# facebookresearch/robust_cvd

Measured on AMD Instinct MI355X. Metric: GN/LM iterations/sec (and ms/iter) on 300-frame 384x224 video, 1/2/4/8 GPU, higher is better.
Workload: dtype f64

## Files before the change

### include/cvd_hip_debug.h

```cpp
#ifndef CVD_HIP_DEBUG_H
#define CVD_HIP_DEBUG_H

#include "cvd_hip.h"

#ifdef __cplusplus
extern "C" {
#endif

typedef struct cvd_debug_options {
  uint64_t struct_size;
  int32_t force_iterations;
  int32_t force_sharded_path;
  int32_t pcg_lockstep;
  int32_t stall_fused_tail_once;
  int32_t tail_no_row_staging;
  int32_t tail_closes_scalars;
} cvd_debug_options;
void cvd_debug_options_default(cvd_debug_options* o);
int32_t cvd_set_debug_options(cvd_handle* h, const cvd_debug_options* o);

int32_t cvd_set_generic_kernels(cvd_handle* h, int32_t enabled);

int32_t cvd_comm_init_local_group(cvd_handle* h, int32_t rank, int32_t world, uint64_t group_key);
int32_t cvd_comm_init_phantom(cvd_handle* h, int32_t rank, int32_t world);

int32_t cvd_block_inverse_debug(cvd_handle* h, int32_t num_blocks, int32_t block_size, const double* a, int32_t variant,
                                float* inverse, int32_t* failed);

int32_t cvd_epipolar_debug(cvd_handle* h, int32_t num_pairs, const int64_t* offsets, const float* loc, double pixel_scale,
                           double threshold_px, int32_t iterations, uint64_t seed, uint8_t* is_static_out,
                           double* fundamental_out, int32_t* best_out, int32_t* counts_out, double* hypotheses_out);
int32_t cvd_flow_masks_debug(cvd_handle* h, int32_t num_frames, int32_t height, int32_t width, int32_t channels,
                             const float* color, int32_t num_pairs, const int32_t* pair_frames, const float* flow_ab,
                             const float* flow_ba, float flow_thresh, float color_thresh, uint8_t* mask_ab, uint8_t* mask_ba,
                             int32_t* kept, float* errors, double* kernel_ms, int32_t pixels_per_thread);
int32_t cvd_dense_inverse_debug(cvd_handle* h, int32_t n, const double* a, double* inverse, int32_t* failed);
int32_t cvd_coarse_debug(cvd_handle* h, int32_t* num_unknowns, double* a_c, double* a_c_inverse, int32_t* failed);
int32_t cvd_temporal_debug(cvd_handle* h, int32_t* dims6, double* a_t, double* a_t_inverse, double* lam, int32_t* failed);
int32_t cvd_product_launch_debug(cvd_handle* h, int32_t* out6);
int32_t cvd_assembly_launch_debug(cvd_handle* h, int32_t* out6, double* cost_frame);

#ifdef __cplusplus
}
#endif
#endif
```

### robust_cvd_amd/api.py

```python
import ctypes as C
import os
import sys

from . import build as _build
from .binding import Binding
from .ctypes_types import OptParams, SolveSummary, XformDesc

_lib = None
_variant = None


class SolverOptions(C.Structure):
    _fields_ = [
        ("struct_size", C.c_uint64),
        ("pcg_relative_tolerance", C.c_double),
        ("pcg_max_iterations", C.c_int32),
        ("verbose", C.c_int32),
        ("coarse_level", C.c_int32),
        ("robust_loss", C.c_int32),
        ("dense_matrix_free", C.c_int32),
        ("block_inverse_variant", C.c_int32),
        ("coarse_dense_max_unknowns", C.c_int32),
        ("coarse_rebuild_excess", C.c_int32),
        ("coarse_update_budget", C.c_int64),
        ("coarse_dense_shift", C.c_double),
        ("constraint_order", C.c_int32),
        ("coarse_rebuild_excess_dense", C.c_int32),
        ("pcg_fused_tail", C.c_int32),
        ("coarse_dense_row_split", C.c_int32),
        ("dist_owner_update", C.c_int32),
        ("temporal_level", C.c_int32),
        ("temporal_step", C.c_int32),
        ("temporal_grid_x", C.c_int32),
        ("temporal_grid_y", C.c_int32),
        ("coarse_temporal_step", C.c_int32),
        ("coarse_over_budget", C.c_int32),
        ("coarse_temporal_min_frames", C.c_int32),
        ("temporal_weight", C.c_double),
    ]


class DebugOptions(C.Structure):
    _fields_ = [
        ("struct_size", C.c_uint64),
        ("force_iterations", C.c_int32),
        ("force_sharded_path", C.c_int32),
        ("pcg_lockstep", C.c_int32),
        ("stall_fused_tail_once", C.c_int32),
        ("tail_no_row_staging", C.c_int32),
        ("tail_closes_scalars", C.c_int32),
    ]


class ConsistencyDesc(C.Structure):
    _fields_ = [
        ("struct_size", C.c_uint64),
        ("precision", C.c_int32),
        ("num_frames", C.c_int32),
        ("num_pairs", C.c_int32),
        ("height", C.c_int32),
        ("width", C.c_int32),
        ("distance_type", C.c_int32),
        ("have_warp", C.c_int32),
        ("reserved", C.c_int32),
        ("lambda_reprojection", C.c_double),
        ("lambda_disparity", C.c_double),
        ("lambda_depth_ratio", C.c_double),
        ("distance_scale", C.c_double),
        ("distance_alpha", C.c_double),
    ]


class SceneFlowDesc(C.Structure):
    _fields_ = [
        ("struct_size", C.c_uint64),
        ("precision", C.c_int32),
        ("num_frames", C.c_int32),
        ("num_pairs", C.c_int32),
        ("height", C.c_int32),
        ("width", C.c_int32),
        ("distance_type_static", C.c_int32),
        ("distance_type_smooth", C.c_int32),
        ("have_warp", C.c_int32),
        ("lambda_static", C.c_double),
        ("lambda_smooth_reprojection", C.c_double),
        ("lambda_smooth_disparity", C.c_double),
        ("lambda_smooth_depth_ratio", C.c_double),
        ("distance_scale", C.c_double),
        ("distance_alpha", C.c_double),
    ]


class SpatialDesc(C.Structure):
    _fields_ = [
        ("struct_size", C.c_uint64),
        ("precision", C.c_int32),
        ("num_frames", C.c_int32),
        ("frames_per_sample", C.c_int32),
        ("height", C.c_int32),
        ("width", C.c_int32),
        ("reserved", C.c_int32),
        ("lambda_disparity_smooth", C.c_double),
        ("sigma_color_grad", C.c_double),
        ("lambda_contrast_loss", C.c_double),
        ("contrast_thresh", C.c_double),
    ]


class ParamDesc(C.Structure):
    _fields_ = [
        ("struct_size", C.c_uint64),
        ("precision", C.c_int32),
        ("num_tensors", C.c_int32),
    ]


class ParamRecord(C.Structure):
    _fields_ = [
        ("beta1", C.c_double),
        ("beta2", C.c_double),
        ("eps", C.c_double),
        ("grad_decay", C.c_double),
        ("param_decay", C.c_double),
        ("step", C.c_double),
        ("denom_scale", C.c_double),
        ("rule", C.c_int32),
        ("reserved", C.c_int32),
    ]


class DatasetDesc(C.Structure):
    _fields_ = [
        ("struct_size", C.c_uint64),
        ("num_frames", C.c_int32),
        ("height", C.c_int32),
        ("width", C.c_int32),
        ("num_pairs", C.c_int32),
        ("num_samples", C.c_int32),
        ("temporal", C.c_int32),
        ("has_depth_orig", C.c_int32),
        ("neighbor_rule_frames", C.c_int32),
    ]


class DatasetBatchOut(C.Structure):
    _fields_ = [
        ("struct_size", C.c_uint64),
        ("images", C.c_void_p),
        ("extrinsics", C.c_void_p),
        ("intrinsics", C.c_void_p),
        ("gc_indices", C.c_void_p),
        ("gc_flows", C.c_void_p * 2),
        ("gc_masks", C.c_void_p * 2),
        ("ts_indices", C.c_void_p),
        ("ts_flows", C.c_void_p * 4),
        ("ts_masks", C.c_void_p * 4),
        ("ts_valid", C.c_void_p),
        ("scales", C.c_void_p),
        ("warp", C.c_void_p),
        ("depth_orig", C.c_void_p),
    ]


PARAM_RULES = {"adam": 0, "radam": 1, "radam_sgd": 2, "moments": 3}

DISTANCE_TYPES = {"l1": 0, "l2": 1, "smooth_l1": 2, "cauchy": 3, "general": 4}
CONSISTENCY_TERMS = ("reproj", "disp", "depth ratio")
SCENE_FLOW_TERMS = ("static", "smooth_reproj", "smooth_disparity", "smooth_depth_ratio")

ABI_REVISION = 6


def consistency_desc(precision, num_frames, num_pairs, height, width, distance="l1", scale=1.0, alpha=1.0,
                     lambdas=(1.0, 0.0, 100.0), have_warp=False):
    if distance not in DISTANCE_TYPES:
        raise ValueError(f"unknown distance {distance!r} (one of {sorted(DISTANCE_TYPES)})")
    d = ConsistencyDesc()
    d.struct_size = C.sizeof(ConsistencyDesc) | (ABI_REVISION << 32)
    d.precision = int(precision)
    d.num_frames, d.num_pairs, d.height, d.width = int(num_frames), int(num_pairs), int(height), int(width)
    d.distance_type = DISTANCE_TYPES[distance]
    d.have_warp = int(bool(have_warp))
    d.lambda_reprojection, d.lambda_disparity, d.lambda_depth_ratio = (float(v) for v in lambdas)
    d.distance_scale, d.distance_alpha = float(scale), float(alpha)
    return d


def scene_flow_desc(precision, num_frames, num_pairs, height, width, distance_static="l1", distance_smooth="l1", scale=1.0,
                    alpha=1.0, lambdas=(1.0, 1.0, 0.0, 100.0), have_warp=False):
    for distance in (distance_static, distance_smooth):
        if distance not in DISTANCE_TYPES:
            raise ValueError(f"unknown distance {distance!r} (one of {sorted(DISTANCE_TYPES)})")
    d = SceneFlowDesc()
    d.struct_size = C.sizeof(SceneFlowDesc) | (ABI_REVISION << 32)
    d.precision = int(precision)
    d.num_frames, d.num_pairs, d.height, d.width = int(num_frames), int(num_pairs), int(height), int(width)
    d.distance_type_static, d.distance_type_smooth = DISTANCE_TYPES[distance_static], DISTANCE_TYPES[distance_smooth]
    d.have_warp = int(bool(have_warp))
    (d.lambda_static, d.lambda_smooth_reprojection, d.lambda_smooth_disparity,
     d.lambda_smooth_depth_ratio) = (float(v) for v in lambdas)
    d.distance_scale, d.distance_alpha = float(scale), float(alpha)
    return d

# ... 1289 lines not shown
                self._check(self._fn("raft_encoder_timed")(*args, ms))
                kernel_ms[:] = list(ms)
            if _hip_runtime().hipDeviceSynchronize() != 0:
                raise RuntimeError("raft_encoder: the device reported an error")
            dev.download(do, out)
        return out

    @staticmethod
    def _midas_f32(who, arrays):
        import numpy as np
        for a in arrays:
            if a is not None and a.dtype != np.float32:
                raise TypeError(f"{who}: every array must be float32 (got {a.dtype})")

    def midas_conv(self, x, weight, bias=None, relu_in=False, relu=False, a=None, relu_a=False, b=None, split=0):
        import numpy as np
        x, weight = np.asarray(x), np.asarray(weight)
        bias, a, b = (None if v is None else np.asarray(v) for v in (bias, a, b))
        self._midas_f32("midas_conv", [x, weight, bias, a, b])
        B, H, W, Cin, N, k = midas_check_conv(x.shape, weight.shape, None if bias is None else bias.shape,
                                              None if a is None else a.shape, None if b is None else b.shape, split)
        out = np.zeros((B, N, H, W), np.float32)
        with _DeviceArrays() as dev:
            dx, dw = dev.upload(np.ascontiguousarray(x)), dev.upload(np.ascontiguousarray(weight))
            db, da, d2 = (None if v is None else dev.upload(np.ascontiguousarray(v)) for v in (bias, a, b))
            do = dev.alloc(out.nbytes)
            self._check(self._fn("midas_conv_device")(
                self._h, C.c_int32(B), C.c_int32(H), C.c_int32(W), C.c_int32(Cin), C.c_int32(N), C.c_int32(k), dx, dw, db,
                C.c_int32(1 if relu_in else 0), C.c_int32(1 if relu else 0), da, C.c_int32(1 if relu_a else 0), d2, C.c_int32(split),
                do, None))
            if _hip_runtime().hipDeviceSynchronize() != 0:
                raise RuntimeError("midas_conv: the device reported an error")
            dev.download(do, out)
        return out

    def midas_upsample2x(self, x, align_corners=True):
        import numpy as np
        x = np.asarray(x)
        self._midas_f32("midas_upsample2x", [x])
        B, Cn, H, W = midas_check_upsample2x(x.shape)
        out = np.zeros((B, Cn, 2 * H, 2 * W), np.float32)
        with _DeviceArrays() as dev:
            dx = dev.upload(np.ascontiguousarray(x))
            do = dev.alloc(out.nbytes)
            self._check(self._fn("midas_upsample2x_device")(
                self._h, C.c_int32(B), C.c_int32(Cn), C.c_int32(H), C.c_int32(W), C.c_int32(1 if align_corners else 0), dx, do, None))
            if _hip_runtime().hipDeviceSynchronize() != 0:
                raise RuntimeError("midas_upsample2x: the device reported an error")
            dev.download(do, out)
        return out

    def midas_head(self, x, weight2, bias2, weight4, bias4, non_negative=True):
        import numpy as np
        arrays = [np.asarray(v) for v in (x, weight2, bias2, weight4, bias4)]
        self._midas_f32("midas_head", arrays)
        B, H, W, Cin = midas_check_head(*[v.shape for v in arrays])
        out = np.zeros((B, H, W), np.float32)
        with _DeviceArrays() as dev:
            dx, dw2, db2, dw4, db4 = (dev.upload(np.ascontiguousarray(v)) for v in arrays)
            do = dev.alloc(out.nbytes)
            self._check(self._fn("midas_head_device")(
                self._h, C.c_int32(B), C.c_int32(H), C.c_int32(W), C.c_int32(Cin), C.c_int32(MIDAS_HEAD_MID), dx, dw2, db2, dw4, db4,
                C.c_int32(1 if non_negative else 0), do, None))
            if _hip_runtime().hipDeviceSynchronize() != 0:
                raise RuntimeError("midas_head: the device reported an error")
            dev.download(do, out)
        return out

    def midas_decoder(self, maps, weights, biases, non_negative=True, kernel_ms=None):
        import numpy as np
        maps = [np.asarray(v) for v in maps]
        weights, biases = [np.asarray(v) for v in weights], [np.asarray(v) for v in biases]
        self._midas_f32("midas_decoder", maps + weights + biases)
        B, features, channels, heights, widths = midas_check_decoder([v.shape for v in maps], [v.shape for v in weights],
                                                                     [v.shape for v in biases])
        out = np.zeros((B, 4 * heights[0], 4 * widths[0]), np.float32)
        with _DeviceArrays() as dev:
            dm = (C.c_void_p * 4)(*[dev.upload(np.ascontiguousarray(v)).value for v in maps])
            dw = (C.c_void_p * 21)(*[dev.upload(np.ascontiguousarray(v)).value for v in weights])
            db = (C.c_void_p * 17)(*[dev.upload(np.ascontiguousarray(v)).value for v in biases])
            do = dev.alloc(out.nbytes)
            args = (self._h, C.c_int32(B), C.c_int32(features), (C.c_int32 * 4)(*channels), (C.c_int32 * 4)(*heights),
                    (C.c_int32 * 4)(*widths), dm, dw, db, C.c_int32(1 if non_negative else 0), do, None)
            if kernel_ms is None:
                self._check(self._fn("midas_decoder_device")(*args))
            else:
                ms = (C.c_double * MIDAS_TIMED_SLOTS)()
                self._check(self._fn("midas_decoder_timed")(*args, ms))
                kernel_ms[:] = list(ms)
            if _hip_runtime().hipDeviceSynchronize() != 0:
                raise RuntimeError("midas_decoder: the device reported an error")
            dev.download(do, out)
        return out

    def num_active_constraints(self):
        return int(self._lib.cvd_num_active_constraints(self._h))

    def block_inverse_debug(self, blocks, variant=0):
        import numpy as np
        a = np.ascontiguousarray(blocks, dtype=np.float64)
        n, B, B2 = a.shape
        assert B == B2
        out = np.zeros((n, B, B), dtype=np.float32)
        fl = C.c_int32(0)
        self._check(self._fn("block_inverse_debug")(self._h, C.c_int32(n), C.c_int32(B), a.ctypes.data_as(C.POINTER(C.c_double)),
                                                    C.c_int32(variant), out.ctypes.data_as(C.POINTER(C.c_float)), C.byref(fl)))
        return out, fl.value

    def dense_inverse_debug(self, a):
        import numpy as np
        a = np.ascontiguousarray(a, dtype=np.float64)
        n = a.shape[0]
        assert a.shape == (n, n)
        out = np.zeros((n, n), dtype=np.float64)
        fl = C.c_int32(0)
        self._check(self._fn("dense_inverse_debug")(self._h, C.c_int32(n), a.ctypes.data_as(C.POINTER(C.c_double)),
                                                    out.ctypes.data_as(C.POINTER(C.c_double)), C.byref(fl)))
        return out, fl.value

    def temporal_debug(self):
        import numpy as np
        dims = (C.c_int32 * 6)()
        self._check(self._fn("temporal_debug")(self._h, dims, None, None, None, None))
        if dims[0] == 0:
            return None
        n = dims[0]
        a = np.zeros((n, n))
        ai = np.zeros((n, n))
        lam = np.zeros(self.num_frames * self.block_size())
        fl = C.c_int32(0)
        dp = lambda x: x.ctypes.data_as(C.POINTER(C.c_double))
        self._check(self._fn("temporal_debug")(self._h, dims, dp(a), dp(ai), dp(lam), C.byref(fl)))
        return {"NT": n, "S": dims[1], "nn": dims[2], "step": dims[3], "Sx": dims[4], "Sy": dims[5], "a_t": a, "a_t_inverse": ai,
                "lam": lam, "failed": fl.value}

    def path_info(self):
        out = (C.c_int32 * 8)()
        self._check(self._fn("path_info")(self._h, out))
        form = {-1: "none", 0: "exact sparse factor", 1: "exact dense inverse", 2: "temporal pose level"}[out[1]]
        return {"pose_graph_level": form, "depth_grid_level": bool(out[2]), "fused_tail": bool(out[3] & 1), "tail_rows_staged": bool(out[3] & 2),
                "product_sums_shares": bool(out[3] & 4), "rz_shares": out[3] >> 8,
                "tail_disabled": bool(out[4]),
                "taps": out[5], "work_items": out[6], "cross_blocks": bool(out[7])}

    def product_launch_debug(self):
        out = (C.c_int32 * 6)()
        self._check(self._fn("product_launch_debug")(self._h, out))
        kind = {-1: "none", 0: "generic list", 1: "fast list", 2: "fast dense", 3: "cross blocks"}[out[3]]
        return {"threads": out[0], "spec": out[1], "kd": out[2], "kind": out[3], "kind_name": kind, "work_items": out[4],
                "num_cu": out[5]}

    def assembly_launch_debug(self):
        import numpy as np
        out = (C.c_int32 * 6)()
        cost = np.zeros(self.num_frames, dtype=np.float64)
        self._check(self._fn("assembly_launch_debug")(self._h, out, cost.ctypes.data_as(C.POINTER(C.c_double))))
        kind = {-1: "none", 0: "generic", 1: "fast list", 2: "fast dense", 3: "dense fold"}[out[3]]
        return {"threads": out[0], "spec": out[1], "kd": out[2], "kind": out[3], "kind_name": kind, "workgroups": out[4],
                "split_parts": out[5], "cost_frame": cost}

    def coarse_debug(self):
        import numpy as np
        n = C.c_int32(0)
        self._check(self._fn("coarse_debug")(self._h, C.byref(n), None, None, None))
        if n.value == 0:
            return None
        a = np.zeros((n.value, n.value))
        ai = np.zeros((n.value, n.value))
        fl = C.c_int32(0)
        self._check(self._fn("coarse_debug")(self._h, C.byref(n), a.ctypes.data_as(C.POINTER(C.c_double)),
                                             ai.ctypes.data_as(C.POINTER(C.c_double)), C.byref(fl)))
        return {"a_c": a, "a_c_inverse": ai, "failed": fl.value}
```

### robust_cvd_amd/csrc/cvd_api.hip

```cpp
#include "cvd_host.h"
#include "cvd_coarse.h"

namespace cvd {

static void poseOptimizationStep(cvd_handle* h, const cvd_opt_params& p, double depthDeformReg) {
  solve(h, p, depthDeformReg, PK_POSE_STEP);
  paramsToPoses(h, p);
}

static void poseOptimization(cvd_handle* h, const cvd_opt_params& p) {
  posesToParams(h);
  h->records.clear();
  int ctfRows = p.ctf_long, ctfCols = p.ctf_short;
  int dsoRows = p.dso_long, dsoCols = p.dso_short;
  if (h->aspect >= 1.f) {
    std::swap(ctfCols, ctfRows);
    std::swap(dsoCols, dsoRows);
  }
  int initGrid[3] = {1, 1, 1};
  if (h->ddesc.depth_type == CVD_DEPTH_GRID)
    for (int i = 0; i < 3; ++i) initGrid[i] = h->ddesc.grid_size[i];
  const int Nval = (h->ddesc.depth_type == CVD_DEPTH_IDENTITY) ? 0 : valueNumParams(h->ddesc.value_xform);
  size_t nDmax = static_cast<size_t>(h->nD());
  if (p.coarse_to_fine && h->ddesc.depth_type != CVD_DEPTH_IDENTITY && p.num_steps > 1)
// ... 103 lines not shown
extern "C" {

static std::string g_createError;

cvd_handle* cvd_create(int32_t device) {
  try {
    int count = 0;
    hipError_t e = hipGetDeviceCount(&count);
    if (e != hipSuccess || count <= 0)
      throw std::runtime_error("no HIP device available: the optimizer has no CPU path");
    if (device < 0 || device >= count) throw std::runtime_error("invalid device ordinal");
    HIP_CHECK(hipSetDevice(device));
    auto* h = new cvd_handle_t();
    h->device = device;
    h->frontend = makeFrontend();
    HIP_CHECK(hipDeviceGetAttribute(&h->numCU, hipDeviceAttributeMultiprocessorCount, device));
    HIP_CHECK(hipStreamCreateWithFlags(&h->stream, hipStreamNonBlocking));
    {
      int prioLow = 0, prioHigh = 0;
      HIP_CHECK(hipDeviceGetStreamPriorityRange(&prioLow, &prioHigh));
      HIP_CHECK(hipStreamCreateWithPriority(&h->stream2, hipStreamNonBlocking, prioHigh));
    }
    HIP_CHECK(hipEventCreateWithFlags(&h->evCoarseIn, hipEventDisableTiming));
    HIP_CHECK(hipEventCreateWithFlags(&h->evCoarseDone, hipEventDisableTiming));
    HIP_CHECK(hipStreamCreateWithFlags(&h->stream3, hipStreamNonBlocking));
    HIP_CHECK(hipEventCreateWithFlags(&h->evInvIn, hipEventDisableTiming));
    HIP_CHECK(hipEventCreateWithFlags(&h->evInvDone, hipEventDisableTiming));
    cvd_solver_options_default(&h->opt);
    cvd_debug_options_default(&h->dbg);
    touchModule_setup(); touchModule_eval(); touchModule_matvec(); touchModule_precond(); touchModule_temporal(); touchModule_solve(); touchModule_frontend();
    if (device < PersistentGate::kMaxDevices) {
      PersistentGate::Slot& sl = PersistentGate::slot(device);
      std::lock_guard<std::mutex> lock(sl.m);
      if (++g_liveHandles[device] > 1) HIP_CHECK(hipDeviceSynchronize());
    }
    return h;
  } catch (const std::exception& e) {
    g_createError = e.what();
    return nullptr;
  }
}
void cvd_destroy(cvd_handle* h) {
  if (h && h->device >= 0 && h->device < PersistentGate::kMaxDevices) --g_liveHandles[h->device];
  delete h;
}
const char* cvd_last_error(cvd_handle* h) { return h ? h->err.c_str() : g_createError.c_str(); }

int32_t cvd_abi_revision(void) { return CVD_ABI_REVISION; }
void cvd_abi_sizes(int32_t* out6) {
  out6[0] = sizeof(cvd_xform_desc);
  out6[1] = sizeof(cvd_opt_params);
  out6[2] = sizeof(cvd_frame_pose);
  out6[3] = sizeof(cvd_iteration_record);
  out6[4] = sizeof(cvd_solve_summary);
  out6[5] = sizeof(cvd_solver_options);
}

void cvd_opt_params_default(cvd_opt_params* p) {
  std::memset(p, 0, sizeof(*p));
  p->max_iterations = 1000;
  p->num_threads = 12;
  p->num_steps = 4;
  p->robustness = 0.5;
  p->static_loss_type = CVD_STATIC_REPRO_DISPARITY;
  p->static_spatial_weight = 1.0;
  p->static_depth_weight = 1.0;
  p->smooth_loss_type = CVD_SMOOTH_REPRO_DISPARITY_LAPLACIAN;
  p->scale_reg = 1.0;
  p->scale_reg_grid_size = 10;
  p->depth_deform_reg_initial = 1.0;
  p->depth_deform_reg_final = 0.1;
  p->spatial_deform_reg = 1.0;
  p->focal_reg = 1.0;
  p->coarse_to_fine = 1;
  p->ctf_long = 17;
  p->ctf_short = 10;
  p->dso_long = 4;
  p->dso_short = 3;
  p->focal_long = 0.3461538376301239;
  p->intr_opt = CVD_INTR_PER_FRAME;
  p->normalize_depth_from_first_frame = 1;
}

void cvd_solver_options_default(cvd_solver_options* o) {
  o->struct_size = CVD_STRUCT_STAMP(cvd_solver_options);
  o->pcg_relative_tolerance = 1e-3;
  o->pcg_max_iterations = 300;
  o->verbose = 0;
  o->coarse_level = 1;
  o->robust_loss = 0;
  o->dense_matrix_free = 0;
  o->block_inverse_variant = 0;
  o->coarse_dense_max_unknowns = 4096;
  o->coarse_rebuild_excess = 16;
  o->coarse_update_budget = 40000;
  o->coarse_dense_shift = 1e-5;
  o->constraint_order = 1;
  o->coarse_rebuild_excess_dense = 0;
  o->pcg_fused_tail = 1;
  o->coarse_dense_row_split = 5;
  o->dist_owner_update = 1;
  o->temporal_level = 1;
  o->temporal_step = 32;
  o->temporal_grid_x = 0;
  o->temporal_grid_y = 0;
  o->coarse_temporal_step = 8;
  o->coarse_over_budget = 0;
  o->coarse_temporal_min_frames = 128;
  o->temporal_weight = 0.7;
}
int32_t cvd_set_solver_options(cvd_handle* h, const cvd_solver_options* o) {
  CVD_TRY(h, {
    if (o->struct_size != CVD_STRUCT_STAMP(cvd_solver_options))
      throw std::runtime_error(fmt("cvd_solver_options: struct_size %#llx != %#llx = sizeof | revision << 32 (caller built against "
                                   "another cvd_hip.h; start from cvd_solver_options_default)",
                                   static_cast<unsigned long long>(o->struct_size),
                                   static_cast<unsigned long long>(CVD_STRUCT_STAMP(cvd_solver_options))));
    if (o->pcg_fused_tail < 0 || o->pcg_fused_tail > 1) throw std::runtime_error("pcg_fused_tail in {0, 1}");
    if (!(o->pcg_relative_tolerance > 0.0 && o->pcg_relative_tolerance < 1.0)) throw std::runtime_error("pcg_relative_tolerance must lie in (0, 1)");
    if (o->pcg_max_iterations < 1) throw std::runtime_error("pcg_max_iterations must be >= 1");
    if (!(o->coarse_dense_shift >= 0.0 && o->coarse_dense_shift < 1.0)) throw std::runtime_error("coarse_dense_shift must lie in [0, 1)");
    if (o->coarse_rebuild_excess < 0 || o->coarse_rebuild_excess_dense < -1 || o->coarse_update_budget < 0)
      throw std::runtime_error("coarse_rebuild_excess / coarse_update_budget must be >= 0, coarse_rebuild_excess_dense >= -1");
    if (o->coarse_dense_max_unknowns < 0 || o->coarse_dense_max_unknowns > kDenseCoarseMaxUnknowns)
      throw std::runtime_error(fmt("coarse_dense_max_unknowns must lie in [0, %d] (what k_dense_spd_inverse holds in registers)",
                                   kDenseCoarseMaxUnknowns));
    if (o->coarse_level < 0 || o->coarse_level > 3 || o->coarse_temporal_step < 2 || o->robust_loss < 0 || o->robust_loss > 1 || o->block_inverse_variant < 0 ||
        o->block_inverse_variant > 2)
      throw std::runtime_error("coarse_level in {0, 1, 2, 3}, coarse_temporal_step >= 2, robust_loss in {0, 1}, block_inverse_variant in {0, 1, 2}");
    if (o->coarse_over_budget < 0 || o->coarse_over_budget > 1) throw std::runtime_error("coarse_over_budget in {0, 1}");
    if (o->coarse_temporal_min_frames < 0) throw std::runtime_error("coarse_temporal_min_frames must be >= 0");
    if (!(o->temporal_weight > 0.0 && o->temporal_weight <= 2.0)) throw std::runtime_error("temporal_weight must lie in (0, 2]");
    if (o->coarse_dense_row_split < 0 || o->coarse_dense_row_split > 8) throw std::runtime_error("coarse_dense_row_split must lie in [0, 8]");
    if (o->temporal_level < 0 || o->temporal_level > 2 || o->temporal_step < 2 || o->temporal_grid_x < 0 || o->temporal_grid_y < 0 ||
        o->temporal_grid_x == 1 || o->temporal_grid_y == 1)
      throw std::runtime_error("temporal_level in {0, 1, 2}, temporal_step >= 2, temporal_grid_x / _y 0 (automatic) or >= 2");
    if (o->coarse_update_budget != h->opt.coarse_update_budget || o->coarse_dense_max_unknowns != h->opt.coarse_dense_max_unknowns ||
        (o->coarse_level == 3) != (h->opt.coarse_level == 3) || o->coarse_temporal_step != h->opt.coarse_temporal_step ||
        o->coarse_over_budget != h->opt.coarse_over_budget || o->coarse_temporal_min_frames != h->opt.coarse_temporal_min_frames ||
        o->pcg_fused_tail != h->opt.pcg_fused_tail)
      h->tableValid = false;
    if (o->constraint_order != h->opt.constraint_order) h->orderGx = h->orderGy = -1;
    h->opt = *o;
  });
}
void cvd_debug_options_default(cvd_debug_options* o) {
  o->struct_size = CVD_STRUCT_STAMP(cvd_debug_options);
  o->force_iterations = 0;
  o->force_sharded_path = 0;
  o->pcg_lockstep = 0;
  o->stall_fused_tail_once = 0;
  o->tail_no_row_staging = 0;
  o->tail_closes_scalars = 0;
}
int32_t cvd_set_debug_options(cvd_handle* h, const cvd_debug_options* o) {
  CVD_TRY(h, {
    if (o->struct_size != CVD_STRUCT_STAMP(cvd_debug_options))
      throw std::runtime_error("cvd_debug_options: struct_size does not match this library's cvd_hip_debug.h (start from cvd_debug_options_default)");
    h->dbg = *o;
    h->distForced = h->world == 1 && (h->comm != nullptr || h->localGroup || h->phantom) && o->force_sharded_path != 0;
  });
}
void cvd_comm_unique_id(uint8_t* out128) {
  ncclUniqueId id;
  std::memset(&id, 0, sizeof(id));
  (void)ncclGetUniqueId(&id);
  std::memcpy(out128, &id, sizeof(id));
}
int32_t cvd_comm_init(cvd_handle* h, int32_t rank, int32_t world, const uint8_t* id128) {
  CVD_TRY(h, {
    if (world < 1 || rank < 0 || rank >= world) throw std::runtime_error("invalid rank / world size");
    if (h->comm) { NCCL_CHECK(ncclCommDestroy(h->comm)); h->comm = nullptr; }
    ncclUniqueId id;
    std::memcpy(&id, id128, sizeof(id));
    NCCL_CHECK(ncclCommInitRank(&h->comm, world, id, rank));
    h->rank = rank;
    h->world = world;
    h->localGroup.reset();
    h->distForced = world == 1 && h->dbg.force_sharded_path != 0;
    h->tableValid = false;
  });
}
int32_t cvd_comm_init_local_group(cvd_handle* h, int32_t rank, int32_t world, uint64_t group_key) {
  CVD_TRY(h, {
    if (world < 1 || rank < 0 || rank >= world) throw std::runtime_error("invalid rank / world size");
    if (h->comm) { NCCL_CHECK(ncclCommDestroy(h->comm)); h->comm = nullptr; }
    h->localGroup = joinLocalGroup(group_key, world);
    h->rank = rank;
    h->world = world;
    h->distForced = world == 1 && h->dbg.force_sharded_path != 0;
    h->tableValid = false;
  });
}
int32_t cvd_comm_init_phantom(cvd_handle* h, int32_t rank, int32_t world) {
  CVD_TRY(h, {
    if (world < 1 || rank < 0 || rank >= world) throw std::runtime_error("invalid rank / world size");
    if (h->comm) { NCCL_CHECK(ncclCommDestroy(h->comm)); h->comm = nullptr; }
    if (h->localGroup) { leaveLocalGroup(*h->localGroup); h->localGroup.reset(); }
    h->phantom = true;
    h->rank = rank;
    h->world = world;
    h->distForced = world == 1;
    h->tableValid = false;
  });
}
int32_t cvd_set_generic_kernels(cvd_handle* h, int32_t enabled) { CVD_TRY(h, h->forceGeneric = enabled != 0); }

int32_t cvd_set_video(cvd_handle* h, int32_t numFrames, int32_t width, int32_t height, float aspect, float invAspect) {
  CVD_TRY(h, {
    if (numFrames <= 0 || width <= 0 || height <= 0) throw std::runtime_error("invalid video dimensions");
    h->F = numFrames; h->W = width; h->H = height; h->aspect = aspect; h->invAspect = invAspect;
    h->haveDynMasks = false;
    h->adaptGx = h->adaptGy = 0;
    h->dDepth.ensure(static_cast<size_t>(numFrames) * width * height);
    HIP_CHECK(hipMemsetAsync(h->dDepth.p, 0, static_cast<size_t>(numFrames) * width * height * sizeof(float), h->stream));
    h->median.assign(numFrames, 0.f);
    h->medianDirty = true;
    h->poses.assign(numFrames, cvd_frame_pose{{0, 0, 0}, {0, 0, 0, 1}, 0.f, 0.f});
    h->poseParamsValid = false;
    cvd_xform_desc dd{};
    dd.type = CVD_XFORM_DEPTH;
    dd.depth_type = CVD_DEPTH_IDENTITY;
    cvd_xform_desc sd{};
    sd.type = CVD_XFORM_SPATIAL;
    sd.spatial_type = CVD_SPATIAL_IDENTITY;
    resetXforms(h, dd, false);
    resetXforms(h, sd, true);
    h->tableValid = false;
    h->P = 0;
    h->C = 0;
    h->dense = false;
    h->denseListValid = false;
    h->haveTriplets = false;
    h->tripCenter.clear();
    h->tripOff.clear();
    h->tripC = 0;
    h->tripActive.clear();
    h->haveGlobalEdges = false;
    h->globalEdges.clear();
    h->coarse.valid = false;
    h->pairA.clear();
    h->pairB.clear();
    h->pairOff.assign(1, 0);
  });
}

int32_t cvd_set_depth(cvd_handle* h, int32_t frame, const float* depth) {
  CVD_TRY(h, {
    if (frame < 0 || frame >= h->F) throw std::runtime_error("frame out of range");
    const size_t n = static_cast<size_t>(h->W) * h->H;
    HIP_CHECK(hipMemcpyAsync(h->dDepth.p + frame * n, depth, n * sizeof(float), hipMemcpyHostToDevice, h->stream));
    h->medianDirty = true;
    h->tableValid = false;
    HIP_CHECK(hipStreamSynchronize(h->stream));
  });
}

int32_t cvd_set_depth_all(cvd_handle* h, const float* depth) {
  CVD_TRY(h, {
    if (h->F <= 0) throw std::runtime_error("no video set");
    const size_t n = static_cast<size_t>(h->F) * h->W * h->H;
    HIP_CHECK(hipMemcpyAsync(h->dDepth.p, depth, n * sizeof(float), hipMemcpyHostToDevice, h->stream));
    h->medianDirty = true;
    h->tableValid = false;
    HIP_CHECK(hipStreamSynchronize(h->stream));
  });
}

int32_t cvd_set_pair_constraints(cvd_handle* h, int32_t numPairs, const int32_t* pairFrames, const int64_t* offsets,
                                 const float* loc4, const uint8_t* isStatic) {
  CVD_TRY(h, {
    if (numPairs < 0 || !offsets || (numPairs > 0 && !pairFrames)) throw std::runtime_error("invalid pair constraints");
    std::vector<int> order(numPairs);
    for (int i = 0; i < numPairs; ++i) order[i] = i;
    std::stable_sort(order.begin(), order.end(), [&](int a, int b) {
      if (pairFrames[2 * a] != pairFrames[2 * b]) return pairFrames[2 * a] < pairFrames[2 * b];
      return pairFrames[2 * a + 1] < pairFrames[2 * b + 1];
    });
    if (offsets[0] != 0) throw std::runtime_error("pair constraint offsets must start at 0");
    for (int i = 0; i < numPairs; ++i)
      if (offsets[i + 1] < offsets[i]) throw std::runtime_error("pair constraint offsets must be non-decreasing");
    for (int k = 1; k < numPairs; ++k)
      if (pairFrames[2 * order[k]] == pairFrames[2 * order[k - 1]] && pairFrames[2 * order[k] + 1] == pairFrames[2 * order[k - 1] + 1])
        throw std::runtime_error("duplicate directed frame pair in the constraint list (merge the two lists: the reference keeps "
                                 "one entry per pair key, lib/FlowConstraints.h:149)");
    const long long C = offsets[numPairs];
    if (C > 0 && !loc4) throw std::runtime_error("invalid pair constraints");
    for (int k = 0; k < numPairs; ++k)
      if (pairFrames[2 * k] < 0 || pairFrames[2 * k] >= h->F || pairFrames[2 * k + 1] < 0 || pairFrames[2 * k + 1] >= h->F)
        throw std::runtime_error("pair frame out of range");
    h->dense = false;
    h->denseListValid = false;
    h->dFlow.release();
    h->dFMask.release();
    h->P = numPairs;
    h->C = C;
    h->pairA.resize(numPairs);
    h->pairB.resize(numPairs);
    h->pairOff.assign(numPairs + 1, 0);
    std::vector<float> loc(static_cast<size_t>(C) * 4);
    std::vector<unsigned char> st(C, 1);
    std::vector<int> cpair(C);
    long long o = 0;
    for (int k = 0; k < numPairs; ++k) {
      const int src = order[k];
      const int a = pairFrames[2 * src], b = pairFrames[2 * src + 1];
      if (a < 0 || a >= h->F || b < 0 || b >= h->F) throw std::runtime_error("pair frame out of range");
      h->pairA[k] = a;
      h->pairB[k] = b;
      h->pairOff[k] = o;
      const long long n = offsets[src + 1] - offsets[src];
// ... 463 lines not shown
int32_t cvd_get_summary(cvd_handle* h, cvd_solve_summary* s) { CVD_TRY(h, *s = h->summary); }
int32_t cvd_num_records(cvd_handle* h) { return h ? static_cast<int32_t>(h->records.size()) : 0; }
int32_t cvd_get_records(cvd_handle* h, cvd_iteration_record* out) {
  CVD_TRY(h, std::memcpy(out, h->records.data(), sizeof(cvd_iteration_record) * h->records.size()));
}
int32_t cvd_get_kernel_times(cvd_handle* h, double* avgMs6, int64_t* launches6) {
  CVD_TRY(h, {
    for (int k = 0; k < KC_COUNT; ++k) {
      avgMs6[k] = h->kcN[k] ? h->kcMs[k] / h->kcN[k] : 0.0;
      launches6[k] = h->kcN[k];
    }
  });
}
int32_t cvd_get_dense_times(cvd_handle* h, double* avgMs2, int64_t* launches2) {
  CVD_TRY(h, {
    for (int k = 0; k < 2; ++k) {
      avgMs2[k] = h->kcN[KC_DENSE_WALK + k] ? h->kcMs[KC_DENSE_WALK + k] / h->kcN[KC_DENSE_WALK + k] : 0.0;
      launches2[k] = h->kcN[KC_DENSE_WALK + k];
    }
  });
}
int32_t cvd_get_comm_times(cvd_handle* h, double* avgMs3, int64_t* counts3) {
  CVD_TRY(h, {
    for (int k = 0; k < 3; ++k) {
      avgMs3[k] = h->kcN[KC_COUNT + k] ? h->kcMs[KC_COUNT + k] / h->kcN[KC_COUNT + k] : 0.0;
      counts3[k] = h->kcN[KC_COUNT + k];
    }
  });
}
int32_t cvd_set_kernel_timing(cvd_handle* h, int32_t enabled) {
  CVD_TRY(h, {
    h->timingStride = ((enabled >> 8) & 0xff) + 1;
    h->timingCounter = 0;
    for (auto& k : h->timingCounterKc) k = 0;
    enabled &= 0xff;
    h->timing = enabled == 1 ? 0x3f : enabled;
    for (int k = 0; k < KC_TOTAL; ++k) { h->kcMs[k] = 0.0; h->kcN[k] = 0; }
  });
}
int64_t cvd_num_active_constraints(cvd_handle* h) { return h ? h->numValid : 0; }

int32_t cvd_set_pair_graph(cvd_handle* h, int32_t numPairs, const int32_t* pairFrames) {
  CVD_TRY(h, {
    std::set<std::pair<int, int>> uniq;
    for (int i = 0; i < numPairs; ++i) {
      const int a = pairFrames[2 * i], b = pairFrames[2 * i + 1];
      if (a < 0 || a >= h->F || b < 0 || b >= h->F) throw std::runtime_error("pair graph frame out of range");
      if (a != b) uniq.insert({std::min(a, b), std::max(a, b)});
    }
    h->globalEdges.assign(uniq.begin(), uniq.end());
    h->haveGlobalEdges = numPairs > 0;
    h->tableValid = false;
  });
}

int32_t cvd_block_inverse_debug(cvd_handle* h, int32_t num_blocks, int32_t block_size, const double* a, int32_t variant,
                                float* inverse, int32_t* failed) {
  CVD_TRY(h, {
    if (num_blocks <= 0 || block_size <= 0 || block_size > kMaxFrameBlock) throw std::runtime_error("block_inverse_debug: bad sizes");
    if (variant < 0 || variant > 2) throw std::runtime_error("block_inverse_debug: variant must be 0, 1 or 2");
    const size_t n = static_cast<size_t>(num_blocks) * block_size * block_size;
    DevBuf<double> dA;
    DevBuf<double> dL;
    DevBuf<float> dM;
    DevBuf<int> dF;
    dA.ensure(n);
    dL.ensure(static_cast<size_t>(num_blocks) * block_size);
    dM.ensure(n);
    dF.ensure(1);
    hipStream_t s = h->stream;
    dA.upload(a, n, s);
    HIP_CHECK(hipMemsetAsync(dL.p, 0, static_cast<size_t>(num_blocks) * block_size * sizeof(double), s));
    HIP_CHECK(hipMemsetAsync(dM.p, 0, n * sizeof(float), s));
    HIP_CHECK(hipMemsetAsync(dF.p, 0, sizeof(int), s));
    Layout L{};
    L.F = num_blocks;
    L.B = block_size;
    launchBlockInverseRaw(h, L, dA.p, dL.p, dM.p, dF.p, variant);
    int fl = 0;
    dM.download(inverse, n, s);
    dF.download(&fl, 1, s);
    HIP_CHECK(hipStreamSynchronize(s));
    if (failed) *failed = fl;
  });
}

int32_t cvd_epipolar_debug(cvd_handle* h, int32_t num_pairs, const int64_t* offsets, const float* loc, double pixel_scale,
                           double threshold_px, int32_t iterations, uint64_t seed, uint8_t* is_static_out,
                           double* fundamental_out, int32_t* best_out, int32_t* counts_out, double* hypotheses_out) {
  CVD_TRY(h, epipolarStaticFlags(h, num_pairs, offsets, loc, pixel_scale, threshold_px, iterations, seed, is_static_out,
                                 fundamental_out, best_out, nullptr, counts_out, hypotheses_out));
}

int32_t cvd_dense_inverse_debug(cvd_handle* h, int32_t n, const double* a, double* inverse, int32_t* failed) {
  CVD_TRY(h, {
    if (n <= 0 || n > 8192) throw std::runtime_error("dense_inverse_debug: bad size");
    const size_t nn = static_cast<size_t>(n) * n;
    DevBuf<double> dA;
    DevBuf<double> dM;
    DevBuf<int> dF;
    dA.ensure(nn);
    dM.ensure(nn);
    dF.ensure(2);
    hipStream_t s = h->stream;
    dA.upload(a, nn, s);
    HIP_CHECK(hipMemsetAsync(dM.p, 0, nn * sizeof(double), s));
    HIP_CHECK(hipMemsetAsync(dF.p, 0, 2 * sizeof(int), s));
    launchDenseSpdInverse(h, n, dA.p, dM.p, dF.p, s, dF.p + 1);
    int fl[2] = {0, 0};
    dM.download(inverse, nn, s);
    dF.download(fl, 2, s);
    HIP_CHECK(hipStreamSynchronize(s));
    if (failed) *failed = fl[0];
  });
}

int32_t cvd_temporal_debug(cvd_handle* h, int32_t* dims6, double* a_t, double* a_t_inverse, double* lam, int32_t* failed) {
  CVD_TRY(h, {
    auto& T = h->temporal;
    hipStream_t s = h->stream;
    const bool on = T.on && T.built;
    const int dims[6] = {on ? T.NT : 0, T.S, T.nn, T.step, T.Sx, T.Sy};
    for (int i = 0; i < 6; ++i) dims6[i] = dims[i];
    if (on) {
      const size_t n2 = static_cast<size_t>(T.NT) * T.NT;
      if (a_t) T.A.download(a_t, n2, s);
      if (a_t_inverse) T.Ainv.download(a_t_inverse, n2, s);
      if (lam) h->dLam.download(lam, static_cast<size_t>(h->F) * h->Bsz(), s);
      int fl = 0;
      T.fail.download(&fl, 1, s);
      HIP_CHECK(hipStreamSynchronize(s));
      if (failed) *failed = fl;
    }
  });
}
int32_t cvd_path_info(cvd_handle* h, int32_t* out8) {
  CVD_TRY(h, {
    out8[0] = h->coarseOn ? 1 : 0;
    out8[1] = !h->coarseOn ? -1 : (h->coarse.temporalPose ? 2 : (h->coarse.denseMode ? 1 : 0));
    out8[2] = h->temporal.on ? 1 : 0;
    out8[3] = h->lastFusedTail ? (h->tailStageRows ? 3 : 1) : 0;
    if (h->lastFusedTail && h->lastShares) out8[3] |= 4 | (h->lastShareCount << 8);
    out8[4] = h->tailDisabled ? 1 : 0;
    out8[5] = h->lastKD;
    out8[6] = static_cast<int32_t>(h->itemFa.size());
    out8[7] = h->lastCross ? 1 : 0;
  });
}
int32_t cvd_product_launch_debug(cvd_handle* h, int32_t* out6) {
  CVD_TRY(h, {
    for (int i = 0; i < 6; ++i) out6[i] = h->lastProduct[i];
  });
}
int32_t cvd_assembly_launch_debug(cvd_handle* h, int32_t* out6, double* cost_frame) {
  CVD_TRY(h, {
    for (int i = 0; i < 6; ++i) out6[i] = h->lastAssembly[i];
    const size_t F = static_cast<size_t>(h->F);
    if (cost_frame && h->lastAssembly[3] >= 0 && h->dCostFrame.n >= F) {
      h->dCostFrame.download(cost_frame, F, h->stream);
      HIP_CHECK(hipStreamSynchronize(h->stream));
    }
  });
}
int32_t cvd_coarse_debug(cvd_handle* h, int32_t* num_unknowns, double* a_c, double* a_c_inverse, int32_t* failed) {
  CVD_TRY(h, {
    auto& C = h->coarse;
    if (!C.valid || !h->coarseOn) {
      *num_unknowns = 0;
    } else if (C.temporalPose) {
      const size_t n = static_cast<size_t>(C.ptN);
      *num_unknowns = static_cast<int32_t>(n);
      hipStream_t s = h->stream;
      int fl = 0;
      C.fail.download(&fl, 1, s);
      if (a_c) C.ptMat.download(a_c, n * n, s);
      if (a_c_inverse) C.ptInv.download(a_c_inverse, n * n, s);
      HIP_CHECK(hipStreamSynchronize(s));
      if (failed) *failed = fl;
    } else {
      const int F = h->F;
      const size_t n = static_cast<size_t>(F) * kCB;
      *num_unknowns = static_cast<int32_t>(n);
      hipStream_t s = h->stream;
      int fl = 0;
      C.fail.download(&fl, 1, s);
      if (a_c_inverse) {
        std::vector<double> save(n), unit(n, 0.0);
        C.rc.download(save.data(), n, s);
        HIP_CHECK(hipStreamSynchronize(s));
        DevBuf<double> scalTmp;
        scalTmp.ensure(S_COUNT);
        HIP_CHECK(hipMemsetAsync(scalTmp.p, 0, S_COUNT * sizeof(double), s));
        for (size_t k = 0; k < n; ++k) {
          unit[k] = 1.0;
          C.rc.upload(unit.data(), n, s);
          if (C.denseMode) {
            hipLaunchKernelGGL(k_coarse_dense_apply, dim3(F), dim3(256), 0, s, F, C.denseInv.p, C.rc.p, C.c.p, C.modeActive.p,
                               C.dotPart.p, scalTmp.p, h->dCounters.p + 3, C.fail.p, 1, 0.0, static_cast<double*>(nullptr));
          } else {
            hipLaunchKernelGGL(k_coarse_apply_w, dim3(F), dim3(1024), 0, s, C.plan, C.Wb.p, C.rc.p, C.y.p, C.dotPart.p,
                               scalTmp.p, h->dCounters.p + 3, C.fail.p, 1, 0.0, static_cast<double*>(nullptr));
            hipLaunchKernelGGL(k_coarse_apply_wt, dim3(F), dim3(256), 0, s, coarseView(h, true, true), F, C.c.p,
                               scalTmp.p, 1);
          }
          C.c.download(a_c_inverse + k * n, n, s);
          HIP_CHECK(hipStreamSynchronize(s));
          unit[k] = 0.0;
        }
        C.rc.upload(save.data(), n, s);
        HIP_CHECK(hipStreamSynchronize(s));
      }
      std::vector<double> diag(static_cast<size_t>(F) * kCBB), edges(static_cast<size_t>(std::max(C.nEdges, 1)) * kCBB);
      std::vector<unsigned char> act(n);
      std::vector<int> efa(C.nEdges), efb(C.nEdges);
      C.diag.download(diag.data(), diag.size(), s);
      C.edges.download(edges.data(), static_cast<size_t>(C.nEdges) * kCBB, s);
      C.modeActive.download(act.data(), n, s);
      C.edgeFa.download(efa.data(), efa.size(), s);
      C.edgeFb.download(efb.data(), efb.size(), s);
      HIP_CHECK(hipStreamSynchronize(s));
      if (failed) *failed = fl;
      if (a_c) {
        std::fill(a_c, a_c + n * n, 0.0);
        for (int f = 0; f < F; ++f)
          for (int i = 0; i < kCB; ++i)
            for (int j = 0; j < kCB; ++j) a_c[(static_cast<size_t>(f) * kCB + i) * n + f * kCB + j] = diag[static_cast<size_t>(f) * kCBB + i * kCB + j];
        for (int e = 0; e < C.nEdges; ++e)
          for (int i = 0; i < kCB; ++i)
            for (int j = 0; j < kCB; ++j) {
              double v = edges[static_cast<size_t>(e) * kCBB + i * kCB + j];
              if (!act[efa[e] * kCB + i] || !act[efb[e] * kCB + j]) v = 0.0;
              a_c[(static_cast<size_t>(efa[e]) * kCB + i) * n + efb[e] * kCB + j] = v;
              a_c[(static_cast<size_t>(efb[e]) * kCB + j) * n + efa[e] * kCB + i] = v;
            }
      }
    }
  });
}

}
```

### robust_cvd_amd/csrc/cvd_assembly.h

```cpp
#pragma once

#include "cvd_kernels.h"

namespace cvd {

template <int KD, int KS>
inline __global__ __launch_bounds__(256) void k_assemble(Layout L, Table T, const double* __restrict__ x,
                                                  const FrameConst* __restrict__ fc, const double* __restrict__ mask,
                                                  const float* __restrict__ median,
                                                  const unsigned char* __restrict__ inRange,
                                                  const unsigned char* __restrict__ rangeFlags,
                                                  const int* __restrict__ fpOff, const int* __restrict__ fpList,
                                                  double* __restrict__ gOut, double* __restrict__ hOut,
                                                  double* __restrict__ costFrame, double* __restrict__ focalG,
                                                  double* __restrict__ focalH, AsmPanels panels, int panelCap) {
  extern __shared__ __attribute__((aligned(16))) double sm[];
  const int B = L.B;
  double* Hs = sm;
  double* gs = Hs + panelCap;
  double* xf = gs + B;
  double* xo = xf + B;
  FrameConst* fcs = reinterpret_cast<FrameConst*>(xo + B);
  double* red = reinterpret_cast<double*>(fcs + 2);
  const int f = blockIdx.x;
  const int tid = threadIdx.x;
  for (int i = tid; i < B; i += 256) {
    gs[i] = 0.0;
    xf[i] = x[static_cast<size_t>(f) * B + i];
  }
  constexpr int FCW = sizeof(FrameConst) / 8;
  if (tid < FCW) reinterpret_cast<double*>(fcs)[tid] = reinterpret_cast<const double*>(fc + f)[tid];
  const double* mf = mask + static_cast<size_t>(f) * B;
  double* hf = hOut + static_cast<size_t>(f) * B * B;
  double staticCost = 0.0, regCostTotal = 0.0;

  for (int pass = 0; pass < panels.n; ++pass) {
  const int r0 = panels.row[pass], r1 = panels.row[pass + 1];
  const int base = r0 * (r0 + 1) / 2, npk = r1 * (r1 + 1) / 2 - base;
  const bool first = pass == 0;
#define CVD_PANEL_ADD(hi_, lo_, val_)                                                       \
  do {                                                                                      \
    const int hi__ = (hi_);                                                                 \
    if (hi__ >= r0 && hi__ < r1) atomicAdd(&Hs[packedIdx(hi__, (lo_)) - base], (val_));     \
  } while (0)
  __syncthreads();
  for (int i = tid; i < npk; i += 256) Hs[i] = 0.0;
  __syncthreads();

  double PP[28];
  double gp[7];
  double cost = 0.0;
  double shG = 0.0, shH = 0.0;
#pragma unroll
  for (int i = 0; i < 28; ++i) PP[i] = 0.0;
#pragma unroll
  for (int i = 0; i < 7; ++i) gp[i] = 0.0;

  if (L.includeStatic) {
    for (int e = fpOff[f]; e < fpOff[f + 1]; ++e) {
      const int code = fpList[e];
      const int p = code >> 1;
      const int side = code & 1;
      const int o = side ? T.pairA[p] : T.pairB[p];
      __syncthreads();
      for (int i = tid; i < B; i += 256) xo[i] = x[static_cast<size_t>(o) * B + i];
      if (tid < FCW) reinterpret_cast<double*>(fcs + 1)[tid] = reinterpret_cast<const double*>(fc + o)[tid];
      __syncthreads();
      const FrameConst& fa = side ? fcs[1] : fcs[0];
      const FrameConst& fb = side ? fcs[0] : fcs[1];
      const double* xa = side ? xo : xf;
      const double* xb = side ? xf : xo;
      for (long long c = T.pairOff[p] + tid; c < T.pairOff[p + 1]; c += 256) {
        const float2 d = T.dsrc[c];
        if (!(d.x > 0.f)) continue;
        Sample<KD, KS> s;
        evalSample<KD, KS, true>(L, fa, fb, xa, xb, T.ndc[c], d, s);
        const double w = s.rho1;
        if (L.intrOpt == kIntrShared) {
#pragma unroll
          for (int rr = 0; rr < 3; ++rr) {
            const double tot = s.a.Jp[rr][6] + s.b.Jp[rr][6];
            s.a.Jp[rr][6] = tot;
            s.b.Jp[rr][6] = tot;
          }
          if (!side && first) {
            shG += w * (s.a.Jp[0][6] * s.r[0] + s.a.Jp[1][6] * s.r[1] + s.a.Jp[2][6] * s.r[2]);
            shH += w * (s.a.Jp[0][6] * s.a.Jp[0][6] + s.a.Jp[1][6] * s.a.Jp[1][6] + s.a.Jp[2][6] * s.a.Jp[2][6]);
          }
        }
        const Side<KD, KS>& me = side ? s.b : s.a;
        if (!side && first) cost += s.rho0;
        if (first) {
          int q = 0;
#pragma unroll
          for (int i = 0; i < 7; ++i) {
            gp[i] += w * (me.Jp[0][i] * s.r[0] + me.Jp[1][i] * s.r[1] + me.Jp[2][i] * s.r[2]);
#pragma unroll
            for (int j = 0; j <= i; ++j) {
              PP[q] += w * (me.Jp[0][i] * me.Jp[0][j] + me.Jp[1][i] * me.Jp[1][j] + me.Jp[2][i] * me.Jp[2][j]);
              ++q;
            }
          }
        }
        const int nt = sideNumTapCols(L, me);
        for (int t = 0; t < nt; ++t) {
          int ct;
          double Jt[3];
          sideTapCol(L, me, t, ct, Jt);
          const double wj0 = w * Jt[0], wj1 = w * Jt[1], wj2 = w * Jt[2];
          if (first) atomicAdd(&gs[ct], wj0 * s.r[0] + wj1 * s.r[1] + wj2 * s.r[2]);
          if (ct >= r0 && ct < r1) {
            const int rowBase = ct * (ct + 1) / 2 - base;
#pragma unroll
            for (int i = 0; i < 7; ++i)
              atomicAdd(&Hs[rowBase + i], wj0 * me.Jp[0][i] + wj1 * me.Jp[1][i] + wj2 * me.Jp[2][i]);
          }
          for (int t2 = 0; t2 <= t; ++t2) {
            int c2;
            double J2[3];
            sideTapCol(L, me, t2, c2, J2);
            const double val = wj0 * J2[0] + wj1 * J2[1] + wj2 * J2[2];
            const int hi = ct > c2 ? ct : c2, lo = ct > c2 ? c2 : ct;
            CVD_PANEL_ADD(hi, lo, val);
          }
        }
      }
    }
  }
  __syncthreads();
  if (first) {
    {
#pragma unroll
      for (int i = 0; i < 28; ++i) PP[i] = waveSum(PP[i]);
#pragma unroll
      for (int i = 0; i < 7; ++i) gp[i] = waveSum(gp[i]);
      cost = waveSum(cost);
      const int wv = tid >> 6;
      if ((tid & 63) == 0) {
#pragma unroll
        for (int i = 0; i < 28; ++i) red[wv * 36 + i] = PP[i];
#pragma unroll
        for (int i = 0; i < 7; ++i) red[wv * 36 + 28 + i] = gp[i];
        red[wv * 36 + 35] = cost;
      }
    }
    __syncthreads();
    if (tid < 28) {
      int i = 0;
      while ((i + 1) * (i + 2) / 2 <= tid) ++i;
      const int j = tid - i * (i + 1) / 2;
      Hs[packedIdx(i, j)] += red[tid] + red[36 + tid] + red[72 + tid] + red[108 + tid];
    } else if (tid < 35) {
      gs[tid - 28] += red[tid] + red[36 + tid] + red[72 + tid] + red[108 + tid];
    }
    __syncthreads();
    staticCost = 0.5 * (red[35] + red[36 + 35] + red[72 + 35] + red[108 + 35]);
    __syncthreads();
  }
  if (L.intrOpt == kIntrShared) {
    if (first) {
      shG = waveSum(shG);
      shH = waveSum(shH);
      if ((tid & 63) == 0) { red[tid >> 6] = shG; red[4 + (tid >> 6)] = shH; }
      __syncthreads();
      if (tid == 0) {
        focalG[f] = red[0] + red[1] + red[2] + red[3];
        focalH[f] = red[4] + red[5] + red[6] + red[7];
        gs[6] = 0.0;
        Hs[packedIdx(6, 6)] = 0.0;
      }
    }
    if (f != 0) {
      for (int j = tid; j < B; j += 256) {
        if (j == 6) continue;
        const int hi = j > 6 ? j : 6, lo = j > 6 ? 6 : j;
        if (hi >= r0 && hi < r1) Hs[packedIdx(hi, lo) - base] = 0.0;
      }
    }
    __syncthreads();
  }

  double regCost = 0.0;
  if (inRange[f]) {
    const int nr = numRegResiduals<KD>(L);
    for (int i = tid; i < nr; i += 256) {
      double r;
      int n;
      int cols[2 * KD + 2];
      double jac[2 * KD + 2];
      regResidual<KD>(L, f, i, xf, median[f], r, n, cols, jac);
      if (first) regCost += r * r;
      for (int a = 0; a < n; ++a) {
        if (first) atomicAdd(&gs[cols[a]], jac[a] * r);
        for (int b = 0; b <= a; ++b) {
          const int hi = cols[a] > cols[b] ? cols[a] : cols[b];
          const int lo = cols[a] > cols[b] ? cols[b] : cols[a];
          CVD_PANEL_ADD(hi, lo, jac[a] * jac[b]);
        }
      }
    }
  }
  if (tid == 0 && L.positionRegSqrt > 0.0 && first) {
    double o3[3] = {0, 0, 0}, dg = 0.0, cst = 0.0;
    posRegFrame(L, rangeFlags, f, x, nullptr, o3, dg, cst);
    for (int i = 0; i < 3; ++i) {
      atomicAdd(&gs[i], o3[i]);
      atomicAdd(&Hs[packedIdx(i, i)], dg);
    }
    regCost += cst;
  }
  if (first) {
    regCost = waveSum(regCost);
    __syncthreads();
    if ((tid & 63) == 0) red[tid >> 6] = regCost;
    __syncthreads();
    regCostTotal = 0.5 * (red[0] + red[1] + red[2] + red[3]);
  }
  __syncthreads();
  for (int idx = tid; idx < npk; idx += 256) {
    int i = static_cast<int>((sqrt(8.0 * static_cast<double>(idx + base) + 1.0) - 1.0) * 0.5);
    while (i * (i + 1) / 2 > idx + base) --i;
    while ((i + 1) * (i + 2) / 2 <= idx + base) ++i;
    const int j = idx + base - i * (i + 1) / 2;
    const double v = Hs[idx] * mf[i] * mf[j];
    hf[static_cast<size_t>(i) * B + j] = v;
    hf[static_cast<size_t>(j) * B + i] = v;
  }
#undef CVD_PANEL_ADD
  }
  if (tid == 0) costFrame[f] = staticCost + regCostTotal;
  __syncthreads();
  for (int i = tid; i < B; i += 256) gOut[static_cast<size_t>(f) * B + i] = gs[i] * mf[i];
}

inline __global__ __launch_bounds__(256) void k_shared_focal_fixup(Layout L, const double* __restrict__ focalG,
                                                            const double* __restrict__ focalH,
                                                            const double* __restrict__ mask, double* __restrict__ g,
                                                            double* __restrict__ hBlocks) {
  __shared__ double red[8];
  double a = 0.0, b = 0.0;
  for (int f = threadIdx.x; f < L.F; f += 256) { a += focalG[f]; b += focalH[f]; }
  a = waveSum(a);
  b = waveSum(b);
  if ((threadIdx.x & 63) == 0) { red[threadIdx.x >> 6] = a; red[4 + (threadIdx.x >> 6)] = b; }
  __syncthreads();
  if (threadIdx.x == 0) {
    const double m = mask[6];
    g[6] += (red[0] + red[1] + red[2] + red[3]) * m;
    hBlocks[static_cast<size_t>(6) * L.B + 6] += (red[4] + red[5] + red[6] + red[7]) * m * m;
  }
}

inline __global__ void k_extract_diag(Layout L, const double* __restrict__ hBlocks, double* __restrict__ out) {
  const size_t n = static_cast<size_t>(L.F) * L.B;
  const size_t i = static_cast<size_t>(blockIdx.x) * blockDim.x + threadIdx.x;
  if (i >= n) return;
  const size_t f = i / L.B, c = i - f * L.B;
  out[i] = hBlocks[(f * L.B + c) * L.B + c];
}


#ifdef CVD_ASM_PROFILE
__device__ unsigned long long g_asmProf[2048 * 16];
#define ASM_STAMP(slot) do { if (lane == 0) g_asmProf[(blockIdx.x & 2047) * 16 + (slot)] = wall_clock64(); } while (0)
#else
#define ASM_STAMP(slot) do {} while (0)
#endif

template <int KD, int SPEC>
__device__ __forceinline__ void asmWalkSpec(const Layout& L, const Table& T, RecordStream<false>& rs, long long cBegin, int n,
                                            int lane, const bool side, const FrameConst& Fa, const FrameConst& Fb,
                                            const double* __restrict__ xa, const double* __restrict__ xb, double* Hs,
                                            double* gs, double (&PP)[28], double (&gp)[7], double (&GD)[19], double& cost) {
  const double A = L.aspect;
  double RaU[9], RbU[9], dTU[3];
#pragma unroll
  for (int i = 0; i < 9; ++i) { RaU[i] = uniformValue(Fa.R[i]); RbU[i] = uniformValue(Fb.R[i]); }
#pragma unroll
  for (int i = 0; i < 3; ++i) dTU[i] = uniformValue(Fa.t[i] - Fb.t[i]);
  const double fya = uniformValue(Fa.fy), fxa = fya * A;
  const double fyb = uniformValue(Fb.fy);
  const double ifyb = uniformValue(1.0 / fyb), ifxb = uniformValue(1.0 / (fyb * A));
  for (int ci = lane; ci < n; ci += 64) {
    float4 nd;
    float2 d;
    if (!rs.take(T, cBegin, ci, 64, n, 0, 0, 0, nd, d)) continue;
    const double da = static_cast<double>(d.x), db = static_cast<double>(d.y);
    FastTaps<KD> ta, tb;
    fastGather<KD>(L, nd.x, nd.y, ta);
    fastGather<KD>(L, nd.z, nd.w, tb);
    double Da = 0.0, Db = 0.0;
#pragma unroll
    for (int k = 0; k < KD; ++k) {
      if (ta.ok(k)) Da += xa[7 + ta.I(k)] * ta.Wt(k);
      if (tb.ok(k)) Db += xb[7 + tb.I(k)] * tb.Wt(k);
    }
    Da *= da;
    Db *= db;
    const double pax = static_cast<double>(nd.x), pay = static_cast<double>(nd.y);
    const double pbx = static_cast<double>(nd.z), pby = static_cast<double>(nd.w);
    double ca[3], Rca[3];
    fastRay(RaU, pax, pay, fxa, fya, ca, Rca);
    const double v[3] = {dTU[0] + Rca[0] * Da, dTU[1] + Rca[1] * Da, dTU[2] + Rca[2] * Da};
    double zz, iz, u, vv, r[3], dr2dA, dr2dDb;
    fastProject<true>(L, RbU, v, ifxb, ifyb, pbx, pby, zz, iz, u, vv, r[0], r[1]);
    fastDepthResidual<true>(L, kLossDisparity, zz, iz, Db, r[2], dr2dA, dr2dDb);
    const double sq = r[0] * r[0] + r[1] * r[1] + r[2] * r[2];
    const double w = fastRobustRho1<SPEC>(L, sq);
    if (!side) cost += fastRobustRho0<SPEC>(L, sq);

    double m00, m11, m02, m12;
    fastRows(L, iz, u, vv, ifxb, ifyb, m00, m11, m02, m12);
    const double m22 = -dr2dA;
    double G[3][3];
#pragma unroll
    for (int i = 0; i < 3; ++i) {
      G[0][i] = m00 * RbU[i * 3 + 0] + m02 * RbU[i * 3 + 2];
      G[1][i] = m11 * RbU[i * 3 + 1] + m12 * RbU[i * 3 + 2];
      G[2][i] = m22 * RbU[i * 3 + 2];
    }
    double Jp[3][7];
    double JD[3];
    if (!side) {
      const double X[3] = {Da * Rca[0], Da * Rca[1], Da * Rca[2]};
      const double cf0 = pax * A, cf1 = pay;
      const double dXdf[3] = {Da * (RaU[0] * cf0 + RaU[1] * cf1), Da * (RaU[3] * cf0 + RaU[4] * cf1),
                              Da * (RaU[6] * cf0 + RaU[7] * cf1)};
#pragma unroll
      for (int rr = 0; rr < 3; ++rr) {
        Jp[rr][0] = G[rr][0]; Jp[rr][1] = G[rr][1]; Jp[rr][2] = G[rr][2];
        Jp[rr][3] = X[1] * G[rr][2] - X[2] * G[rr][1];
        Jp[rr][4] = X[2] * G[rr][0] - X[0] * G[rr][2];
        Jp[rr][5] = X[0] * G[rr][1] - X[1] * G[rr][0];
        Jp[rr][6] = dot3(G[rr], dXdf);
        JD[rr] = dot3(G[rr], Rca);
      }
    } else {
#pragma unroll
      for (int rr = 0; rr < 3; ++rr) {
        Jp[rr][0] = -G[rr][0]; Jp[rr][1] = -G[rr][1]; Jp[rr][2] = -G[rr][2];
        Jp[rr][3] = G[rr][1] * v[2] - G[rr][2] * v[1];
        Jp[rr][4] = G[rr][2] * v[0] - G[rr][0] * v[2];
        Jp[rr][5] = G[rr][0] * v[1] - G[rr][1] * v[0];
      }
      Jp[0][6] = -L.ws * u * ifyb;
      Jp[1][6] = -L.ws * vv * ifyb;
      Jp[2][6] = 0.0;
      JD[0] = 0.0; JD[1] = 0.0; JD[2] = dr2dDb;
    }
    int qi = 0;
#pragma unroll
    for (int i = 0; i < 7; ++i) {
      gp[i] += w * (Jp[0][i] * r[0] + Jp[1][i] * r[1] + Jp[2][i] * r[2]);
#pragma unroll
      for (int j = 0; j <= i; ++j) {
        PP[qi] += w * (Jp[0][i] * Jp[0][j] + Jp[1][i] * Jp[1][j] + Jp[2][i] * Jp[2][j]);
        ++qi;
      }
    }
    double v7[7];
#pragma unroll
    for (int i = 0; i < 7; ++i) v7[i] = w * (Jp[0][i] * JD[0] + Jp[1][i] * JD[1] + Jp[2][i] * JD[2]);
    const double sDD = w * (JD[0] * JD[0] + JD[1] * JD[1] + JD[2] * JD[2]);
    const double sDr = w * (JD[0] * r[0] + JD[1] * r[1] + JD[2] * r[2]);
    const FastTaps<KD>& tm = side ? tb : ta;
    const double dm = side ? db : da;
    if constexpr (KD == 1) {
      const double fac = tm.Wt(0) * dm;
#pragma unroll
      for (int i = 0; i < 7; ++i) GD[i] += v7[i] * fac;
      GD[17] += sDr * fac;
      GD[14] += sDD * fac * fac;
    } else {
#pragma unroll
      for (int ka = 0; ka < KD; ++ka) {
        if (!tm.ok(ka)) continue;
        const double fa = tm.Wt(ka) * dm;
        const int ct = 7 + tm.I(ka);
        const int rowBase = ct * (ct + 1) / 2;
        atomicAdd(&gs[ct], sDr * fa);
#pragma unroll
        for (int i = 0; i < 7; ++i) atomicAdd(&Hs[rowBase + i], v7[i] * fa);
        const double sfa = sDD * fa;
#pragma unroll
        for (int kb = 0; kb <= ka; ++kb) {
          if (!tm.ok(kb)) continue;
          const int c2 = 7 + tm.I(kb);
          const int hi = (KD == 16 || ct > c2) ? ct : c2, lo = (KD == 16 || ct > c2) ? c2 : ct;
          atomicAdd(&Hs[packedIdx(hi, lo)], sfa * (tm.Wt(kb) * dm));
        }
      }
    }
  }
}

template <int NT>
__device__ __forceinline__ void asmLocalToAxisAngle(const double* __restrict__ Jl, int B, int tid, double* Hs, double* gs) {
  double J[9];
#pragma unroll
  for (int i = 0; i < 9; ++i) J[i] = Jl[i];
  for (int j = tid; j < B; j += NT) {
    if (j >= 3 && j <= 5) continue;
    const int i0 = j < 3 ? packedIdx(3, j) : packedIdx(j, 3);
    const int i1 = j < 3 ? packedIdx(4, j) : packedIdx(j, 4);
    const int i2 = j < 3 ? packedIdx(5, j) : packedIdx(j, 5);
    const double h0 = Hs[i0], h1 = Hs[i1], h2 = Hs[i2];
    Hs[i0] = J[0] * h0 + J[1] * h1 + J[2] * h2;
    Hs[i1] = J[3] * h0 + J[4] * h1 + J[5] * h2;
    Hs[i2] = J[6] * h0 + J[7] * h1 + J[8] * h2;
  }
  if (tid == NT - 1) {
    double S[3][3], JS[3][3];
#pragma unroll
    for (int a = 0; a < 3; ++a)
#pragma unroll
      for (int b = 0; b < 3; ++b) S[a][b] = Hs[a >= b ? packedIdx(3 + a, 3 + b) : packedIdx(3 + b, 3 + a)];
#pragma unroll
    for (int a = 0; a < 3; ++a)
#pragma unroll
      for (int b = 0; b < 3; ++b) JS[a][b] = J[a * 3] * S[0][b] + J[a * 3 + 1] * S[1][b] + J[a * 3 + 2] * S[2][b];
#pragma unroll
    for (int a = 0; a < 3; ++a)
#pragma unroll
      for (int b = 0; b <= a; ++b)
        Hs[packedIdx(3 + a, 3 + b)] = JS[a][0] * J[b * 3] + JS[a][1] * J[b * 3 + 1] + JS[a][2] * J[b * 3 + 2];
    const double g0 = gs[3], g1 = gs[4], g2 = gs[5];
    gs[3] = J[0] * g0 + J[1] * g1 + J[2] * g2;
    gs[4] = J[3] * g0 + J[4] * g1 + J[5] * g2;
    gs[5] = J[6] * g0 + J[7] * g1 + J[8] * g2;
  }
}

template <int KD, int NT>
__device__ __forceinline__ double asmRegularisersSpec(const Layout& L, int f, int tid, const double* __restrict__ xf, float median,
                                                      double* Hs, double* gs) {
  constexpr double eps = 1e-6;
  double regCost = 0.0;
  if (L.scaleRegSqrt > 0.0) {
    const int ns = L.sregX * L.sregY;
    const bool taps = KD > 1 || L.depthType == kDepthGlobal;
    for (int i = tid; i < ns; i += NT) {
      const int y = i / L.sregX, x = i - y * L.sregX;
      const float lx = __fadd_rn(-1.f, __fdiv_rn(__fmul_rn(2.f, static_cast<float>(x)), static_cast<float>(L.sregX - 1)));
      const float ly = __fadd_rn(-1.f, __fdiv_rn(__fmul_rn(2.f, static_cast<float>(y)), static_cast<float>(L.sregY - 1)));
      FastTaps<KD> t;
      fastGather<KD>(L, lx, ly, t);
      const double d = static_cast<double>(median);
      double D = (L.depthType == kDepthIdentity) ? d : 0.0;
#pragma unroll
      for (int k = 0; k < KD; ++k)
        if (taps && t.ok(k)) D += d * xf[7 + t.I(k)] * t.Wt(k);
      const bool o = !(D < eps);
      const double dd = o ? D : eps;
      const double r = L.scaleRegSqrt * (1.0 / dd - 1.0);
      const double drdD = o ? (-L.scaleRegSqrt / (dd * dd)) : 0.0;
      regCost += r * r;
#pragma unroll
      for (int ka = 0; ka < KD; ++ka) {
        if (!(taps && t.ok(ka))) continue;
        const int ca = 7 + t.I(ka);
        const double ja = drdD * t.Wt(ka) * d;
        atomicAdd(&gs[ca], ja * r);
#pragma unroll
        for (int kb = 0; kb <= ka; ++kb) {
          if (!t.ok(kb)) continue;
          const int cb = 7 + t.I(kb);
          const int hi = ca > cb ? ca : cb, lo = ca > cb ? cb : ca;
          atomicAdd(&Hs[packedIdx(hi, lo)], ja * (drdD * t.Wt(kb) * d));
        }
      }
    }
  }
  Layout Lr = L;
  Lr.scaleRegSqrt = 0.0;
  const int nr = numRegResiduals<KD>(Lr);
  for (int i = tid; i < nr; i += NT) {
    double r;
    int n;
    int cols[2 * KD + 2];
    double jac[2 * KD + 2];
    regResidual<KD>(Lr, f, i, xf, median, r, n, cols, jac);
    regCost += r * r;
    if (n >= 1) {
      atomicAdd(&gs[cols[0]], jac[0] * r);
      atomicAdd(&Hs[packedIdx(cols[0], cols[0])], jac[0] * jac[0]);
    }
    if (n >= 2) {
      atomicAdd(&gs[cols[1]], jac[1] * r);
      const int hi = cols[1] > cols[0] ? cols[1] : cols[0], lo = cols[1] > cols[0] ? cols[0] : cols[1];
      atomicAdd(&Hs[packedIdx(hi, lo)], jac[1] * jac[0]);
      atomicAdd(&Hs[packedIdx(cols[1], cols[1])], jac[1] * jac[1]);
    }
  }
  return regCost;
}

template <int KD, bool DENSE = false, bool STAGE = false, bool FOLD = false, int SPEC = 0>
inline __global__ __launch_bounds__(kAsmThreads) void k_assemble_fast(Layout L, Table T, const double* __restrict__ x,
                                                       const FrameConst* __restrict__ fc,
                                                       const double* __restrict__ mask, const float* __restrict__ median,
                                                       const unsigned char* __restrict__ regOwner,
                                                       const unsigned char* __restrict__ rangeFlags,
                                                       AsmWork work,
                                                       double* __restrict__ gOut, double* __restrict__ hOut,
                                                       double* __restrict__ costFrame, double* __restrict__ focalG,
                                                       double* __restrict__ focalH, DenseRecords dr = DenseRecords{}) {
  extern __shared__ __attribute__((aligned(16))) double sm[];
  constexpr double eps = 1e-6;
  const int B = L.B;
  const int npk = B * (B + 1) / 2;
  double* Hs = sm;
  double* gs = Hs + npk;
  double* xf = gs + B;
  double* red = xf + B;
  double* xstage = red + 4 * 36;
  const AsmPart me = FOLD ? AsmPart{static_cast<int>(blockIdx.x), 0, 0, 0, 1, 0} : work.parts[blockIdx.x];
  const int f = me.frame;
  const int tid = threadIdx.x;
  static_assert(SPEC == 0 || (!DENSE && !FOLD), "the specialised walk is list mode only");
  constexpr int NT = kAsmThreads;
  const int wv = __builtin_amdgcn_readfirstlane(tid >> 6);
  const int lane = tid & 63;
  if (tid == 0) ASM_STAMP(0);
  for (int i = tid; i < npk; i += NT) Hs[i] = 0.0;
  if (tid < 48) red[tid] = 0.0;
  for (int i = tid; i < B; i += NT) {
    gs[i] = 0.0;
    xf[i] = x[static_cast<size_t>(f) * B + i];
  }
  __syncthreads();
  if (tid == 0) ASM_STAMP(1);

  double PP[28], gp[7];
  double GD[19];
#pragma unroll
  for (int i = 0; i < 19; ++i) GD[i] = 0.0;
  double cost = 0.0;
  double shG = 0.0, shH = 0.0;
#pragma unroll
  for (int i = 0; i < 28; ++i) PP[i] = 0.0;
#pragma unroll
  for (int i = 0; i < 7; ++i) gp[i] = 0.0;
  const int N = SPEC ? 1 : L.N;
  const double A = L.aspect;

  if constexpr (FOLD) {
    if (L.includeStatic) {
      const int G = L.nD;
      const int recN = dwRecordDoubles(G);
      const int e0 = dr.fpOff[f], e1 = dr.fpOff[f + 1];
      const int nOut = 36 + 13 * G;
      for (int o = tid; o < nOut; o += NT) {
        int off0, off1, c = -1, v = 0;
        if (o < 28) {
          int i = 0;
          while ((i + 1) * (i + 2) / 2 <= o) ++i;
          const int j = o - i * (i + 1) / 2;
          off0 = i * 16 + j;
          off1 = (7 + i) * 16 + 7 + j;
        } else if (o < 35) {
          off0 = (o - 28) * 16 + 14;
          off1 = (7 + o - 28) * 16 + 14;
        } else if (o == 35) {
          off0 = 256 + 40 * G;
          off1 = -1;
        } else {
          const int e = o - 36;
          c = e / G;
          v = e - c * G;
          if (c < 7) { off0 = 256 + c * G + v; off1 = 256 + 15 * G + (7 + c) * G + v; }
          else if (c == 7) { off0 = 256 + 14 * G + v; off1 = 256 + 29 * G + v; }
          else { off0 = 256 + 30 * G + (c - 8) * G + v; off1 = 256 + 35 * G + (c - 8) * G + v; }
        }
        double s = 0.0;
        for (int e = e0; e < e1; ++e) {
          const int code = dr.fpList[e];
          const int off = (code & 1) ? off1 : off0;
          if (off < 0) continue;
          for (int q = dr.recOff[code >> 1]; q < dr.recOff[(code >> 1) + 1]; ++q) s += dr.records[static_cast<size_t>(q) * recN + off];
        }
        if (o < 36) atomicAdd(&red[o], s);
        else if (c < 7) Hs[packedIdx(7 + v, c)] = s;
        else if (c == 7) gs[7 + v] = s;
        else {
          const int d = c - 8;
          const int v2 = v + (d == 0 ? 0 : (d == 1 ? 1 : L.gx + d - 3));
          if (v2 < G) atomicAdd(&Hs[packedIdx(7 + v2, 7 + v)], s);
        }
      }
    }
  } else
  if (L.includeStatic) {
    for (int u = me.u0 + wv; u < me.u1; u += NT / 64) {
      const int2 unit = work.units[u];
      const int code = __builtin_amdgcn_readfirstlane(unit.x);
      const int p = code >> 1;
      const int side = code & 1;
      const int o = side ? T.pairA[p] : T.pairB[p];
      const double* __restrict__ xo = x + static_cast<size_t>(o) * B;
      const FrameConst& Fa = side ? fc[o] : fc[f];
      const FrameConst& Fb = side ? fc[f] : fc[o];
      double* xw = xstage + wv * B;
      if constexpr (SPEC != 0) {
        const long long pOff = T.pairOff[p];
        const long long cb = pOff + __builtin_amdgcn_readfirstlane(unit.y);
        const long long pEnd = T.pairOff[p + 1];
        const int n = static_cast<int>((cb + kAsmUnit < pEnd ? cb + kAsmUnit : pEnd) - cb);
        RecordStream<false> rs;
        rs.prime(T, cb, lane, n);
        if constexpr (STAGE) {
          for (int i = lane; i < B; i += 64) xw[i] = xo[i];
          asm volatile("s_waitcnt vmcnt(0) lgkmcnt(0)" ::: "memory");
        }
        const double* xov = STAGE ? xw : xo;
        asmWalkSpec<KD, SPEC>(L, T, rs, cb, n, lane, side != 0, Fa, Fb, side ? xov : xf,
                              side ? xf : xov, Hs, gs, PP, gp, GD, cost);
        continue;
      }
      if constexpr (STAGE) {
        for (int i = lane; i < B; i += 64) xw[i] = xo[i];
        asm volatile("s_waitcnt vmcnt(0) lgkmcnt(0)" ::: "memory");
      }
      const double* xa = STAGE ? (side ? xw : xf) : (side ? xo : xf);
      const double* xb = STAGE ? (side ? xf : xw) : (side ? xf : xo);
      const double fya = Fa.fy, fxa = Fa.fy * A;
      const double fyb = Fb.fy;
      const double ifyb = 1.0 / fyb, ifxb = 1.0 / (fyb * A);
      const long long cBegin = T.pairOff[p] + __builtin_amdgcn_readfirstlane(unit.y);
      constexpr int kUnit = DENSE ? kAsmUnitDense : kAsmUnit;
      const long long cEnd = cBegin + kUnit < T.pairOff[p + 1] ? cBegin + kUnit : T.pairOff[p + 1];
      const int fsrc = side ? o : f, ftgt = side ? f : o;
      const long long cFirst = DENSE ? cBegin + static_cast<long long>(lane) * kDenseRun : cBegin + lane;
      const long long cStop = DENSE ? (cFirst + kDenseRun < cEnd ? cFirst + kDenseRun : cEnd) : cEnd;
      constexpr long long cStep = DENSE ? 1 : 64;
      RecordStream<true> rs;
      const int iFirst = static_cast<int>(cFirst - cBegin), iStop = static_cast<int>(cStop - cBegin);
      if constexpr (DENSE) rs.prime(T, cBegin, iFirst, iStop);
      for (long long c = cFirst; c < cStop; c += cStep) {
        float4 nd;
        float2 d;
        if constexpr (DENSE) {
          if (!rs.take(T, cBegin, static_cast<int>(c - cBegin), 1, iStop, T.pairOff[p], fsrc, ftgt, nd, d)) continue;
        } else {
          if (!loadConstraint<false>(T, c, T.pairOff[p], fsrc, ftgt, nd, d)) continue;
        }
        const double da = static_cast<double>(d.x), db = static_cast<double>(d.y);
        FastTaps<KD> ta, tb;
        fastGather<KD>(L, nd.x, nd.y, ta);
        fastGather<KD>(L, nd.z, nd.w, tb);
        double Da, Db;
        if (N == 0) {
          Da = da; Db = db;
        } else {
          Da = 0.0; Db = 0.0;
#pragma unroll
          for (int k = 0; k < KD; ++k) {
            if (ta.ok(k)) {
              const int ia = ta.I(k);
              if (N == 2) Da += (da * xa[7 + ia * 2] + xa[7 + ia * 2 + 1]) * ta.Wt(k);
              else Da += da * xa[7 + ia] * ta.Wt(k);
            }
            if (tb.ok(k)) {
              const int ib = tb.I(k);
              if (N == 2) Db += (db * xb[7 + ib * 2] + xb[7 + ib * 2 + 1]) * tb.Wt(k);
              else Db += db * xb[7 + ib] * tb.Wt(k);
            }
          }
        }
        const double pax = static_cast<double>(nd.x), pay = static_cast<double>(nd.y);
        const double pbx = static_cast<double>(nd.z), pby = static_cast<double>(nd.w);
        const double ca[3] = {pax * fxa, pay * fya, -1.0};
        const double Rca[3] = {dot3(Fa.R, ca), dot3(Fa.R + 3, ca), dot3(Fa.R + 6, ca)};
        const double v[3] = {Fa.t[0] + Rca[0] * Da - Fb.t[0], Fa.t[1] + Rca[1] * Da - Fb.t[1],
                             Fa.t[2] + Rca[2] * Da - Fb.t[2]};
        const double q0 = Fb.R[0] * v[0] + Fb.R[3] * v[1] + Fb.R[6] * v[2];
        const double q1 = Fb.R[1] * v[0] + Fb.R[4] * v[1] + Fb.R[7] * v[2];
        const double q2 = Fb.R[2] * v[0] + Fb.R[5] * v[1] + Fb.R[8] * v[2];
        const double zz = -q2;
        const double iz = 1.0 / zz;
        const double u = q0 * iz * ifxb;
        const double vv = q1 * iz * ifyb;
        double r[3];
        r[0] = (u - pbx) * L.ws;
        r[1] = (vv - pby) * L.ws;
        double dr2dA, dr2dDb;
        if (L.lossType == kLossDisparity) {
          const bool zo = !(zz < eps), bo = !(Db < eps);
          const double izc = zo ? iz : 1.0 / eps, ibc = 1.0 / (bo ? Db : eps);
          r[2] = (izc - ibc) * L.wd;
          dr2dA = zo ? (-L.wd * izc * izc) : 0.0;
          dr2dDb = bo ? (L.wd * ibc * ibc) : 0.0;
        } else {
          const bool zIsMax = !(zz < Db), zIsMin = !(Db < zz);
          const double mx = zIsMax ? zz : Db, mn = zIsMin ? zz : Db;
          if (L.lossType == kLossRatio) {
            r[2] = (mx / mn - 1.0) * L.wd;
            const double dmx = 1.0 / mn, dmn = -mx / (mn * mn);
            dr2dA = ((zIsMax ? dmx : 0.0) + (zIsMin ? dmn : 0.0)) * L.wd;
            dr2dDb = ((zIsMax ? 0.0 : dmx) + (zIsMin ? 0.0 : dmn)) * L.wd;
          } else {
            r[2] = log(mn / mx) * L.wd;
            const double dmn = 1.0 / mn, dmx = -1.0 / mx;
            dr2dA = ((zIsMax ? dmx : 0.0) + (zIsMin ? dmn : 0.0)) * L.wd;
            dr2dDb = ((zIsMax ? 0.0 : dmx) + (zIsMin ? 0.0 : dmn)) * L.wd;
          }
        }
        double rho0, w;
        robustRho(L, r[0] * r[0] + r[1] * r[1] + r[2] * r[2], rho0, w);
        if (!side) cost += rho0;

        const double wiz = L.ws * iz;
        const double m00 = wiz * ifxb, m11 = wiz * ifyb, m02 = wiz * u, m12 = wiz * vv, m22 = -dr2dA;
        double Jp[3][7];
        double JD[3];
        const FastTaps<KD>& tm = side ? tb : ta;
        const double dm = side ? db : da;
        if (!side) {
          double G[3][3];
#pragma unroll
          for (int i = 0; i < 3; ++i) {
            G[0][i] = m00 * Fb.R[i * 3 + 0] + m02 * Fb.R[i * 3 + 2];
            G[1][i] = m11 * Fb.R[i * 3 + 1] + m12 * Fb.R[i * 3 + 2];
            G[2][i] = m22 * Fb.R[i * 3 + 2];
          }
          const double cf[3] = {pax * A, pay, 0.0};
          const double dXdf[3] = {Da * (Fa.R[0] * cf[0] + Fa.R[1] * cf[1]), Da * (Fa.R[3] * cf[0] + Fa.R[4] * cf[1]),
                                  Da * (Fa.R[6] * cf[0] + Fa.R[7] * cf[1])};
#pragma unroll
          for (int rr = 0; rr < 3; ++rr) {
            Jp[rr][0] = G[rr][0]; Jp[rr][1] = G[rr][1]; Jp[rr][2] = G[rr][2];
            Jp[rr][6] = dot3(G[rr], dXdf);
            JD[rr] = dot3(G[rr], Rca);
          }
#pragma unroll
          for (int i = 0; i < 3; ++i) {
            const double dX[3] = {Da * dot3(Fa.dR[i], ca), Da * dot3(Fa.dR[i] + 3, ca), Da * dot3(Fa.dR[i] + 6, ca)};
            Jp[0][3 + i] = dot3(G[0], dX);
            Jp[1][3 + i] = dot3(G[1], dX);
            Jp[2][3 + i] = dot3(G[2], dX);
          }
        } else {
#pragma unroll
          for (int i = 0; i < 3; ++i) {
            Jp[0][i] = -(m00 * Fb.R[i * 3 + 0] + m02 * Fb.R[i * 3 + 2]);
            Jp[1][i] = -(m11 * Fb.R[i * 3 + 1] + m12 * Fb.R[i * 3 + 2]);
            Jp[2][i] = -(m22 * Fb.R[i * 3 + 2]);
            const double* D = Fb.dR[i];
            const double dq0 = D[0] * v[0] + D[3] * v[1] + D[6] * v[2];
            const double dq1 = D[1] * v[0] + D[4] * v[1] + D[7] * v[2];
            const double dq2 = D[2] * v[0] + D[5] * v[1] + D[8] * v[2];
            Jp[0][3 + i] = m00 * dq0 + m02 * dq2;
            Jp[1][3 + i] = m11 * dq1 + m12 * dq2;
            Jp[2][3 + i] = m22 * dq2;
          }
          Jp[0][6] = -L.ws * u * ifyb;
          Jp[1][6] = -L.ws * vv * ifyb;
          Jp[2][6] = 0.0;
          JD[0] = 0.0; JD[1] = 0.0; JD[2] = dr2dDb;
        }
        if (L.intrOpt == kIntrShared) {
          if (!side) {
            Jp[0][6] += -L.ws * u * ifyb;
            Jp[1][6] += -L.ws * vv * ifyb;
          } else {
            const double cf[3] = {pax * A, pay, 0.0};
            const double dXdf[3] = {Da * (Fa.R[0] * cf[0] + Fa.R[1] * cf[1]), Da * (Fa.R[3] * cf[0] + Fa.R[4] * cf[1]),
                                    Da * (Fa.R[6] * cf[0] + Fa.R[7] * cf[1])};
#pragma unroll
            for (int i = 0; i < 3; ++i) {
              Jp[0][6] += (m00 * Fb.R[i * 3 + 0] + m02 * Fb.R[i * 3 + 2]) * dXdf[i];
              Jp[1][6] += (m11 * Fb.R[i * 3 + 1] + m12 * Fb.R[i * 3 + 2]) * dXdf[i];
              Jp[2][6] += (m22 * Fb.R[i * 3 + 2]) * dXdf[i];
            }
          }
          if (!side) {
            shG += w * (Jp[0][6] * r[0] + Jp[1][6] * r[1] + Jp[2][6] * r[2]);
            shH += w * (Jp[0][6] * Jp[0][6] + Jp[1][6] * Jp[1][6] + Jp[2][6] * Jp[2][6]);
          }
        }
        int qi = 0;
#pragma unroll
        for (int i = 0; i < 7; ++i) {
          gp[i] += w * (Jp[0][i] * r[0] + Jp[1][i] * r[1] + Jp[2][i] * r[2]);
#pragma unroll
          for (int j = 0; j <= i; ++j) {
            PP[qi] += w * (Jp[0][i] * Jp[0][j] + Jp[1][i] * Jp[1][j] + Jp[2][i] * Jp[2][j]);
            ++qi;
          }
        }
        if (N > 0) {
          double v7[7];
#pragma unroll
          for (int i = 0; i < 7; ++i) v7[i] = w * (Jp[0][i] * JD[0] + Jp[1][i] * JD[1] + Jp[2][i] * JD[2]);
          const double sDD = w * (JD[0] * JD[0] + JD[1] * JD[1] + JD[2] * JD[2]);
          const double sDr = w * (JD[0] * r[0] + JD[1] * r[1] + JD[2] * r[2]);
          if constexpr (KD == 16) {
#pragma unroll
            for (int ka = 0; ka < 16; ++ka) {
              if (!tm.ok(ka)) continue;
              const double wa = tm.Wt(ka);
              const int ia = tm.I(ka);
#pragma unroll
              for (int na = 0; na < 2; ++na) {
                if (na >= N) continue;
                const int ct = 7 + ia * N + na;
                const double fa = (N == 2 && na == 1) ? wa : wa * dm;
                const int rowBase = ct * (ct + 1) / 2;
                atomicAdd(&gs[ct], sDr * fa);
#pragma unroll
                for (int i = 0; i < 7; ++i) atomicAdd(&Hs[rowBase + i], v7[i] * fa);
#pragma unroll
                for (int kb = 0; kb <= ka; ++kb) {
                  if (!tm.ok(kb)) continue;
                  const double wb = tm.Wt(kb);
                  const int ib = tm.I(kb);
#pragma unroll
                  for (int nb = 0; nb < 2; ++nb) {
                    if (nb >= N || (kb == ka && nb > na)) continue;
                    const int c2 = 7 + ib * N + nb;
                    const double fb = (N == 2 && nb == 1) ? wb : wb * dm;
                    atomicAdd(&Hs[rowBase + c2], sDD * fa * fb);
                  }
                }
              }
            }
          } else {
          double fac[KD * 2];
          int col[KD * 2];
#pragma unroll
          for (int k = 0; k < KD; ++k) {
            if (N == 2) {
              col[2 * k] = 7 + tm.I(k) * 2;       fac[2 * k] = tm.Wt(k) * dm;
              col[2 * k + 1] = col[2 * k] + 1;    fac[2 * k + 1] = tm.Wt(k);
            } else {
              col[k] = 7 + tm.I(k);               fac[k] = tm.Wt(k) * dm;
            }
          }
          const int nt = (N == 2) ? 2 * KD : KD;
          if constexpr (KD == 1) {
#pragma unroll
            for (int a = 0; a < 2; ++a) {
              if (a < nt) {
#pragma unroll
                for (int i = 0; i < 7; ++i) GD[a * 7 + i] += v7[i] * fac[a];
                GD[17 + a] += sDr * fac[a];
              }
            }
            GD[14] += sDD * fac[0] * fac[0];
            if (N == 2) { GD[15] += sDD * fac[1] * fac[0]; GD[16] += sDD * fac[1] * fac[1]; }
          } else {
#pragma unroll
          for (int a = 0; a < KD * 2; ++a) {
            if (a < nt) {
              const int ct = col[a];
              const int rowBase = ct * (ct + 1) / 2;
              atomicAdd(&gs[ct], sDr * fac[a]);
#pragma unroll
              for (int i = 0; i < 7; ++i) atomicAdd(&Hs[rowBase + i], v7[i] * fac[a]);
#pragma unroll
              for (int b = 0; b < KD * 2; ++b) {
                if (b <= a) {
                  const int c2 = col[b];
                  const int hi = ct > c2 ? ct : c2, lo = ct > c2 ? c2 : ct;
                  atomicAdd(&Hs[packedIdx(hi, lo)], sDD * fac[a] * fac[b]);
                }
              }
            }
          }
          }
          }
        }
      }
    }
  }
  ASM_STAMP(4 + wv);
  __syncthreads();
  if (tid == 0) ASM_STAMP(2);
  {
#pragma unroll
    for (int i = 0; i < 28; ++i) PP[i] = waveSum(PP[i]);
#pragma unroll
    for (int i = 0; i < 7; ++i) gp[i] = waveSum(gp[i]);
    cost = waveSum(cost);
    if constexpr (KD == 1) {
      if (N > 0) {
#pragma unroll
        for (int i = 0; i < 19; ++i) GD[i] = waveSum(GD[i]);
        if (lane == 0) {
          for (int a = 0; a < N; ++a) {
            const int ct = 7 + a;
            for (int i = 0; i < 7; ++i) atomicAdd(&Hs[ct * (ct + 1) / 2 + i], GD[a * 7 + i]);
            atomicAdd(&gs[ct], GD[17 + a]);
          }
          atomicAdd(&Hs[packedIdx(7, 7)], GD[14]);
          if (N == 2) { atomicAdd(&Hs[packedIdx(8, 7)], GD[15]); atomicAdd(&Hs[packedIdx(8, 8)], GD[16]); }
        }
      }
    }
    if (lane == 0) {
#pragma unroll
      for (int i = 0; i < 28; ++i) atomicAdd(&red[i], PP[i]);
#pragma unroll
      for (int i = 0; i < 7; ++i) atomicAdd(&red[28 + i], gp[i]);
      atomicAdd(&red[35], cost);
    }
  }
  __syncthreads();
  if (tid < 28) {
    int i = 0;
    while ((i + 1) * (i + 2) / 2 <= tid) ++i;
    const int j = tid - i * (i + 1) / 2;
    Hs[packedIdx(i, j)] += red[tid];
  } else if (tid < 35) {
    gs[tid - 28] += red[tid];
  }
  __syncthreads();
  const double staticCost = 0.5 * red[35];
  __syncthreads();
  if constexpr (SPEC != 0) {
    asmLocalToAxisAngle<NT>(fc[f].Jl, B, tid, Hs, gs);
    __syncthreads();
  }
  if (tid == 0) ASM_STAMP(13);
  if (L.intrOpt == kIntrShared) {
    shG = waveSum(shG);
    shH = waveSum(shH);
    if (lane == 0) { red[wv] = shG; red[16 + wv] = shH; }
    __syncthreads();
    if (tid == 0) {
      double sg = 0.0, sh = 0.0;
      for (int w = 0; w < NT / 64; ++w) { sg += red[w]; sh += red[16 + w]; }
      focalG[f] = sg;
      focalH[f] = sh;
      red[42] = sg;
      red[43] = sh;
      gs[6] = 0.0;
      Hs[packedIdx(6, 6)] = 0.0;
    }
    if (f != 0) {
      for (int j = tid; j < B; j += NT)
        if (j != 6) Hs[j > 6 ? packedIdx(j, 6) : packedIdx(6, j)] = 0.0;
    }
    __syncthreads();
  }

  if (tid == 0) ASM_STAMP(14);
  double regCost = 0.0;
  if constexpr (SPEC != 0) {
    if (regOwner[f] && me.part == 0) regCost = asmRegularisersSpec<KD, NT>(L, f, tid, xf, median[f], Hs, gs);
  } else
  if (regOwner[f] && me.part == 0) {
    const int nr = numRegResiduals<KD>(L);
    for (int i = tid; i < nr; i += NT) {
      double r;
      int n;
      int cols[2 * KD + 2];
      double jac[2 * KD + 2];
      regResidual<KD>(L, f, i, xf, median[f], r, n, cols, jac);
      regCost += r * r;
      for (int a = 0; a < n; ++a) {
        atomicAdd(&gs[cols[a]], jac[a] * r);
        for (int b = 0; b <= a; ++b) {
          const int hi = cols[a] > cols[b] ? cols[a] : cols[b];
          const int lo = cols[a] > cols[b] ? cols[b] : cols[a];
          atomicAdd(&Hs[packedIdx(hi, lo)], jac[a] * jac[b]);
        }
      }
    }
  }
  if (tid == 0 && L.positionRegSqrt > 0.0 && me.part == 0) {
    double o3[3] = {0, 0, 0}, dg = 0.0, cst = 0.0;
    posRegFrame(L, rangeFlags, f, x, nullptr, o3, dg, cst);
    for (int i = 0; i < 3; ++i) {
      atomicAdd(&gs[i], o3[i]);
      atomicAdd(&Hs[packedIdx(i, i)], dg);
    }
    regCost += cst;
  }
  regCost = waveSum(regCost);
  __syncthreads();
  if (tid == 0) ASM_STAMP(15);
  if (lane == 0) red[wv] = regCost;
  __syncthreads();
  if (tid == 0) {
    double rc = 0.0;
    for (int w = 0; w < NT / 64; ++w) rc += red[w];
    if (me.nParts == 1) costFrame[f] = staticCost + 0.5 * rc;
    red[40] = staticCost + 0.5 * rc;
  }
  if (me.nParts > 1) {
    __syncthreads();
    const size_t stride = static_cast<size_t>(npk) + B + 4;
    double* mine = work.scratch + static_cast<size_t>(me.slot0 + me.part) * stride;
    for (int i = tid; i < npk; i += NT) mine[i] = Hs[i];
    for (int i = tid; i < B; i += NT) mine[npk + i] = gs[i];
    if (tid == 0) {
      mine[npk + B] = red[40];
      if (L.intrOpt == kIntrShared) { mine[npk + B + 1] = red[42]; mine[npk + B + 2] = red[43]; }
    }
    if (!lastBlockArrives(work.counters + f, static_cast<unsigned int>(me.nParts), reinterpret_cast<int*>(red + 41))) return;
#if CVD_DETERMINISTIC
    double costSum = 0.0, sgSum = 0.0, shSum = 0.0;
    for (int i = tid; i < npk; i += NT) Hs[i] = 0.0;
    for (int i = tid; i < B; i += NT) gs[i] = 0.0;
    for (int q = 0; q < me.nParts; ++q) {
#else
    double costSum = red[40];
    double sgSum = red[42], shSum = red[43];
    for (int q = 0; q < me.nParts; ++q) {
      if (q == me.part) continue;
#endif
      const double* other = work.scratch + static_cast<size_t>(me.slot0 + q) * stride;
      for (int i = tid; i < npk; i += NT) Hs[i] += other[i];
      for (int i = tid; i < B; i += NT) gs[i] += other[npk + i];
      costSum += other[npk + B];
      if (L.intrOpt == kIntrShared) { sgSum += other[npk + B + 1]; shSum += other[npk + B + 2]; }
    }
    if (tid == 0) {
      costFrame[f] = costSum;
      if (L.intrOpt == kIntrShared) { focalG[f] = sgSum; focalH[f] = shSum; }
    }
    __syncthreads();
  }

  if (tid == 0) ASM_STAMP(3);
  const double* mf = mask + static_cast<size_t>(f) * B;
// ... 12 lines not shown
```

### robust_cvd_amd/csrc/cvd_eval.hip

```cpp
#include "cvd_host.h"
#include "cvd_cost.h"
#include "cvd_assembly.h"
#include "cvd_triplets.h"
#include "cvd_dense_walk.h"

namespace cvd {

void launchFrameConsts(Ctx& c, const double* x) {
  launchFrameConsts(c.L, x, c.h->dFc.p, c.h->stream);
  HIP_CHECK(hipGetLastError());
}

void spinStream(hipStream_t s) {
  hipError_t e;
  while ((e = hipStreamQuery(s)) == hipErrorNotReady) {}
  HIP_CHECK(e);
}
void spinEvent(hipEvent_t ev) {
  hipError_t e;
  while ((e = hipEventQuery(ev)) == hipErrorNotReady) {}
  HIP_CHECK(e);
}
void readScalars(Ctx& c) {
  HIP_CHECK(hipMemcpyAsync(c.h->hScal, c.h->dScal.p, S_COUNT * sizeof(double), hipMemcpyDeviceToHost, c.h->stream));
  spinStream(c.h->stream);
}

void enqueueCost(Ctx& c, const double* x) {
  cvd_handle* h = c.h;
  hipStream_t s = h->stream;
  launchFrameConsts(c, x);
  const int slot = h->tBegin(KC_COST);
  if (c.L.includeStatic && c.nItems > 0) {
    const size_t lds = (2 * c.L.B) * 8 + 2 * sizeof(FrameConst) + 8 * 8;
    const bool fast = !h->forceGeneric && c.KS == 0 && fastLoss(c.L);
    if (fast) {
      CVD_DISPATCH_KD(c.KD, {
        if (h->dense) {
          allowLds((k_cost_items_fast<KD, true>), lds);
          hipLaunchKernelGGL((k_cost_items_fast<KD, true>), dim3(c.nItems), dim3(256), lds, s, c.L, c.T, c.it, x, h->dFc.p,
                             h->dCostItem.p);
        } else {
          allowLds((k_cost_items_fast<KD, false>), lds);
          hipLaunchKernelGGL((k_cost_items_fast<KD, false>), dim3(c.nItems), dim3(256), lds, s, c.L, c.T, c.it, x, h->dFc.p,
                             h->dCostItem.p);
        }
      });
    } else {
      CVD_DISPATCH(c.KD, c.KS, {
        allowLds(k_cost_items<KD, KS>, lds);
        hipLaunchKernelGGL((k_cost_items<KD, KS>), dim3(c.nItems), dim3(256), lds, s, c.L, c.T, c.it, x, h->dFc.p,
                           h->dCostItem.p);
      });
    }
    HIP_CHECK(hipGetLastError());
  }
  CVD_DISPATCH_KD(c.KD, {
    hipLaunchKernelGGL((k_cost_frames<KD>), dim3(c.L.F), dim3(256), static_cast<size_t>(c.L.B) * 8, s, c.L, x, h->dMedian.p, h->dRegOwner.p, h->dInRange.p,
                       h->dCostFrame.p);
  });
  HIP_CHECK(hipGetLastError());
  if (c.trip && c.TT.nGroups > 0) {
    CVD_DISPATCH(c.KD, c.KS, {
      hipLaunchKernelGGL((k_cost_triplets<KD, KS>), dim3(c.TT.nGroups), dim3(256), 0, s, c.L, c.TT, x, h->dFc.p,
                         h->dCostFrame.p);
    });
    HIP_CHECK(hipGetLastError());
  }
  hipLaunchKernelGGL(k_sum2, dim3(1), dim3(256), 0, s, h->dCostItem.p, (c.L.includeStatic ? c.nItems : 0),
                     h->dCostFrame.p, c.L.F, h->dScal.p, S_COST);
  HIP_CHECK(hipGetLastError());
  if (h->dist()) commAllReduce(h, h->dScal.p + S_COST, 1, CT_F64, s);
  h->tEnd(slot);
}
double evalCost(Ctx& c, const double* x) {
  enqueueCost(c, x);
  readScalars(c);
  return c.h->hScal[S_COST];
}

void enqueueStats(Ctx& c) {
  cvd_handle* h = c.h;
  const int G = static_cast<int>(std::min<size_t>(128, (c.n + 511) / 512));
  h->dStatPart.ensure(7 * 128);
  hipLaunchKernelGGL(k_step_stats, dim3(G), dim3(256), 0, h->stream, c.n, h->dDx.p, h->dG.p, h->dR.p, h->dLam.p,
                     h->dX.p, h->dHd.p, h->dScal.p, h->dStatPart.p, h->dCounters.p + 2);
  HIP_CHECK(hipGetLastError());
}

bool crossScope(cvd_handle* h, const Ctx& c) {
  const bool off = h->opt.dense_matrix_free != 0;
  return h->dense && !off && !h->forceGeneric && c.L.includeStatic && !h->xFa.empty() && c.KS == 0 && fastLoss(c.L) &&
         c.L.N == 1 && c.L.nD > 0 && (c.KD == 4 || (c.KD == 1 && c.L.nD == 1)) && c.L.intrOpt != CVD_INTR_SHARED && !c.trip && !(c.L.positionRegSqrt > 0.0) &&
         c.L.B <= 256 && (static_cast<size_t>(c.L.B) * (c.L.B + 1) / 2 + 2 * c.L.B + 4 * 36) * 8 <= kMaxLds &&
         dwLdsBytes(c.L.nD, c.L.B, kDwThreads) <= kMaxLds;
}
CrossPairs crossPairs(cvd_handle* h) {
  return CrossPairs{h->dXFa.p, h->dXFb.p, h->dXRange.p, h->dXSlot.p, static_cast<int>(h->xFa.size())};
}
DenseRecords denseRecords(cvd_handle* h) {
  return DenseRecords{h->dDwRecords.p, h->dDwRecOff.p, h->dFpOff.p, h->dFpList.p};
}
void launchDenseWalk(Ctx& c, const double* x) {
  cvd_handle* h = c.h;
  const int G = c.L.nD, B = c.L.B;
  h->dDwRecords.ensure(static_cast<size_t>(std::max(1, h->nDwRecords)) * dwRecordDoubles(G));
  h->dDwGg.ensure(static_cast<size_t>(std::max<long long>(1, h->C)));
  if (h->nDwRecords == 0) return;
  const size_t lds = dwLdsBytes(G, B, kDwThreads);
  const DenseWalkList wl{h->dDwPair.p, h->nDwRecords, denseLaneMap(h->W, h->H)};
  allowLds((k_dense_walk<4>), lds);
  const int slot = h->tBegin(KC_DENSE_WALK);
  hipLaunchKernelGGL((k_dense_walk<4>), dim3(h->nDwRecords), dim3(kDwThreads), lds, h->stream, c.L, c.T, wl, x, h->dFc.p,
                     h->dDwRecords.p, h->dDwGg.p);
  h->tEnd(slot);
  HIP_CHECK(hipGetLastError());
}
void launchCrossAssemble(Ctx& c, const double* x) {
  (void)x;
  cvd_handle* h = c.h;
  const size_t B = c.L.B, G = c.L.nD;
  h->dXBlocks.ensure(h->xFa.size() * B * B);
  const unsigned nP = static_cast<unsigned>(h->xFa.size());
  if (nP == 0) return;
  hipLaunchKernelGGL(k_dense_fold_cross, dim3(nP), dim3(256), 0, h->stream, c.L, crossPairs(h), h->dXDir.p, h->dDwRecOff.p,
                     h->dDwRecords.p, h->dXBlocks.p);
  int panelW = static_cast<int>(((kMaxLds - 4096) / 8) / G);
  panelW = std::max(1, std::min<int>(panelW, static_cast<int>(G)));
  const int nPanels = static_cast<int>((G + panelW - 1) / panelW);
  panelW = static_cast<int>((G + nPanels - 1) / nPanels);
  const size_t ldsGrid = static_cast<size_t>(panelW) * G * 8;
  allowLds((k_dense_gg<4>), ldsGrid);
  const int slot = h->tBegin(KC_DENSE_GG);
  for (int dir = 0; dir < 2; ++dir)
    hipLaunchKernelGGL((k_dense_gg<4>), dim3(nP, nPanels), dim3(kGgThreads), ldsGrid, h->stream, c.L, c.T, crossPairs(h), h->dXDir.p,
                       h->dDwGg.p, panelW, dir, h->dXBlocks.p);
  h->tEnd(slot);
  HIP_CHECK(hipGetLastError());
}

double evalFull(Ctx& c, const double* x, bool withStats, bool noReadBack) {
  cvd_handle* h = c.h;
  hipStream_t s = h->stream;
  launchFrameConsts(c, x);
  const size_t B = c.L.B;
  const int slot = h->tBegin(KC_ASSEMBLE);
  const bool fast = !h->forceGeneric && c.KS == 0 && fastLoss(c.L);
  const size_t ldsFast = (B * (B + 1) / 2 + 2 * B + 4 * 36) * 8;
  const size_t ldsRest = 3 * B * 8 + 2 * sizeof(FrameConst) + 4 * 36 * 8;
  int panelCap = 0;
  const bool fastFits = ldsFast <= kMaxLds;
  auto recordAsm = [h](int threads, int spec, int kd, int kind, int groups, int splitParts) {
    const int v[6] = {threads, spec, kd, kind, groups, splitParts};
    for (int i = 0; i < 6; ++i) h->lastAssembly[i] = v[i];
  };
  if (fast && fastFits) {
    h->dAsmScratch.ensure(static_cast<size_t>(h->nAsmSlots) * (B * (B + 1) / 2 + B + 4));
    const AsmWork work{h->dAsmParts.p, h->dAsmUnits.p, h->dAsmScratch.p, h->dAsmCount.p};
    const int spec = (!h->dense && c.L.N == 1 && c.L.lossType == CVD_STATIC_REPRO_DISPARITY && c.L.intrOpt != CVD_INTR_SHARED)
                         ? (c.L.robustKind == 0 ? 1 : 2) : 0;
    const size_t ldsStage = ldsFast + static_cast<size_t>(kAsmThreads / 64) * B * 8;
    const bool stage = ldsStage <= kMaxLds;
#define CVD_LAUNCH_ASM_S(DENSEV, STAGEV, SPECV)                                                                            \
    CVD_DISPATCH_KD(c.KD, {                                                                                              \
      recordAsm(kAsmThreads, SPECV, KD, DENSEV ? 2 : 1, h->nAsmParts, h->nAsmSlots);                                       \
      allowLds((k_assemble_fast<KD, DENSEV, STAGEV, false, SPECV>), STAGEV ? ldsStage : ldsFast);                          \
      hipLaunchKernelGGL((k_assemble_fast<KD, DENSEV, STAGEV, false, SPECV>), dim3(h->nAsmParts),                          \
                         dim3(kAsmThreads), STAGEV ? ldsStage : ldsFast, s,                                                \
                         c.L, c.T, x, h->dFc.p, h->dMask.p, h->dMedian.p, h->dRegOwner.p, h->dInRange.p, work, h->dG.p, h->dH.p,  \
                         h->dCostFrame.p, h->dFocal.p, h->dFocal.p + c.L.F);                                             \
    })
#define CVD_LAUNCH_ASM(DENSEV, STAGEV) CVD_LAUNCH_ASM_S(DENSEV, STAGEV, 0)
#ifndef CVD_ASM_STAGE
#define CVD_ASM_STAGE 1
#endif
    if (c.cross) {
      launchDenseWalk(c, x);
      recordAsm(kAsmThreads, 0, c.KD, 3, c.L.F, 0);
      if (c.KD == 1) {
        allowLds((k_assemble_fast<1, true, false, true>), ldsFast);
        hipLaunchKernelGGL((k_assemble_fast<1, true, false, true>), dim3(c.L.F), dim3(kAsmThreads), ldsFast, s, c.L, c.T, x, h->dFc.p,
                           h->dMask.p, h->dMedian.p, h->dRegOwner.p, h->dInRange.p, work, h->dG.p, h->dH.p, h->dCostFrame.p,
                           h->dFocal.p, h->dFocal.p + c.L.F, denseRecords(h));
      } else {
        allowLds((k_assemble_fast<4, true, false, true>), ldsFast);
        hipLaunchKernelGGL((k_assemble_fast<4, true, false, true>), dim3(c.L.F), dim3(kAsmThreads), ldsFast, s, c.L, c.T, x, h->dFc.p,
                           h->dMask.p, h->dMedian.p, h->dRegOwner.p, h->dInRange.p, work, h->dG.p, h->dH.p, h->dCostFrame.p,
                           h->dFocal.p, h->dFocal.p + c.L.F, denseRecords(h));
      }
    } else if (h->dense) { if (stage && CVD_ASM_STAGE) CVD_LAUNCH_ASM(true, true); else CVD_LAUNCH_ASM(true, false); }
    else if (spec == 1) { if (stage && CVD_ASM_STAGE) CVD_LAUNCH_ASM_S(false, true, 1); else CVD_LAUNCH_ASM_S(false, false, 1); }
    else if (spec == 2) { if (stage && CVD_ASM_STAGE) CVD_LAUNCH_ASM_S(false, true, 2); else CVD_LAUNCH_ASM_S(false, false, 2); }
    else { if (stage && CVD_ASM_STAGE) CVD_LAUNCH_ASM(false, true); else CVD_LAUNCH_ASM(false, false); }
#undef CVD_LAUNCH_ASM
#undef CVD_LAUNCH_ASM_S
  } else {
    if (h->dense && c.L.includeStatic) throw std::logic_error("dense mode: the generic assembly has no images to read (DenseListScope should have taken this solve)");
    const AsmPanels panels = makePanels(static_cast<int>(B), (kMaxLds - ldsRest) / 8, panelCap);
    const size_t lds = static_cast<size_t>(panelCap) * 8 + ldsRest;
    recordAsm(256, 0, c.KD, 0, c.L.F, 0);
    CVD_DISPATCH(c.KD, c.KS, {
      allowLds(k_assemble<KD, KS>, lds);
      hipLaunchKernelGGL((k_assemble<KD, KS>), dim3(c.L.F), dim3(256), lds, s, c.L, c.T, x, h->dFc.p, h->dMask.p,
                         h->dMedian.p, h->dRegOwner.p, h->dInRange.p, h->dFpOff.p, h->dFpList.p, h->dG.p, h->dH.p, h->dCostFrame.p,
                       h->dFocal.p, h->dFocal.p + c.L.F, panels, panelCap);
    });
  }
  HIP_CHECK(hipGetLastError());
  if (c.trip && c.TT.nGroups > 0) {
    int panelCapT = 0;
    const AsmPanels panelsT = makePanels(static_cast<int>(B), (kMaxLds - B * 8 - 256) / 8, panelCapT);
    const size_t ldsT = (static_cast<size_t>(panelCapT) + B) * 8;
    CVD_DISPATCH(c.KD, c.KS, {
      allowLds(k_assemble_triplets<KD, KS>, ldsT);
      hipLaunchKernelGGL((k_assemble_triplets<KD, KS>), dim3(c.L.F), dim3(256), ldsT, s, c.L, c.TT, x, h->dFc.p,
                         h->dMask.p, h->dFtOff.p, h->dFtList.p, h->dG.p, h->dH.p, h->dFocal.p, h->dFocal.p + c.L.F,
                         panelsT, panelCapT);
      hipLaunchKernelGGL((k_cost_triplets<KD, KS>), dim3(c.TT.nGroups), dim3(256), 0, s, c.L, c.TT, x, h->dFc.p,
                         h->dCostFrame.p);
    });
    HIP_CHECK(hipGetLastError());
  }
  if (c.L.intrOpt == CVD_INTR_SHARED) {
    hipLaunchKernelGGL(k_shared_focal_fixup, dim3(1), dim3(256), 0, s, c.L, h->dFocal.p, h->dFocal.p + c.L.F, h->dMask.p,
                       h->dG.p, h->dH.p);
    HIP_CHECK(hipGetLastError());
  }
  if (c.cross) launchCrossAssemble(c, x);
  h->tEnd(slot);
  if (h->dist()) {
    const int ct = h->tBegin(KC_COMM_EVAL);
    const size_t chunkH = static_cast<size_t>(h->ownChunk()) * B * B;
    commGroupStart(h);
    commAllReduce(h, h->dG.p, c.n, CT_F64, s);
    commAllReduce(h, h->dCostFrame.p, c.L.F, CT_F64, s);
    commReduceScatter(h, h->dH.p, h->dH.p + static_cast<size_t>(h->rank) * chunkH, chunkH, CT_F64, s);
    commGroupEnd(h);
    Layout own = c.L;
    own.F = h->ownCount();
    if (own.F > 0)
      hipLaunchKernelGGL(k_extract_diag, dim3((static_cast<size_t>(own.F) * B + 255) / 256), dim3(256), 0, s, own,
                         h->dH.p + static_cast<size_t>(h->ownFirst()) * B * B, h->dHd.p + static_cast<size_t>(h->ownFirst()) * B);
    const size_t chunkD = static_cast<size_t>(h->ownChunk()) * B;
    commAllGather(h, h->dHd.p + static_cast<size_t>(h->rank) * chunkD, h->dHd.p, chunkD, CT_F64, s);
    h->tEnd(ct);
  } else {
    hipLaunchKernelGGL(k_extract_diag, dim3((c.n + 255) / 256), dim3(256), 0, s, c.L, h->dH.p, h->dHd.p);
  }
  hipLaunchKernelGGL(k_sum2, dim3(1), dim3(256), 0, s, h->dCostFrame.p, c.L.F, h->dCostFrame.p, 0, h->dScal.p, S_COST);
  HIP_CHECK(hipGetLastError());
  if (noReadBack) return 0.0;
  if (withStats) {
    HIP_CHECK(hipMemsetAsync(h->dLam.p, 0, c.n * sizeof(double), s));
    enqueueStats(c);
  }
  readScalars(c);
  return h->hScal[S_COST];
}

void touchModule_eval() {
  hipFuncAttributes a;
  (void)hipFuncGetAttributes(&a, reinterpret_cast<const void*>(k_sum2));
}

}

#ifdef CVD_ASM_PROFILE
extern "C" int32_t cvd_debug_asm_profile(unsigned long long* out) {
  (void)hipDeviceSynchronize();
  return hipMemcpyFromSymbol(out, HIP_SYMBOL(cvd::g_asmProf), sizeof(unsigned long long) * 2048 * 16) == hipSuccess ? 0 : 1;
}
#endif
```

### robust_cvd_amd/csrc/cvd_host.h

```cpp
#pragma once

#include <hip/hip_runtime.h>
#include <hip/hip_ext.h>
#include <rccl/rccl.h>
#include <rocblas/rocblas.h>
#include <rocsolver/rocsolver.h>

#include <algorithm>
#include <array>
#include <atomic>
#include <chrono>
#include <condition_variable>
#include <cmath>
#include <cstdarg>
#include <cstdint>
#include <cstdio>
#include <cstdlib>
#include <cstring>
#include <functional>
#include <limits>
#include <map>
#include <memory>
#include <mutex>
#include <set>
#include <stdexcept>
#include <string>
#include <thread>
#include <tuple>
#include <vector>

#include "../../include/cvd_hip_debug.h"
#include "cvd_kernels.h"


namespace cvd {

inline std::string fmt(const char* f, ...) {
  char buf[1024];
  va_list ap;
  va_start(ap, f);
  vsnprintf(buf, sizeof(buf), f, ap);
  va_end(ap);
  return buf;
}

#define HIP_CHECK(expr)                                                                          \
  do {                                                                                           \
    hipError_t e_ = (expr);                                                                      \
    if (e_ != hipSuccess)                                                                        \
      throw std::runtime_error(fmt("HIP error %s at %s:%d: %s", hipGetErrorName(e_), __FILE__,    \
                                   __LINE__, hipGetErrorString(e_)));                            \
  } while (0)

#define NCCL_CHECK(expr)                                                                         \
  do {                                                                                           \
    ncclResult_t r_ = (expr);                                                                    \
    if (r_ != ncclSuccess)                                                                       \
      throw std::runtime_error(fmt("RCCL error %s at %s:%d", ncclGetErrorString(r_), __FILE__, __LINE__)); \
  } while (0)

inline double nowSeconds() {
  using namespace std::chrono;
  return duration<double>(steady_clock::now().time_since_epoch()).count();
}

template <typename T>
struct DevBuf {
  T* p = nullptr;
  size_t n = 0;
  ~DevBuf() { release(); }
  void release() {
    if (p) (void)hipFree(p);
    p = nullptr;
    n = 0;
  }
  void ensure(size_t count) {
    if (count <= n) return;
    release();
    HIP_CHECK(hipMalloc(reinterpret_cast<void**>(&p), std::max<size_t>(count, 1) * sizeof(T)));
    n = count;
  }
  void upload(const T* src, size_t count, hipStream_t s) {
    ensure(count);
    if (count) HIP_CHECK(hipMemcpyAsync(p, src, count * sizeof(T), hipMemcpyHostToDevice, s));
  }
  void download(T* dst, size_t count, hipStream_t s) const {
    if (count) HIP_CHECK(hipMemcpyAsync(dst, p, count * sizeof(T), hipMemcpyDeviceToHost, s));
  }
  void grow(size_t newCount, size_t keepCount, hipStream_t s) {
    DevBuf<T> bigger;
    bigger.ensure(newCount);
    if (keepCount) HIP_CHECK(hipMemcpyAsync(bigger.p, p, keepCount * sizeof(T), hipMemcpyDeviceToDevice, s));
    HIP_CHECK(hipStreamSynchronize(s));
    std::swap(p, bigger.p);
    std::swap(n, bigger.n);
  }
};

inline int valueNumParams(int t) {
  if (t == CVD_VALUE_SCALE) return 1;
  if (t == CVD_VALUE_SCALE_SHIFT) return 2;
  throw std::runtime_error("Invalid value transform.");
}
inline int xformBlockSize(const cvd_xform_desc& d) {
  if (d.type == CVD_XFORM_DEPTH) return d.depth_type == CVD_DEPTH_IDENTITY ? 0 : valueNumParams(d.value_xform);
  return d.spatial_type == CVD_SPATIAL_IDENTITY ? 0 : 2;
}
inline int xformNumBlocks(const cvd_xform_desc& d) {
  if (d.type == CVD_XFORM_DEPTH) {
    switch (d.depth_type) {
      case CVD_DEPTH_IDENTITY: return 0;
      case CVD_DEPTH_GLOBAL: return 1;
      case CVD_DEPTH_GRID: {
        const int gx = d.grid_size[0], gy = d.grid_size[1], gz = d.grid_size[2];
        if (gx > 1 || gy > 1)
          if (gx < 2 || gy < 2)
            throw std::runtime_error(
                "Spatial grid transforms must have at least two rows and columns, respectively.");
        if (valueNumParams(d.value_xform) * gx * gy * gz <= 1)
          throw std::runtime_error("Grid transform cannot have an empty grid.");
        return gx * gy * gz;
      }
      default: throw std::runtime_error("Invalid depth transform type.");
    }
  } else if (d.type == CVD_XFORM_SPATIAL) {
    switch (d.spatial_type) {
      case CVD_SPATIAL_IDENTITY: return 0;
      case CVD_SPATIAL_VERTICAL_LINEAR: return 2;
      case CVD_SPATIAL_CORNERS_BILINEAR: return 4;
      case CVD_SPATIAL_BILINEAR_GRID:
      case CVD_SPATIAL_BICUBIC_GRID:
        if (d.grid_size[1] < 2 || d.grid_size[0] < 2)
          throw std::logic_error("Need at least two rows and columns in depth transform grid.");
        return d.grid_size[0] * d.grid_size[1];
      default: throw std::runtime_error("Invalid spatial transform type.");
    }
  }
  throw std::runtime_error("Invalid transform type.");
}

enum KernelClass { KC_ASSEMBLE = 0, KC_MATVEC_PAIRS, KC_MATVEC_FINISH, KC_CG_UPDATE, KC_INVERSE, KC_COST, KC_COUNT,
                   KC_COMM_EVAL = KC_COUNT, KC_COMM_PRODUCT, KC_COMM_COARSE,
                   KC_DENSE_WALK, KC_DENSE_GG, KC_TOTAL };

enum ProblemKind { PK_POSE_STEP = 0, PK_NORMALIZE = 1 };

enum CommType { CT_F64 = 0, CT_F32, CT_I32, CT_U64 };
struct LocalGroup;
struct Frontend;

}

namespace cvd {
std::shared_ptr<LocalGroup> joinLocalGroup(unsigned long long key, int world);
void leaveLocalGroup(LocalGroup& g);
std::shared_ptr<Frontend> makeFrontend();
}

using namespace cvd;

struct cvd_handle_t {
  int device = 0;
  hipStream_t stream = nullptr;
  std::string err;
  cvd_solver_options opt{};
  cvd_debug_options dbg{};

  int F = 0, W = 0, H = 0;
  float aspect = 1.f, invAspect = 1.f;
  DevBuf<float> dDepth;
  std::vector<float> median;
  DevBuf<float> dMedian;
  bool medianDirty = true;

  int P = 0;
  long long C = 0;
  std::vector<int> pairA, pairB;
  std::vector<long long> pairOff;
  DevBuf<int> dPairA, dPairB, dCPair;
  DevBuf<long long> dPairOff;
  DevBuf<float4> dLoc, dNdc, dNdcOrd;
  DevBuf<float2> dDsrc, dDsrcOrd;
  int orderGx = -1, orderGy = -1;
  bool tableOrdered = false;
  DevBuf<unsigned char> dStatic, dInRange, dRegOwner;
  bool dense = false;
  DevBuf<float2> dFlow;
  DevBuf<unsigned char> dFMask;

  ncclComm_t comm = nullptr;
  int rank = 0, world = 1;
  std::shared_ptr<LocalGroup> localGroup;
  bool phantom = false;
  DevBuf<unsigned char> dCommStage;
  DevBuf<const unsigned char*> dCommPtrs;
  bool distForced = false;
  bool dist() const { return world > 1 || distForced; }
  int ownChunk() const { return (F + world - 1) / world; }
  int ownFirst() const { return std::min(F, rank * ownChunk()); }
  int ownCount() const { return std::min(F, (rank + 1) * ownChunk()) - ownFirst(); }
  int framesPadded() const { return dist() ? ownChunk() * world : F; }
  bool haveTriplets = false;
  std::vector<int> tripCenter;
  std::vector<long long> tripOff;
  long long tripC = 0;
  DevBuf<float> dTLoc, dTDsrc;
  DevBuf<float2> dTNdc;
  DevBuf<unsigned char> dTStatic;
  DevBuf<int> dTGroupOfC, dTCenterAll, dTCenter, dTSlot, dFtOff, dFtList;
  DevBuf<long long> dTOff;
  DevBuf<double> dCostTrip;
  std::vector<int> tripActive;
  bool tableWithTriplets = false;
  long long numValidTrip = 0;
  int qRows = 0;

  std::vector<int> itemFa, itemFb;
  std::vector<long long> itemRange;
  DevBuf<int> dItemFa, dItemFb, dItemSlot, dFiOff, dFiList, dFpOff, dFpList;
  DevBuf<AsmPart> dAsmParts;
  DevBuf<int2> dAsmUnits;
  DevBuf<double> dAsmScratch;
  DevBuf<unsigned int> dAsmCount;
  int nAsmParts = 0, nAsmSlots = 0;
  int numCU = 256;
  hipStream_t stream2 = nullptr;
  rocblas_handle rbMain = nullptr;
  DevBuf<double> dInvScratch;
  DevBuf<int> dInvInfo;
  hipEvent_t evCoarseIn = nullptr, evCoarseDone = nullptr;
  hipStream_t stream3 = nullptr;
  hipEvent_t evInvIn = nullptr, evInvDone = nullptr;
  DevBuf<FrameConst> dFc2;
  DevBuf<long long> dItemRange;
  DevBuf<ItemRecord> dItemRec;
  std::vector<int> xFa, xFb;
  DevBuf<int> dXFa, dXFb, dXSlot, dXFiOff, dXPairEdge, dXDiagSlot;
  bool xDiagRows = false;
  int xRows = 0;
  DevBuf<long long> dXRange;
  DevBuf<double> dXBlocks;
  DevBuf<int> dDwPair, dDwRecOff, dXDir;
  DevBuf<double> dDwRecords, dDwGg;
  int nDwRecords = 0;
  bool denseAsList = false;
  bool denseListValid = false;
  std::vector<long long> denseListOff;
  DevBuf<int> dDlCounts;
  DevBuf<long long> dDlOffsets;
  DevBuf<unsigned int> dCounters;
  DevBuf<unsigned int> dTailBar;
  DevBuf<double> dOwnerScal;
  std::vector<unsigned char> tableRange;
  bool tableValid = false;
  bool tableIgnoresStatic = false;
  long long numValid = 0;

  std::vector<cvd_frame_pose> poses;
  cvd_xform_desc ddesc{}, sdesc{};
  std::vector<double> dparams, sparams;
  std::vector<std::array<double, 7>> poseParams;
  bool poseParamsValid = false;

  DevBuf<double> dX, dXc, dG, dLam, dMask, dScale, dDx, dR, dR1, dZ, dP0, dP1, dQ, dH, dQPart;
  DevBuf<float> dMinv;
  DevBuf<double> dFdot, dCostItem, dCostFrame, dScal, dHd, dFocal;
  DevBuf<double> dStatPart;
  DevBuf<unsigned char> dDynMask;
  DevBuf<double> dAdaptW;
  int dynW = 0, dynH = 0, adaptGx = 0, adaptGy = 0;
  bool haveDynMasks = false;
  std::shared_ptr<Frontend> frontend;

  struct CoarseHost {
    bool valid = false;
    int nEdges = 0, nBlocks = 0, nLevels = 0;
    std::vector<int> itemEdge;
    DevBuf<int> order, pos, levelPtr, levelCols, lvlBlkPtr, lvlBlks, blkCol, blkRow, colPtr, rowPtr, rowBlk, updPtr, updBlk,
        updA, updB, edgeBlk, edgeFa, edgeFb, wPtr, wRow, wtPtr, wtBlk, wtCol, wtFrame, wuPtr, wuL, wuW, itemEdgeDev, wSlot;
    DevBuf<double> edges, diag, Lb, Linv, Wb, rc, qc, y, c, dotPart, fdotY, wq, dropDiag;
    bool sparsified = false;
    bool temporalPose = false;
    int ptNn = 0, ptStepFrames = 0, ptN = 0, ptBlocks = 0;
    std::vector<int> edgeFaHost, edgeFbHost;
    DevBuf<int> ptA, ptB, ptPtr, ptList;
    DevBuf<double> ptMat, ptInv, ptR, ptT, ptDot, ptRec;
    DevBuf<TlStep> ptStepDev;
    std::vector<unsigned char> ptStepHost;
    DevBuf<unsigned int> ptCounter;
    bool denseMode = false;
    int denseForB = 0;
    bool denseReady = false;
    DevBuf<double> denseA, densePanel;
    DevBuf<double> denseInv;
    DevBuf<int> denseValid;
    int nW = 0;
    DevBuf<unsigned char> modeActive;
    DevBuf<int> fail;
    DevBuf<unsigned int> barrier;
    bool ptInvPending = false;
    int* ptInvFail = nullptr;
    DevBuf<double> Wb2;
    DevBuf<int> fail2;
    CoarsePlan plan{};
  } coarse;
  bool coarseOn = false;
  struct TemporalHost {
    bool on = false;
    bool built = false;
    int S = 0, Sx = 0, Sy = 0, nn = 0, step = 0, NT = 0, width = 0, nGroups = 0, nBlocks = 0;
    std::vector<unsigned char> stepHost;
    int tabGx = 0, tabGy = 0, tabSx = 0, tabSy = 0;
    int grpF = 0, grpStep = 0;
    std::vector<int> grpFa, grpFb;
    DevBuf<float> hx, hy, elW;
    DevBuf<int> bx, by, gOff, gItems, blkA, blkB, gPtr, gather, fail, valid;
    DevBuf<float4> vW;
    DevBuf<unsigned int> vIdx, counter;
    DevBuf<unsigned char> elV;
    DevBuf<double> Cf, E, part, A, Ainv, sq, rT, t, tl, dotPart, rec;
    DevBuf<double> invPanel;
    DevBuf<unsigned int> invBarrier;
    DevBuf<TlStep> stepDev;
    hipEvent_t evIn = nullptr, evDone = nullptr;
    bool sidePending = false;
    double* sqPtr = nullptr;
  } temporal;
  hipEvent_t evRebuild[2] = {nullptr, nullptr};
  bool rebuildTimed = false;
  double coarseRebuildMs = 0.0, pcgIterMs = 0.0;
  std::vector<std::pair<int, int>> globalEdges;
  bool haveGlobalEdges = false;
  DevBuf<double> dRegJac;
  DevBuf<unsigned short> dRegCol;
  DevBuf<unsigned char> dRegCnt;
  RegCache regCache{};
  DevBuf<FrameConst> dFc;
  DevBuf<int> dFail;
  DevBuf<unsigned long long> dCount;
  double* hScal = nullptr;
  double* hStage[2] = {nullptr, nullptr};
  size_t hStageN[2] = {0, 0};
  double* hPcg = nullptr;
  hipEvent_t pcgEvent[2] = {nullptr, nullptr};

  cvd_solve_summary summary{};
  std::vector<cvd_iteration_record> records;

  bool lastFusedTail = false, lastCross = false;
  bool lastShares = false;
  int lastShareCount = 0;
  int sharesF = -1, sharesN = -1;
  bool tailStageRows = false;
  int lastKD = 0;
  int lastProduct[6] = {0, 0, 0, -1, 0, 0};
  int lastAssembly[6] = {0, 0, 0, -1, 0, 0};
  bool tailDisabled = false;
  bool forceGeneric = false;

  int timing = 0;
  int timingStride = 1;
  long long timingCounter = 0;
  long long timingCounterKc[16] = {0};
  std::vector<std::pair<hipEvent_t, hipEvent_t>> evPool;
  std::vector<int> evClass;
  std::vector<int> evIter;
  int curPcgIter = -1;
  size_t evUsed = 0;
  double kcMs[KC_TOTAL] = {0};
  long long kcN[KC_TOTAL] = {0};

  ~cvd_handle_t() {
    for (auto& e : evPool) { (void)hipEventDestroy(e.first); (void)hipEventDestroy(e.second); }
    if (rbMain) (void)rocblas_destroy_handle(rbMain);
    if (comm) (void)ncclCommDestroy(comm);
    if (localGroup) leaveLocalGroup(*localGroup);
    if (hScal) (void)hipHostFree(hScal);
    for (auto& p : hStage) if (p) (void)hipHostFree(p);
    if (hPcg) (void)hipHostFree(hPcg);
    for (auto& e : pcgEvent) if (e) (void)hipEventDestroy(e);
    for (auto& e : evRebuild) if (e) (void)hipEventDestroy(e);
    if (temporal.evIn) (void)hipEventDestroy(temporal.evIn);
    if (temporal.evDone) (void)hipEventDestroy(temporal.evDone);
    if (evCoarseIn) (void)hipEventDestroy(evCoarseIn);
    if (evCoarseDone) (void)hipEventDestroy(evCoarseDone);
    if (evInvIn) (void)hipEventDestroy(evInvIn);
    if (evInvDone) (void)hipEventDestroy(evInvDone);
    if (stream3) (void)hipStreamDestroy(stream3);
    if (stream2) (void)hipStreamDestroy(stream2);
    if (stream) (void)hipStreamDestroy(stream);
  }

  int nD() const { return xformNumBlocks(ddesc) * xformBlockSize(ddesc); }
  int nS() const { return xformNumBlocks(sdesc) * xformBlockSize(sdesc); }
  int Bsz() const { return 7 + nD() + nS(); }

  int tBegin(int kc) {
    if (kc >= KC_COUNT ? timing == 0 : !(timing & (1 << kc))) return -1;
    if (timingStride > 1 && kc < KC_DENSE_WALK && (timingCounterKc[kc]++ % timingStride) != 0) return -1;
    if (evUsed == evPool.size()) {
      hipEvent_t a, b;
      HIP_CHECK(hipEventCreate(&a));
      HIP_CHECK(hipEventCreate(&b));
      evPool.emplace_back(a, b);
      evClass.push_back(kc);
      evIter.push_back(-1);
    }
    evClass[evUsed] = kc;
    evIter[evUsed] = curPcgIter;
    HIP_CHECK(hipEventRecord(evPool[evUsed].first, stream));
    return static_cast<int>(evUsed++);
  }
  void tEnd(int slot) {
    if (slot >= 0) HIP_CHECK(hipEventRecord(evPool[slot].second, stream));
  }
  int tReserve(int kc, hipEvent_t& start, hipEvent_t& stop) {
    start = nullptr;
    stop = nullptr;
    if (!(timing & (1 << kc))) return -1;
    if (timingStride > 1 && (timingCounter++ % timingStride) != 0) return -1;
    if (evUsed == evPool.size()) {
      hipEvent_t a, b;
      HIP_CHECK(hipEventCreate(&a));
      HIP_CHECK(hipEventCreate(&b));
      evPool.emplace_back(a, b);
      evClass.push_back(kc);
      evIter.push_back(-1);
    }
    evClass[evUsed] = kc;
    evIter[evUsed] = curPcgIter;
    start = evPool[evUsed].first;
    stop = evPool[evUsed].second;
    return static_cast<int>(evUsed++);
  }
  void tDropFrom(size_t firstSlot, int firstDeadIter) {
    for (size_t i = firstSlot; i < evUsed; ++i)
      if (evIter[i] >= firstDeadIter) evClass[i] = -1;
  }
  void tCollect() {
    if (!timing || evUsed == 0) return;
    HIP_CHECK(hipStreamSynchronize(stream));
    for (size_t i = 0; i < evUsed; ++i) {
      if (evClass[i] < 0) continue;
      float ms = 0.f;
      HIP_CHECK(hipEventElapsedTime(&ms, evPool[i].first, evPool[i].second));
      kcMs[evClass[i]] += ms;
      kcN[evClass[i]] += 1;
    }
    evUsed = 0;
  }
};

namespace cvd {

struct Ctx {
  cvd_handle* h;
  Layout L;
  int KD, KS;
  Table T;
  Items it;
  int nItems;
  size_t n;
  int boundDepth0 = 0;
  bool trip = false;
  TripletTable TT{};
  bool cross = false;
};

constexpr long long kListChunk = 768;
constexpr long long kDenseChunk = 8192;

constexpr int kMaxFrameBlock = 512;
constexpr int kDenseCoarseMaxUnknowns = 4928;
#define CVD_DISPATCH(KDv, KSv, ...)                                             \
  do {                                                                          \
    if (KDv == 1 && KSv == 0) { constexpr int KD = 1, KS = 0; __VA_ARGS__; }     \
    else if (KDv == 4 && KSv == 0) { constexpr int KD = 4, KS = 0; __VA_ARGS__; } \
    else if (KDv == 16 && KSv == 0) { constexpr int KD = 16, KS = 0; __VA_ARGS__; } \
    else if (KDv == 1 && KSv == 4) { constexpr int KD = 1, KS = 4; __VA_ARGS__; } \
    else if (KDv == 4 && KSv == 4) { constexpr int KD = 4, KS = 4; __VA_ARGS__; } \
    else if (KDv == 16 && KSv == 4) { constexpr int KD = 16, KS = 4; __VA_ARGS__; } \
    else if (KDv == 1 && KSv == 16) { constexpr int KD = 1, KS = 16; __VA_ARGS__; } \
    else if (KDv == 4 && KSv == 16) { constexpr int KD = 4, KS = 16; __VA_ARGS__; } \
    else { constexpr int KD = 16, KS = 16; __VA_ARGS__; }                        \
  } while (0)

#define CVD_DISPATCH_KD(KDv, ...)                                  \
  do {                                                             \
    if (KDv == 1) { constexpr int KD = 1; __VA_ARGS__; }            \
    else if (KDv == 4) { constexpr int KD = 4; __VA_ARGS__; }       \
    else { constexpr int KD = 16; __VA_ARGS__; }                    \
  } while (0)

constexpr size_t kMaxLds = 160 * 1024;

template <typename K>
void allowLds(K kernel, size_t bytes) {
  if (bytes > kMaxLds)
    throw std::runtime_error(fmt("per-frame block needs %zu B of LDS (> 160 KiB): frame block too large", bytes));
  if (bytes > 48 * 1024) {
    static std::map<std::pair<int, const void*>, size_t> granted;
    static std::mutex grantedMutex;
    int dev = 0;
    HIP_CHECK(hipGetDevice(&dev));
    std::lock_guard<std::mutex> lock(grantedMutex);
    size_t& g = granted[{dev, reinterpret_cast<const void*>(kernel)}];
    if (bytes > g) {
      HIP_CHECK(hipFuncSetAttribute(reinterpret_cast<const void*>(kernel), hipFuncAttributeMaxDynamicSharedMemorySize,
                                    static_cast<int>(bytes)));
// ... 239 lines not shown
```

### robust_cvd_amd/csrc/cvd_setup.hip

```cpp
#include "cvd_host.h"
#include "cvd_table.h"
#include "cvd_triplets.h"
#include "cvd_dense_walk.h"
#include <rocprim/device/device_segmented_radix_sort.hpp>

namespace cvd {

void launchFrameConsts(const Layout& L, const double* x, FrameConst* fc, hipStream_t s) {
  hipLaunchKernelGGL(k_frame_consts, dim3((L.F + 63) / 64), dim3(64), 0, s, L, x, fc);
}

static void quatToMatrix(const double q[4] , double R[3][3]) {
  for (int c = 0; c < 3; ++c) {
    double v[3] = {0, 0, 0};
    v[c] = 1.0;
    const double uv[3] = {2.0 * (q[1] * v[2] - q[2] * v[1]), 2.0 * (q[2] * v[0] - q[0] * v[2]),
                          2.0 * (q[0] * v[1] - q[1] * v[0])};
    R[0][c] = v[0] + q[3] * uv[0] + (q[1] * uv[2] - q[2] * uv[1]);
    R[1][c] = v[1] + q[3] * uv[1] + (q[2] * uv[0] - q[0] * uv[2]);
    R[2][c] = v[2] + q[3] * uv[2] + (q[0] * uv[1] - q[1] * uv[0]);
  }
}
static void matrixToAngleAxis(const double R[3][3], double aa[3]) {
  double q0, q1, q2, q3;
// ... 847 lines not shown
    h->dTNdc.ensure(static_cast<size_t>(std::max<long long>(h->tripC, 1)) * 3);
    h->dTDsrc.ensure(static_cast<size_t>(std::max<long long>(h->tripC, 1)) * 3);
    HIP_CHECK(hipMemsetAsync(h->dCount.p, 0, sizeof(unsigned long long), s));
    if (h->tripC > 0) {
      const unsigned grid = static_cast<unsigned>((h->tripC + 255) / 256);
      hipLaunchKernelGGL(k_build_triplet_table, dim3(grid), dim3(256), 0, s, h->W, h->H, h->invAspect, h->tripC,
                         h->dTLoc.p, h->dTGroupOfC.p, h->dTCenterAll.p, h->F, h->dInRange.p, h->dDepth.p, h->dTNdc.p,
                         h->dTDsrc.p, h->dCount.p);
      HIP_CHECK(hipGetLastError());
    }
    unsigned long long nvt = 0;
    HIP_CHECK(hipMemcpyAsync(&nvt, h->dCount.p, sizeof(nvt), hipMemcpyDeviceToHost, s));
    HIP_CHECK(hipStreamSynchronize(s));
    h->numValidTrip = static_cast<long long>(nvt);
    std::vector<int> mine;
    for (size_t k = 0; k < h->tripActive.size(); ++k)
      if (static_cast<int>(k) % h->world == h->rank) mine.push_back(h->tripActive[k]);
    h->tripActive.swap(mine);
    const int pairCodes = static_cast<int>(h->itemFa.size()) * 2;
    for (size_t k = 0; k < h->tripActive.size(); ++k) {
      const int f1 = h->tripCenter[h->tripActive[k]];
      for (int role = 0; role < 3; ++role) {
        frameItems[f1 - 1 + role].push_back(pairCodes + static_cast<int>(k) * 3 + role);
        frameTrips[f1 - 1 + role].push_back((static_cast<int>(k) << 2) | role);
      }
    }
  }
  h->tableWithTriplets = withTriplets;
  h->coarse.valid = false;
  if (static_cast<size_t>(h->F) * kCB <= kCoarseMaxUnknowns &&
      (!h->dist() ? !h->itemFa.empty() : h->haveGlobalEdges)) {
    std::map<std::pair<int, int>, int> edgeId;
    std::vector<std::pair<int, int>> edgeList;
    if (h->haveGlobalEdges) {
      for (const auto& e : h->globalEdges) {
        if (!inRange[e.first] || !inRange[e.second]) continue;
        edgeId.insert({e, static_cast<int>(edgeList.size())});
        edgeList.push_back(e);
      }
    }
    std::vector<int> itemEdge(h->itemFa.size());
    for (size_t i = 0; i < h->itemFa.size(); ++i) {
      const std::pair<int, int> key{h->itemFa[i], h->itemFb[i]};
      auto it = edgeId.find(key);
      if (it == edgeId.end()) {
        if (h->haveGlobalEdges) throw std::runtime_error("cvd_set_pair_graph: a frame pair with constraints is missing from the graph");
        it = edgeId.insert({key, static_cast<int>(edgeList.size())}).first;
        edgeList.push_back(key);
      }
      itemEdge[i] = it->second;
    }
    const long long updateBudget = h->opt.coarse_update_budget;
    h->coarse.sparsified = false;
    h->coarse.denseMode = false;
    const int denseMaxUnknowns = h->opt.coarse_dense_max_unknowns;
    const bool overBudget = coarseEliminationUpdates(h->F, edgeList) > updateBudget;
    {
      const int stepP = std::max(2, h->opt.coarse_temporal_step);
      const bool fits = ((h->F - 1 + stepP - 1) / stepP + 1) * kCB <= kDenseCoarseMaxUnknowns;
      const bool fusedScope = !h->dist() && h->opt.pcg_fused_tail != 0 && !h->forceGeneric && h->Bsz() <= 256 &&
                              h->opt.coarse_temporal_min_frames > 0 && h->F >= h->opt.coarse_temporal_min_frames &&
                              h->F + 2 * kTlMaxS <= 2 * h->numCU;
      h->coarse.temporalPose = fits && (h->opt.coarse_level == 3 || (overBudget && h->opt.coarse_over_budget == 0) ||
                                        (h->opt.coarse_over_budget == 0 && fusedScope));
    }
    if (h->coarse.temporalPose) {
      h->coarse.denseMode = true;
    } else if (overBudget && h->F * kCB <= denseMaxUnknowns) {
      h->coarse.denseMode = true;
    } else if (overBudget) {
      std::vector<int> newId(edgeList.size(), -1);
      std::vector<std::pair<int, int>> kept;
      for (size_t e = 0; e < edgeList.size(); ++e)
        if (coarseKeepsPair(edgeList[e].first, edgeList[e].second)) {
          newId[e] = static_cast<int>(kept.size());
          kept.push_back(edgeList[e]);
        }
      for (auto& ie : itemEdge) ie = newId[ie];
      h->coarse.sparsified = kept.size() != edgeList.size();
      edgeList.swap(kept);
    }
    buildCoarsePlan(h, edgeList, itemEdge);
    if (h->coarse.temporalPose) poseTemporalPlan(h);
    if (h->dense) {
      std::map<std::pair<int, int>, int> edgeOfPair;
      for (size_t i = 0; i < h->itemFa.size(); ++i) edgeOfPair[{h->itemFa[i], h->itemFb[i]}] = itemEdge[i];
      std::vector<int> pairEdge(std::max<size_t>(1, h->xFa.size()), -1);
      for (size_t k = 0; k < h->xFa.size(); ++k) {
        auto it = edgeOfPair.find({h->xFa[k], h->xFb[k]});
        if (it != edgeOfPair.end()) pairEdge[k] = it->second;
      }
      h->dXPairEdge.upload(pairEdge.data(), pairEdge.size(), s);
    }
  }
  std::vector<int> fiOff(h->F + 1, 0), fiList, fpOff(h->F + 1, 0), fpList;
  for (int f = 0; f < h->F; ++f) {
    fiOff[f + 1] = fiOff[f] + static_cast<int>(frameItems[f].size());
    fiList.insert(fiList.end(), frameItems[f].begin(), frameItems[f].end());
    fpOff[f + 1] = fpOff[f] + static_cast<int>(framePairs[f].size());
    fpList.insert(fpList.end(), framePairs[f].begin(), framePairs[f].end());
  }
  h->dItemFa.upload(h->itemFa.data(), h->itemFa.size(), s);
  h->dItemFb.upload(h->itemFb.data(), h->itemFb.size(), s);
  h->dItemRange.upload(h->itemRange.data(), h->itemRange.size(), s);
  std::vector<int> itemSlot(fiList.size(), 0);
  for (size_t e = 0; e < fiList.size(); ++e) itemSlot[fiList[e]] = static_cast<int>(e);
  h->qRows = static_cast<int>(fiList.size());
  h->dItemSlot.upload(itemSlot.data(), itemSlot.size(), s);
  {
    std::vector<ItemRecord> rec(std::max<size_t>(1, h->itemFa.size()), ItemRecord{});
    for (size_t i = 0; i < h->itemFa.size(); ++i)
      rec[i] = ItemRecord{h->itemFa[i], h->itemFb[i], itemSlot[2 * i], itemSlot[2 * i + 1], h->itemRange[4 * i], h->itemRange[4 * i + 1],
                          h->itemRange[4 * i + 2], h->itemRange[4 * i + 3], {0, 0}};
    h->dItemRec.upload(rec.data(), rec.size(), s);
  }
  if (withTriplets) {
    const size_t nG = h->tripActive.size();
    std::vector<long long> tOff(2 * std::max<size_t>(nG, 1), 0);
    std::vector<int> tCen(std::max<size_t>(nG, 1), 0), tSlot(3 * std::max<size_t>(nG, 1), 0);
    const int pairCodes = static_cast<int>(h->itemFa.size()) * 2;
    for (size_t k = 0; k < nG; ++k) {
      const int g = h->tripActive[k];
      tOff[2 * k] = h->tripOff[g];
      tOff[2 * k + 1] = h->tripOff[g + 1];
      tCen[k] = h->tripCenter[g];
      for (int role = 0; role < 3; ++role) tSlot[3 * k + role] = itemSlot[pairCodes + static_cast<int>(k) * 3 + role];
    }
    std::vector<int> ftOff(h->F + 1, 0), ftList;
    for (int f = 0; f < h->F; ++f) {
      ftOff[f + 1] = ftOff[f] + static_cast<int>(frameTrips[f].size());
      ftList.insert(ftList.end(), frameTrips[f].begin(), frameTrips[f].end());
    }
    h->dTOff.upload(tOff.data(), tOff.size(), s);
    h->dTCenter.upload(tCen.data(), tCen.size(), s);
    h->dTSlot.upload(tSlot.data(), tSlot.size(), s);
    h->dFtOff.upload(ftOff.data(), ftOff.size(), s);
    h->dFtList.upload(ftList.data(), ftList.size(), s);
    h->dCostTrip.ensure(std::max<size_t>(nG, 1));
  }
  {
    std::vector<int2> units;
    std::vector<int> fuOff(h->F + 1, 0);
    for (int f = 0; f < h->F; ++f) {
      for (const int code : framePairs[f]) {
        const long long n = h->pairOff[(code >> 1) + 1] - h->pairOff[code >> 1];
        for (long long o = 0; o < n; o += (h->dense ? kAsmUnitDense : kAsmUnit)) units.push_back(make_int2(code, static_cast<int>(o)));
      }
      fuOff[f + 1] = static_cast<int>(units.size());
    }
    int activeFrames = 0;
    for (int f = 0; f < h->F; ++f) activeFrames += inRange[f] ? 1 : 0;
    constexpr double partsPerCU = 1.0;
    const long long denom = std::max<long long>(1, std::max<long long>(activeFrames, static_cast<long long>(partsPerCU * h->numCU)));
    const int capU = static_cast<int>(std::max<long long>(kAsmThreads / 64, (static_cast<long long>(units.size()) + denom - 1) / denom));
    std::vector<AsmPart> parts;
    int slots = 0;
    for (int f = 0; f < h->F; ++f) {
      const int nu = fuOff[f + 1] - fuOff[f];
      const int np = std::max(1, (nu + capU - 1) / capU);
      const int per = (nu + np - 1) / np;
      for (int q = 0; q < np; ++q) {
        AsmPart a;
        a.frame = f;
        a.u0 = fuOff[f] + std::min(nu, q * per);
        a.u1 = fuOff[f] + std::min(nu, (q + 1) * per);
        a.part = q;
        a.nParts = np;
        a.slot0 = np > 1 ? slots : 0;
        parts.push_back(a);
      }
      if (np > 1) slots += np;
    }
    std::stable_sort(parts.begin(), parts.end(),
                     [](const AsmPart& a, const AsmPart& b) { return a.u1 - a.u0 > b.u1 - b.u0; });
    h->nAsmParts = static_cast<int>(parts.size());
    h->nAsmSlots = slots;
    h->dAsmParts.upload(parts.data(), parts.size(), s);
    h->dAsmUnits.upload(units.data(), units.size(), s);
    if (h->dAsmCount.n < static_cast<size_t>(h->F)) {
      h->dAsmCount.ensure(h->F);
      HIP_CHECK(hipMemsetAsync(h->dAsmCount.p, 0, sizeof(unsigned int) * h->F, s));
    }
  }
  h->dFiOff.upload(fiOff.data(), fiOff.size(), s);
  h->dFiList.upload(fiList.data(), fiList.size(), s);
  h->dFpOff.upload(fpOff.data(), fpOff.size(), s);
  h->dFpList.upload(fpList.data(), fpList.size(), s);
  HIP_CHECK(hipStreamSynchronize(s));
  h->tableRange = inRange;
  h->tableValid = true;
}
void orderTable(cvd_handle* h, const Layout& L, int KD) {
  int gx = 0, gy = 0;
  if (!h->dense && h->C > 0 && h->opt.constraint_order != 0 && L.depthType == kDepthGrid && L.gz <= 1 && (KD == 4 || KD == 16) &&
      L.gx * L.gy <= kOrderMaxCells) {
    gx = L.gx;
    gy = L.gy;
  }
  if (h->orderGx == gx && h->orderGy == gy) return;
  h->orderGx = gx;
  h->orderGy = gy;
  h->tableOrdered = false;
  if (gx == 0) return;
  h->dNdcOrd.ensure(h->C);
  h->dDsrcOrd.ensure(h->C);
  const size_t lds = static_cast<size_t>(gx * gy + 1) * sizeof(int) + 3 * kOrderCap * sizeof(unsigned short);
  allowLds(k_order_table, lds);
  hipLaunchKernelGGL(k_order_table, dim3(h->P), dim3(64), lds, h->stream, h->dPairOff.p, gx, gy, L.maxcx, L.maxcy, h->dNdc.p,
                     h->dDsrc.p, h->dNdcOrd.p, h->dDsrcOrd.p);
  HIP_CHECK(hipGetLastError());
  h->tableOrdered = true;
}

double* pinnedStage(cvd_handle* h, int which, size_t n) {
  if (h->hStageN[which] < n) {
    if (h->hStage[which]) HIP_CHECK(hipHostFree(h->hStage[which]));
    h->hStage[which] = nullptr;
    HIP_CHECK(hipHostMalloc(reinterpret_cast<void**>(&h->hStage[which]), std::max<size_t>(n, 1) * sizeof(double)));
    h->hStageN[which] = n;
  }
  return h->hStage[which];
}

void uploadState(cvd_handle* h, const Layout& L, DevBuf<double>& dst) {
  const size_t nAll = static_cast<size_t>(L.F) * L.B;
  double* x = pinnedStage(h, 1, nAll);
  const int nD = L.nD, nS = L.nS;
  for (int f = 0; f < L.F; ++f) {
    double* xf = &x[static_cast<size_t>(f) * L.B];
    for (int i = 0; i < 7; ++i) xf[i] = h->poseParams[f][i];
    for (int i = 0; i < nD; ++i) xf[7 + i] = h->dparams[static_cast<size_t>(f) * nD + i];
    for (int i = 0; i < nS; ++i) xf[7 + nD + i] = h->sparams[static_cast<size_t>(f) * nS + i];
  }
  dst.upload(x, nAll, h->stream);
  HIP_CHECK(hipStreamSynchronize(h->stream));
}

void downloadState(cvd_handle* h, const Layout& L, const DevBuf<double>& src) {
  const size_t nAll = static_cast<size_t>(L.F) * L.B;
  double* x = pinnedStage(h, 0, nAll);
  src.download(x, nAll, h->stream);
  HIP_CHECK(hipStreamSynchronize(h->stream));
  const int nD = L.nD, nS = L.nS;
  for (int f = 0; f < L.F; ++f) {
    const double* xf = &x[static_cast<size_t>(f) * L.B];
    for (int i = 0; i < 7; ++i) h->poseParams[f][i] = xf[i];
    for (int i = 0; i < nD; ++i) h->dparams[static_cast<size_t>(f) * nD + i] = xf[7 + i];
    for (int i = 0; i < nS; ++i) h->sparams[static_cast<size_t>(f) * nS + i] = xf[7 + nD + i];
  }
}

void buildMask(cvd_handle* h, const Layout& L, const cvd_opt_params& p, ProblemKind kind,
                      const std::vector<int>& range) {
  const size_t nAll = static_cast<size_t>(L.F) * L.B;
  HIP_CHECK(hipStreamSynchronize(h->stream));
  double* m = pinnedStage(h, 0, nAll);
  std::fill(m, m + nAll, 0.0);
  for (int f : range) {
    double* mf = &m[static_cast<size_t>(f) * L.B];
    const bool poseFree = (kind == PK_POSE_STEP) && !p.fix_poses;
    for (int i = 0; i < 6; ++i) mf[i] = poseFree ? 1.0 : 0.0;
    mf[6] = (kind == PK_POSE_STEP && p.intr_opt != CVD_INTR_FIXED) ? 1.0 : 0.0;
    const bool depthFree = (kind == PK_NORMALIZE) || !p.fix_depth_xforms;
    for (int i = 0; i < L.nD; ++i) mf[7 + i] = depthFree ? 1.0 : 0.0;
    const bool spatialFree = (kind == PK_POSE_STEP) && !p.fix_spatial_xforms;
    for (int i = 0; i < L.nS; ++i) mf[7 + L.nD + i] = spatialFree ? 1.0 : 0.0;
  }
  h->dMask.upload(m, nAll, h->stream);
}

void ensureBuffers(Ctx& c) {
  cvd_handle* h = c.h;
  const size_t n = c.n;
  const size_t B = c.L.B;
  h->dX.ensure(n); h->dXc.ensure(n); h->dG.ensure(n); h->dLam.ensure(n); h->dScale.ensure(n);
  const size_t nVec = static_cast<size_t>(h->framesPadded()) * B;
  if (h->dist() && (h->dDx.n < nVec || h->dZ.n < nVec)) {
    h->dDx.ensure(nVec); h->dR.ensure(nVec); h->dZ.ensure(nVec);
    HIP_CHECK(hipMemsetAsync(h->dDx.p, 0, nVec * sizeof(double), h->stream));
    HIP_CHECK(hipMemsetAsync(h->dR.p, 0, nVec * sizeof(double), h->stream));
    HIP_CHECK(hipMemsetAsync(h->dZ.p, 0, nVec * sizeof(double), h->stream));
  }
  h->dDx.ensure(nVec); h->dR.ensure(nVec); h->dR1.ensure(n); h->dZ.ensure(nVec); h->dP0.ensure(n); h->dP1.ensure(n);
  h->dQ.ensure(nVec + static_cast<size_t>(c.L.F) * (kCB + kTlMaxS) + 8);
  h->dOwnerScal.ensure(2 * static_cast<size_t>(std::max(1, h->world)));
  h->dHd.ensure(n);
  {
    const size_t nPad = static_cast<size_t>(h->framesPadded()) * B;
    const bool grow = h->dH.n < nPad * B;
    h->dH.ensure(nPad * B); h->dMinv.ensure(nPad * B + 4); h->dHd.ensure(nPad);
    if (h->dist() && (grow || nPad > n)) {
      HIP_CHECK(hipMemsetAsync(h->dH.p, 0, nPad * B * sizeof(double), h->stream));
      HIP_CHECK(hipMemsetAsync(h->dMinv.p, 0, nPad * B * sizeof(float), h->stream));
      HIP_CHECK(hipMemsetAsync(h->dHd.p, 0, nPad * sizeof(double), h->stream));
    }
  }
  h->dQPart.ensure(std::max<size_t>(1, static_cast<size_t>(std::max(std::max(h->qRows, c.nItems * 2), c.cross ? h->xRows : 0)) * B));
  h->dFdot.ensure(static_cast<size_t>(c.L.F) * 4 + 64);
  h->dCostItem.ensure(std::max(1, c.nItems));
  h->dCostFrame.ensure(c.L.F);
  h->dFocal.ensure(static_cast<size_t>(c.L.F) * 2);
  const bool newScal = h->dScal.p == nullptr;
  h->dScal.ensure(SH_END);
  h->dFc.ensure(c.L.F);
  h->dFail.ensure(1);
  if (!h->dCounters.p) {
    h->dCounters.ensure(8);
    HIP_CHECK(hipMemsetAsync(h->dCounters.p, 0, 8 * sizeof(unsigned int), h->stream));
  }
  if (!h->hScal) HIP_CHECK(hipHostMalloc(reinterpret_cast<void**>(&h->hScal), (S_COUNT + 1) * sizeof(double)));
  if (!h->hPcg) {
    HIP_CHECK(hipHostMalloc(reinterpret_cast<void**>(&h->hPcg), 16 * sizeof(double)));
    for (auto& e : h->pcgEvent) HIP_CHECK(hipEventCreateWithFlags(&e, hipEventDisableTiming));
  }
  if (newScal) {
    HIP_CHECK(hipMemsetAsync(h->dScal.p, 0, SH_END * sizeof(double), h->stream));
    std::memcpy(h->hPcg + kPcgMirrorAddressSlot, &h->hPcg, sizeof(double*));
    HIP_CHECK(hipMemcpyAsync(h->dScal.p + SH_MIRROR, h->hPcg + kPcgMirrorAddressSlot, sizeof(double), hipMemcpyHostToDevice, h->stream));
    h->sharesF = h->sharesN = -1;
  }
}
__global__ void k_pick_median(const float* __restrict__ sorted, size_t n, int first, int count, float* __restrict__ median) {
  const int i = blockIdx.x * blockDim.x + threadIdx.x;
  if (i < count) median[first + i] = sorted[static_cast<size_t>(i) * n + n / 2];
}
void refreshMedians(cvd_handle* h) {
  if (!h->medianDirty) return;
  hipStream_t s = h->stream;
  const size_t n = static_cast<size_t>(h->W) * h->H;
  const int F = h->F;
  h->dMedian.ensure(F);
// ... 33 lines not shown
```

Before: 355.7.

## Walk assembly work as contiguous per-wave segments with double-buffered row staging

Precomputes on the host a per-wave list of merged contiguous segments (same pair and side) for the sparse assembly work list. The specialised assembly kernel walks these segments instead of individual units, and can use two LDS staging rows per wave so the next partner row loads while the current one is consumed. The aim is to cut per-unit scalar overhead and hide the latency of loading partner rows. In exchange it uses more LDS, which can reduce occupancy, and adds setup work plus debug knobs and profiling hooks.

```diff
diff --git a/include/cvd_hip_debug.h b/include/cvd_hip_debug.h
--- a/include/cvd_hip_debug.h
+++ b/include/cvd_hip_debug.h
@@ -15,6 +15,8 @@
   int32_t stall_fused_tail_once;
   int32_t tail_no_row_staging;
   int32_t tail_closes_scalars;
+  int32_t asm_force_stage_depth;
+  int32_t asm_force_part_units;
 } cvd_debug_options;
 void cvd_debug_options_default(cvd_debug_options* o);
 int32_t cvd_set_debug_options(cvd_handle* h, const cvd_debug_options* o);
@@ -38,7 +40,7 @@
 int32_t cvd_coarse_debug(cvd_handle* h, int32_t* num_unknowns, double* a_c, double* a_c_inverse, int32_t* failed);
 int32_t cvd_temporal_debug(cvd_handle* h, int32_t* dims6, double* a_t, double* a_t_inverse, double* lam, int32_t* failed);
 int32_t cvd_product_launch_debug(cvd_handle* h, int32_t* out6);
-int32_t cvd_assembly_launch_debug(cvd_handle* h, int32_t* out6, double* cost_frame);
+int32_t cvd_assembly_launch_debug(cvd_handle* h, int32_t* out8, double* cost_frame);
 
 #ifdef __cplusplus
 }
diff --git a/robust_cvd_amd/api.py b/robust_cvd_amd/api.py
--- a/robust_cvd_amd/api.py
+++ b/robust_cvd_amd/api.py
@@ -49,6 +49,8 @@
         ("stall_fused_tail_once", C.c_int32),
         ("tail_no_row_staging", C.c_int32),
         ("tail_closes_scalars", C.c_int32),
+        ("asm_force_stage_depth", C.c_int32),
+        ("asm_force_part_units", C.c_int32),
     ]
 
 
@@ -1644,12 +1646,12 @@
 
     def assembly_launch_debug(self):
         import numpy as np
-        out = (C.c_int32 * 6)()
+        out = (C.c_int32 * 8)()
         cost = np.zeros(self.num_frames, dtype=np.float64)
         self._check(self._fn("assembly_launch_debug")(self._h, out, cost.ctypes.data_as(C.POINTER(C.c_double))))
         kind = {-1: "none", 0: "generic", 1: "fast list", 2: "fast dense", 3: "dense fold"}[out[3]]
         return {"threads": out[0], "spec": out[1], "kd": out[2], "kind": out[3], "kind_name": kind, "workgroups": out[4],
-                "split_parts": out[5], "cost_frame": cost}
+                "split_parts": out[5], "stage_depth": out[6], "segments": out[7], "cost_frame": cost}
 
     def coarse_debug(self):
         import numpy as np
diff --git a/robust_cvd_amd/csrc/cvd_api.hip b/robust_cvd_amd/csrc/cvd_api.hip
--- a/robust_cvd_amd/csrc/cvd_api.hip
+++ b/robust_cvd_amd/csrc/cvd_api.hip
@@ -279,11 +279,16 @@
   o->stall_fused_tail_once = 0;
   o->tail_no_row_staging = 0;
   o->tail_closes_scalars = 0;
+  o->asm_force_stage_depth = 0;
+  o->asm_force_part_units = 0;
 }
 int32_t cvd_set_debug_options(cvd_handle* h, const cvd_debug_options* o) {
   CVD_TRY(h, {
     if (o->struct_size != CVD_STRUCT_STAMP(cvd_debug_options))
       throw std::runtime_error("cvd_debug_options: struct_size does not match this library's cvd_hip_debug.h (start from cvd_debug_options_default)");
+    if (o->asm_force_stage_depth < 0 || o->asm_force_stage_depth > 3) throw std::runtime_error("asm_force_stage_depth in {0, 1, 2, 3}");
+    if (o->asm_force_part_units < 0) throw std::runtime_error("asm_force_part_units >= 0");
+    if (o->asm_force_part_units != h->dbg.asm_force_part_units) h->tableValid = false;
     h->dbg = *o;
     h->distForced = h->world == 1 && (h->comm != nullptr || h->localGroup || h->phantom) && o->force_sharded_path != 0;
   });
@@ -1053,9 +1058,9 @@
     for (int i = 0; i < 6; ++i) out6[i] = h->lastProduct[i];
   });
 }
-int32_t cvd_assembly_launch_debug(cvd_handle* h, int32_t* out6, double* cost_frame) {
-  CVD_TRY(h, {
-    for (int i = 0; i < 6; ++i) out6[i] = h->lastAssembly[i];
+int32_t cvd_assembly_launch_debug(cvd_handle* h, int32_t* out8, double* cost_frame) {
+  CVD_TRY(h, {
+    for (int i = 0; i < 8; ++i) out8[i] = h->lastAssembly[i];
     const size_t F = static_cast<size_t>(h->F);
     if (cost_frame && h->lastAssembly[3] >= 0 && h->dCostFrame.n >= F) {
       h->dCostFrame.download(cost_frame, F, h->stream);
diff --git a/robust_cvd_amd/csrc/cvd_asm_segments.h b/robust_cvd_amd/csrc/cvd_asm_segments.h
--- /dev/null
+++ b/robust_cvd_amd/csrc/cvd_asm_segments.h
@@ -0,0 +1,63 @@
+#pragma once
+
+#include <cstdint>
+#include <vector>
+
+namespace cvd {
+
+struct alignas(32) AsmSegment {
+  int32_t other;
+  int32_t side;
+  long long first;
+  int32_t count;
+  int32_t last;
+  int32_t pad[2];
+};
+static_assert(sizeof(AsmSegment) == 32, "one scalar load per segment");
+
+struct AsmSegs {
+  const AsmSegment* seg;
+  const int32_t* waveOff;
+  int32_t depth;
+};
+
+struct AsmUnitRange { int32_t u0, u1; };
+struct AsmUnitDesc { int32_t code, offset; };
+
+inline void cutAsmSegments(const std::vector<AsmUnitRange>& parts, const std::vector<AsmUnitDesc>& units, const int32_t* pairA,
+                           const int32_t* pairB, const long long* pairOff, int waves, int unitSize, std::vector<AsmSegment>& seg,
+                           std::vector<int32_t>& waveOff) {
+  seg.clear();
+  waveOff.assign(parts.size() * static_cast<size_t>(waves) + 1, 0);
+  for (size_t q = 0; q < parts.size(); ++q) {
+    const int nu = parts[q].u1 - parts[q].u0;
+    const int base = nu / waves, rem = nu % waves;
+    int u = parts[q].u0;
+    for (int w = 0; w < waves; ++w) {
+      const int uEnd = u + base + (w < rem ? 1 : 0);
+      const size_t segBegin = seg.size();
+      int lastCode = -1;
+      for (; u < uEnd; ++u) {
+        const int p = units[u].code >> 1, side = units[u].code & 1;
+        const long long first = pairOff[p] + units[u].offset;
+        const long long left = pairOff[p + 1] - first;
+        const int32_t n = static_cast<int32_t>(left < unitSize ? left : unitSize);
+        if (units[u].code == lastCode && seg.back().first + seg.back().count == first) {
+          seg.back().count += n;
+          continue;
+        }
+        lastCode = units[u].code;
+        AsmSegment s{};
+        s.other = side ? pairA[p] : pairB[p];
+        s.side = side;
+        s.first = first;
+        s.count = n;
+        seg.push_back(s);
+      }
+      if (seg.size() > segBegin) seg.back().last = 1;
+      waveOff[q * waves + w + 1] = static_cast<int32_t>(seg.size());
+    }
+  }
+}
+
+}
diff --git a/robust_cvd_amd/csrc/cvd_assembly.h b/robust_cvd_amd/csrc/cvd_assembly.h
--- a/robust_cvd_amd/csrc/cvd_assembly.h
+++ b/robust_cvd_amd/csrc/cvd_assembly.h
@@ -1,6 +1,7 @@
 #pragma once
 
 #include "cvd_kernels.h"
+#include "cvd_asm_segments.h"
 
 namespace cvd {
 
@@ -263,135 +264,275 @@
 #ifdef CVD_ASM_PROFILE
 __device__ unsigned long long g_asmProf[2048 * 16];
 #define ASM_STAMP(slot) do { if (lane == 0) g_asmProf[(blockIdx.x & 2047) * 16 + (slot)] = wall_clock64(); } while (0)
+__device__ unsigned long long g_asmWait[2048 * 8 * 8];
+#define ASM_WAIT_DECL unsigned long long asmT[5] = {0, 0, 0, 0, 0}; unsigned long long asmT0 = 0
+#define ASM_WAIT_BEGIN() do { asmT0 = wall_clock64(); } while (0)
+#define ASM_WAIT_LAP(k) do { asm volatile("s_waitcnt vmcnt(0) lgkmcnt(0)" ::: "memory"); const unsigned long long t_ = wall_clock64(); \
+                             asmT[k] += t_ - asmT0; asmT0 = t_; } while (0)
+#define ASM_WAIT_MARK(k) do { const unsigned long long t_ = wall_clock64(); asmT[k] += t_ - asmT0; asmT0 = t_; } while (0)
+#define ASM_WAIT_FLUSH() do { if (lane == 0) for (int k_ = 0; k_ < 5; ++k_) g_asmWait[((blockIdx.x & 2047) * 8 + (wv & 7)) * 8 + k_] = asmT[k_]; } while (0)
+#define ASM_WAIT_PARAMS , unsigned long long (&asmT)[5], unsigned long long& asmT0
+#define ASM_WAIT_ARGS , asmT, asmT0
 #else
 #define ASM_STAMP(slot) do {} while (0)
+#define ASM_WAIT_DECL
+#define ASM_WAIT_BEGIN() do {} while (0)
+#define ASM_WAIT_LAP(k) do {} while (0)
+#define ASM_WAIT_MARK(k) do {} while (0)
+#define ASM_WAIT_FLUSH() do {} while (0)
+#define ASM_WAIT_PARAMS
+#define ASM_WAIT_ARGS
 #endif
+
+struct AsmEntryScalars {
+  double RaU[9], RbU[9], dTU[3];
+  double fxa, fya, ifxb, ifyb;
+  __device__ __forceinline__ void form(const Layout& L, const FrameConst& Fa, const FrameConst& Fb) {
+    const double A = L.aspect;
+#pragma unroll
+    for (int i = 0; i < 9; ++i) { RaU[i] = uniformValue(Fa.R[i]); RbU[i] = uniformValue(Fb.R[i]); }
+#pragma unroll
+    for (int i = 0; i < 3; ++i) dTU[i] = uniformValue(Fa.t[i] - Fb.t[i]);
+    fya = uniformValue(Fa.fy);
+    fxa = fya * A;
+    const double fyb = uniformValue(Fb.fy);
+    ifyb = uniformValue(1.0 / fyb);
+    ifxb = uniformValue(1.0 / (fyb * A));
+  }
+};
+
+template <int KD, int SPEC>
+__device__ __forceinline__ void asmConstraintSpec(const Layout& L, const AsmEntryScalars& S, const float4 nd, const float2 d,
+                                                  const bool side, const double* __restrict__ xa, const double* __restrict__ xb,
+                                                  double* Hs, double* gs, double (&PP)[28], double (&gp)[7], double (&GD)[19],
+                                                  double& cost) {
+  const double A = L.aspect;
+  const double (&RaU)[9] = S.RaU;
+  const double (&RbU)[9] = S.RbU;
+  const double (&dTU)[3] = S.dTU;
+  const double fxa = S.fxa, fya = S.fya, ifxb = S.ifxb, ifyb = S.ifyb;
+  const double da = static_cast<double>(d.x), db = static_cast<double>(d.y);
+  FastTaps<KD> tm;
+  double Dm = 0.0, Do = 0.0;
+  {
+    FastTaps<KD> to;
+    fastGather<KD>(L, side ? nd.x : nd.z, side ? nd.y : nd.w, to);
+    const double* __restrict__ xo_ = side ? xa : xb;
+#pragma unroll
+    for (int k = 0; k < KD; ++k)
+      if (to.ok(k)) Do += xo_[7 + to.I(k)] * to.Wt(k);
+  }
+  fastGather<KD>(L, side ? nd.z : nd.x, side ? nd.w : nd.y, tm);
+  {
+    const double* __restrict__ xm_ = side ? xb : xa;
+#pragma unroll
+    for (int k = 0; k < KD; ++k)
+      if (tm.ok(k)) Dm += xm_[7 + tm.I(k)] * tm.Wt(k);
+  }
+  const double Da = (side ? Do : Dm) * da;
+  const double Db = (side ? Dm : Do) * db;
+  const double pax = static_cast<double>(nd.x), pay = static_cast<double>(nd.y);
+  const double pbx = static_cast<double>(nd.z), pby = static_cast<double>(nd.w);
+  double ca[3], Rca[3];
+  fastRay(RaU, pax, pay, fxa, fya, ca, Rca);
+  const double v[3] = {dTU[0] + Rca[0] * Da, dTU[1] + Rca[1] * Da, dTU[2] + Rca[2] * Da};
+  double zz, iz, u, vv, r[3], dr2dA, dr2dDb;
+  fastProject<true>(L, RbU, v, ifxb, ifyb, pbx, pby, zz, iz, u, vv, r[0], r[1]);
+  fastDepthResidual<true>(L, kLossDisparity, zz, iz, Db, r[2], dr2dA, dr2dDb);
+  const double sq = r[0] * r[0] + r[1] * r[1] + r[2] * r[2];
+  const double w = fastRobustRho1<SPEC>(L, sq);
+  if (!side) cost += fastRobustRho0<SPEC>(L, sq);
+
+  double m00, m11, m02, m12;
+  fastRows(L, iz, u, vv, ifxb, ifyb, m00, m11, m02, m12);
+  const double m22 = -dr2dA;
+  double G[3][3];
+#pragma unroll
+  for (int i = 0; i < 3; ++i) {
+    G[0][i] = m00 * RbU[i * 3 + 0] + m02 * RbU[i * 3 + 2];
+    G[1][i] = m11 * RbU[i * 3 + 1] + m12 * RbU[i * 3 + 2];
+    G[2][i] = m22 * RbU[i * 3 + 2];
+  }
+  double Jp[3][7];
+  double JD[3];
+  if (!side) {
+    const double X[3] = {Da * Rca[0], Da * Rca[1], Da * Rca[2]};
+    const double cf0 = pax * A, cf1 = pay;
+    const double dXdf[3] = {Da * (RaU[0] * cf0 + RaU[1] * cf1), Da * (RaU[3] * cf0 + RaU[4] * cf1),
+                            Da * (RaU[6] * cf0 + RaU[7] * cf1)};
+#pragma unroll
+    for (int rr = 0; rr < 3; ++rr) {
+      Jp[rr][0] = G[rr][0]; Jp[rr][1] = G[rr][1]; Jp[rr][2] = G[rr][2];
+      Jp[rr][3] = X[1] * G[rr][2] - X[2] * G[rr][1];
+      Jp[rr][4] = X[2] * G[rr][0] - X[0] * G[rr][2];
+      Jp[rr][5] = X[0] * G[rr][1] - X[1] * G[rr][0];
+      Jp[rr][6] = dot3(G[rr], dXdf);
+      JD[rr] = dot3(G[rr], Rca);
+    }
+  } else {
+#pragma unroll
+    for (int rr = 0; rr < 3; ++rr) {
+      Jp[rr][0] = -G[rr][0]; Jp[rr][1] = -G[rr][1]; Jp[rr][2] = -G[rr][2];
+      Jp[rr][3] = G[rr][1] * v[2] - G[rr][2] * v[1];
+      Jp[rr][4] = G[rr][2] * v[0] - G[rr][0] * v[2];
+      Jp[rr][5] = G[rr][0] * v[1] - G[rr][1] * v[0];
+    }
+    Jp[0][6] = -L.ws * u * ifyb;
+    Jp[1][6] = -L.ws * vv * ifyb;
+    Jp[2][6] = 0.0;
+    JD[0] = 0.0; JD[1] = 0.0; JD[2] = dr2dDb;
+  }
+  int qi = 0;
+#pragma unroll
+  for (int i = 0; i < 7; ++i) {
+    gp[i] += w * (Jp[0][i] * r[0] + Jp[1][i] * r[1] + Jp[2][i] * r[2]);
+#pragma unroll
+    for (int j = 0; j <= i; ++j) {
+      PP[qi] += w * (Jp[0][i] * Jp[0][j] + Jp[1][i] * Jp[1][j] + Jp[2][i] * Jp[2][j]);
+      ++qi;
+    }
+  }
+  double v7[7];
+#pragma unroll
+  for (int i = 0; i < 7; ++i) v7[i] = w * (Jp[0][i] * JD[0] + Jp[1][i] * JD[1] + Jp[2][i] * JD[2]);
+  const double sDD = w * (JD[0] * JD[0] + JD[1] * JD[1] + JD[2] * JD[2]);
+  const double sDr = w * (JD[0] * r[0] + JD[1] * r[1] + JD[2] * r[2]);
+  const double dm = side ? db : da;
+  if constexpr (KD == 1) {
+    const double fac = tm.Wt(0) * dm;
+#pragma unroll
+    for (int i = 0; i < 7; ++i) GD[i] += v7[i] * fac;
+    GD[17] += sDr * fac;
+    GD[14] += sDD * fac * fac;
+  } else {
+#pragma unroll
+    for (int ka = 0; ka < KD; ++ka) {
+      if (!tm.ok(ka)) continue;
+      const double fa = tm.Wt(ka) * dm;
+      const int ct = 7 + tm.I(ka);
+      const int rowBase = ct * (ct + 1) / 2;
+      atomicAdd(&gs[ct], sDr * fa);
+#pragma unroll
+      for (int i = 0; i < 7; ++i) atomicAdd(&Hs[rowBase + i], v7[i] * fa);
+      const double sfa = sDD * fa;
+#pragma unroll
+      for (int kb = 0; kb <= ka; ++kb) {
+        if (!tm.ok(kb)) continue;
+        const int c2 = 7 + tm.I(kb);
+        const int hi = (KD == 16 || ct > c2) ? ct : c2, lo = (KD == 16 || ct > c2) ? c2 : ct;
+        atomicAdd(&Hs[packedIdx(hi, lo)], sfa * (tm.Wt(kb) * dm));
+      }
+    }
+  }
+}
 
 template <int KD, int SPEC>
 __device__ __forceinline__ void asmWalkSpec(const Layout& L, const Table& T, RecordStream<false>& rs, long long cBegin, int n,
                                             int lane, const bool side, const FrameConst& Fa, const FrameConst& Fb,
                                             const double* __restrict__ xa, const double* __restrict__ xb, double* Hs,
-                                            double* gs, double (&PP)[28], double (&gp)[7], double (&GD)[19], double& cost) {
-  const double A = L.aspect;
-  double RaU[9], RbU[9], dTU[3];
-#pragma unroll
-  for (int i = 0; i < 9; ++i) { RaU[i] = uniformValue(Fa.R[i]); RbU[i] = uniformValue(Fb.R[i]); }
-#pragma unroll
-  for (int i = 0; i < 3; ++i) dTU[i] = uniformValue(Fa.t[i] - Fb.t[i]);
-  const double fya = uniformValue(Fa.fy), fxa = fya * A;
-  const double fyb = uniformValue(Fb.fy);
-  const double ifyb = uniformValue(1.0 / fyb), ifxb = uniformValue(1.0 / (fyb * A));
+                                            double* gs, double (&PP)[28], double (&gp)[7], double (&GD)[19], double& cost ASM_WAIT_PARAMS) {
+  AsmEntryScalars S;
+  S.form(L, Fa, Fb);
+  ASM_WAIT_LAP(2);
   for (int ci = lane; ci < n; ci += 64) {
     float4 nd;
     float2 d;
     if (!rs.take(T, cBegin, ci, 64, n, 0, 0, 0, nd, d)) continue;
-    const double da = static_cast<double>(d.x), db = static_cast<double>(d.y);
-    FastTaps<KD> ta, tb;
-    fastGather<KD>(L, nd.x, nd.y, ta);
-    fastGather<KD>(L, nd.z, nd.w, tb);
-    double Da = 0.0, Db = 0.0;
-#pragma unroll
-    for (int k = 0; k < KD; ++k) {
-      if (ta.ok(k)) Da += xa[7 + ta.I(k)] * ta.Wt(k);
-      if (tb.ok(k)) Db += xb[7 + tb.I(k)] * tb.Wt(k);
-    }
-    Da *= da;
-    Db *= db;
-    const double pax = static_cast<double>(nd.x), pay = static_cast<double>(nd.y);
-    const double pbx = static_cast<double>(nd.z), pby = static_cast<double>(nd.w);
-    double ca[3], Rca[3];
-    fastRay(RaU, pax, pay, fxa, fya, ca, Rca);
-    const double v[3] = {dTU[0] + Rca[0] * Da, dTU[1] + Rca[1] * Da, dTU[2] + Rca[2] * Da};
-    double zz, iz, u, vv, r[3], dr2dA, dr2dDb;
-    fastProject<true>(L, RbU, v, ifxb, ifyb, pbx, pby, zz, iz, u, vv, r[0], r[1]);
-    fastDepthResidual<true>(L, kLossDisparity, zz, iz, Db, r[2], dr2dA, dr2dDb);
-    const double sq = r[0] * r[0] + r[1] * r[1] + r[2] * r[2];
-    const double w = fastRobustRho1<SPEC>(L, sq);
-    if (!side) cost += fastRobustRho0<SPEC>(L, sq);
-
-    double m00, m11, m02, m12;
-    fastRows(L, iz, u, vv, ifxb, ifyb, m00, m11, m02, m12);
-    const double m22 = -dr2dA;
-    double G[3][3];
-#pragma unroll
-    for (int i = 0; i < 3; ++i) {
-      G[0][i] = m00 * RbU[i * 3 + 0] + m02 * RbU[i * 3 + 2];
-      G[1][i] = m11 * RbU[i * 3 + 1] + m12 * RbU[i * 3 + 2];
-      G[2][i] = m22 * RbU[i * 3 + 2];
-    }
-    double Jp[3][7];
-    double JD[3];
-    if (!side) {
-      const double X[3] = {Da * Rca[0], Da * Rca[1], Da * Rca[2]};
-      const double cf0 = pax * A, cf1 = pay;
-      const double dXdf[3] = {Da * (RaU[0] * cf0 + RaU[1] * cf1), Da * (RaU[3] * cf0 + RaU[4] * cf1),
-                              Da * (RaU[6] * cf0 + RaU[7] * cf1)};
-#pragma unroll
-      for (int rr = 0; rr < 3; ++rr) {
-        Jp[rr][0] = G[rr][0]; Jp[rr][1] = G[rr][1]; Jp[rr][2] = G[rr][2];
-        Jp[rr][3] = X[1] * G[rr][2] - X[2] * G[rr][1];
-        Jp[rr][4] = X[2] * G[rr][0] - X[0] * G[rr][2];
-        Jp[rr][5] = X[0] * G[rr][1] - X[1] * G[rr][0];
-        Jp[rr][6] = dot3(G[rr], dXdf);
-        JD[rr] = dot3(G[rr], Rca);
-      }
-    } else {
-#pragma unroll
-      for (int rr = 0; rr < 3; ++rr) {
-        Jp[rr][0] = -G[rr][0]; Jp[rr][1] = -G[rr][1]; Jp[rr][2] = -G[rr][2];
-        Jp[rr][3] = G[rr][1] * v[2] - G[rr][2] * v[1];
-        Jp[rr][4] = G[rr][2] * v[0] - G[rr][0] * v[2];
-        Jp[rr][5] = G[rr][0] * v[1] - G[rr][1] * v[0];
-      }
-      Jp[0][6] = -L.ws * u * ifyb;
-      Jp[1][6] = -L.ws * vv * ifyb;
-      Jp[2][6] = 0.0;
-      JD[0] = 0.0; JD[1] = 0.0; JD[2] = dr2dDb;
-    }
-    int qi = 0;
-#pragma unroll
-    for (int i = 0; i < 7; ++i) {
-      gp[i] += w * (Jp[0][i] * r[0] + Jp[1][i] * r[1] + Jp[2][i] * r[2]);
-#pragma unroll
-      for (int j = 0; j <= i; ++j) {
-        PP[qi] += w * (Jp[0][i] * Jp[0][j] + Jp[1][i] * Jp[1][j] + Jp[2][i] * Jp[2][j]);
-        ++qi;
-      }
-    }
-    double v7[7];
-#pragma unroll
-    for (int i = 0; i < 7; ++i) v7[i] = w * (Jp[0][i] * JD[0] + Jp[1][i] * JD[1] + Jp[2][i] * JD[2]);
-    const double sDD = w * (JD[0] * JD[0] + JD[1] * JD[1] + JD[2] * JD[2]);
-    const double sDr = w * (JD[0] * r[0] + JD[1] * r[1] + JD[2] * r[2]);
-    const FastTaps<KD>& tm = side ? tb : ta;
-    const double dm = side ? db : da;
-    if constexpr (KD == 1) {
-      const double fac = tm.Wt(0) * dm;
-#pragma unroll
-      for (int i = 0; i < 7; ++i) GD[i] += v7[i] * fac;
-      GD[17] += sDr * fac;
-      GD[14] += sDD * fac * fac;
-    } else {
-#pragma unroll
-      for (int ka = 0; ka < KD; ++ka) {
-        if (!tm.ok(ka)) continue;
-        const double fa = tm.Wt(ka) * dm;
-        const int ct = 7 + tm.I(ka);
-        const int rowBase = ct * (ct + 1) / 2;
-        atomicAdd(&gs[ct], sDr * fa);
-#pragma unroll
-        for (int i = 0; i < 7; ++i) atomicAdd(&Hs[rowBase + i], v7[i] * fa);
-        const double sfa = sDD * fa;
-#pragma unroll
-        for (int kb = 0; kb <= ka; ++kb) {
-          if (!tm.ok(kb)) continue;
-          const int c2 = 7 + tm.I(kb);
-          const int hi = (KD == 16 || ct > c2) ? ct : c2, lo = (KD == 16 || ct > c2) ? c2 : ct;
-          atomicAdd(&Hs[packedIdx(hi, lo)], sfa * (tm.Wt(kb) * dm));
-        }
-      }
-    }
-  }
+    asmConstraintSpec<KD, SPEC>(L, S, nd, d, side, xa, xb, Hs, gs, PP, gp, GD, cost);
+  }
+}
+
+__device__ __forceinline__ void asmStageAhead(const double* __restrict__ src, double* dstRow, int B, int lane) {
+  const unsigned int* g = reinterpret_cast<const unsigned int*>(src);
+  const unsigned int lds = static_cast<unsigned int>(reinterpret_cast<uintptr_t>(
+      (__attribute__((address_space(3))) void*)dstRow));
+  const int nDw = 2 * B;
+  for (int k0 = 0; k0 < nDw; k0 += 64) {
+    if (k0 + lane < nDw) {
+      unsigned int keep;
+      const unsigned int dst = __builtin_amdgcn_readfirstlane(lds + 4u * static_cast<unsigned int>(k0));
+      asm volatile("s_mov_b32 %0, m0\n\ts_mov_b32 m0, %2\n\ts_nop 0\n\tglobal_load_lds_dword %1, off\n\ts_mov_b32 m0, %0"
+                   : "=&s"(keep) : "v"(g + k0 + lane), "s"(dst) : "memory");
+    }
+  }
+}
+
+inline DenseRecords asmSegsAsArgument(const AsmSegs& s) {
+  return DenseRecords{reinterpret_cast<const double*>(s.seg), s.waveOff,
+                      reinterpret_cast<const int*>(static_cast<uintptr_t>(s.depth)), nullptr};
+}
+__host__ __device__ __forceinline__ AsmSegs asmSegsFromArgument(const DenseRecords& d) {
+  return AsmSegs{reinterpret_cast<const AsmSegment*>(d.records), d.recOff,
+                 static_cast<int32_t>(reinterpret_cast<uintptr_t>(d.fpOff))};
+}
+
+template <int KD, int SPEC, bool STAGE>
+__device__ __forceinline__ void asmWalkSegments(const Layout& L, const Table& T, const double* __restrict__ x,
+                                                const FrameConst* __restrict__ fc, const int f, const AsmSegs& segs, const int wv,
+                                                const int lane, const double* xf, double* xstage, double* Hs, double* gs,
+                                                double (&PP)[28], double (&gp)[7], double (&GD)[19], double& cost) {
+  const int B = L.B;
+  const int slot = static_cast<int>(blockIdx.x) * (kAsmThreads / 64) + wv;
+  int si = __builtin_amdgcn_readfirstlane(segs.waveOff[slot]);
+  const int sEnd = __builtin_amdgcn_readfirstlane(segs.waveOff[slot + 1]);
+  if (si >= sEnd) return;
+  ASM_WAIT_DECL;
+  ASM_WAIT_BEGIN();
+  const bool ahead = STAGE && segs.depth == 2;
+  double* rows = xstage + static_cast<size_t>(wv) * (ahead ? 2 : 1) * B;
+  int row = 0;
+  AsmSegment cur = segs.seg[si];
+  bool fresh = true;
+  float4 ndNext = make_float4(0.f, 0.f, 0.f, 0.f);
+  float2 dNext = make_float2(0.f, 0.f);
+  for (;;) {
+    if (fresh && lane < cur.count) { dNext = (T.dsrc + cur.first)[lane]; ndNext = (T.ndc + cur.first)[lane]; }
+    if constexpr (STAGE) {
+      if (fresh || !ahead) {
+        const double* __restrict__ xo = x + static_cast<size_t>(cur.other) * B;
+        double* xw = rows + static_cast<size_t>(row) * B;
+        for (int i = lane; i < B; i += 64) xw[i] = xo[i];
+      }
+    }
+    asm volatile("s_waitcnt vmcnt(0) lgkmcnt(0)" ::: "memory");
+    fresh = false;
+    const bool more = cur.last == 0;
+    AsmSegment nxt = cur;
+    if (more) nxt = segs.seg[si + 1];
+    const bool side = cur.side != 0;
+    AsmEntryScalars S;
+    S.form(L, side ? fc[cur.other] : fc[f], side ? fc[f] : fc[cur.other]);
+    const double* xov = STAGE ? rows + static_cast<size_t>(row) * B : x + static_cast<size_t>(cur.other) * B;
+    const double* xa = side ? xov : xf;
+    const double* xb = side ? xf : xov;
+    const int n = cur.count;
+    ASM_WAIT_LAP(2);
+    for (int base = 0; base < n; base += 64) {
+      const int ci = base + lane;
+      const float4 nd = ndNext;
+      const float2 d = dNext;
+      const bool within = base + 64 < n;
+      const long long rb = within ? cur.first : nxt.first;
+      const int ri = within ? ci + 64 : lane;
+      const int rn = within ? n : (more ? nxt.count : 0);
+      if (ri < rn) {
+        dNext = *reinterpret_cast<const float2*>(reinterpret_cast<const char*>(T.dsrc + rb) + static_cast<unsigned int>(ri) * 8u);
+        ndNext = *reinterpret_cast<const float4*>(reinterpret_cast<const char*>(T.ndc + rb) + static_cast<unsigned int>(ri) * 16u);
+      }
+      if (!within && more && ahead)
+        asmStageAhead(x + static_cast<size_t>(nxt.other) * B, rows + static_cast<size_t>(row ^ 1) * B, B, lane);
+      if (ci < n && d.x > 0.f) asmConstraintSpec<KD, SPEC>(L, S, nd, d, side, xa, xb, Hs, gs, PP, gp, GD, cost);
+    }
+    ASM_WAIT_MARK(3);
+#ifdef CVD_ASM_PROFILE
+    ++asmT[4];
+#endif
+    if (!more) break;
+    if (ahead) row ^= 1;
+    ++si;
+    cur = nxt;
+  }
+  ASM_WAIT_FLUSH();
 }
 
 template <int NT>
@@ -591,9 +732,16 @@
     }
   } else
   if (L.includeStatic) {
+    if constexpr (SPEC != 0 && NT > 64) {
+      const AsmSegs segs = asmSegsFromArgument(dr);
+      asmWalkSegments<KD, SPEC, STAGE>(L, T, x, fc, f, segs, wv, lane, xf, xstage, Hs, gs, PP, gp, GD, cost);
+    } else {
+    ASM_WAIT_DECL;
     for (int u = me.u0 + wv; u < me.u1; u += NT / 64) {
+      if constexpr (SPEC != 0) ASM_WAIT_BEGIN();
       const int2 unit = work.units[u];
       const int code = __builtin_amdgcn_readfirstlane(unit.x);
+      if constexpr (SPEC != 0) ASM_WAIT_LAP(0);
       const int p = code >> 1;
       const int side = code & 1;
       const int o = side ? T.pairA[p] : T.pairB[p];
@@ -606,6 +754,10 @@
         const long long cb = pOff + __builtin_amdgcn_readfirstlane(unit.y);
         const long long pEnd = T.pairOff[p + 1];
         const int n = static_cast<int>((cb + kAsmUnit < pEnd ? cb + kAsmUnit : pEnd) - cb);
+#ifdef CVD_ASM_PROFILE
+        asm volatile("" :: "s"(o), "s"(n));
+#endif
+        ASM_WAIT_LAP(1);
         RecordStream<false> rs;
         rs.prime(T, cb, lane, n);
         if constexpr (STAGE) {
@@ -614,7 +766,11 @@
         }
         const double* xov = STAGE ? xw : xo;
         asmWalkSpec<KD, SPEC>(L, T, rs, cb, n, lane, side != 0, Fa, Fb, side ? xov : xf,
-                              side ? xf : xov, Hs, gs, PP, gp, GD, cost);
+                              side ? xf : xov, Hs, gs, PP, gp, GD, cost ASM_WAIT_ARGS);
+        ASM_WAIT_LAP(3);
+#ifdef CVD_ASM_PROFILE
+        ++asmT[4];
+#endif
         continue;
       }
       if constexpr (STAGE) {
@@ -872,6 +1028,8 @@
         }
       }
     }
+    if constexpr (SPEC != 0) ASM_WAIT_FLUSH();
+    }
   }
   ASM_STAMP(4 + wv);
   __syncthreads();
diff --git a/robust_cvd_amd/csrc/cvd_eval.hip b/robust_cvd_amd/csrc/cvd_eval.hip
--- a/robust_cvd_amd/csrc/cvd_eval.hip
+++ b/robust_cvd_amd/csrc/cvd_eval.hip
@@ -150,25 +150,38 @@
   const size_t ldsRest = 3 * B * 8 + 2 * sizeof(FrameConst) + 4 * 36 * 8;
   int panelCap = 0;
   const bool fastFits = ldsFast <= kMaxLds;
-  auto recordAsm = [h](int threads, int spec, int kd, int kind, int groups, int splitParts) {
-    const int v[6] = {threads, spec, kd, kind, groups, splitParts};
-    for (int i = 0; i < 6; ++i) h->lastAssembly[i] = v[i];
+  auto recordAsm = [h](int threads, int spec, int kd, int kind, int groups, int splitParts, int stageDepth = -1, int segments = 0) {
+    const int v[8] = {threads, spec, kd, kind, groups, splitParts, stageDepth, segments};
+    for (int i = 0; i < 8; ++i) h->lastAssembly[i] = v[i];
   };
   if (fast && fastFits) {
     h->dAsmScratch.ensure(static_cast<size_t>(h->nAsmSlots) * (B * (B + 1) / 2 + B + 4));
     const AsmWork work{h->dAsmParts.p, h->dAsmUnits.p, h->dAsmScratch.p, h->dAsmCount.p};
     const int spec = (!h->dense && c.L.N == 1 && c.L.lossType == CVD_STATIC_REPRO_DISPARITY && c.L.intrOpt != CVD_INTR_SHARED)
                          ? (c.L.robustKind == 0 ? 1 : 2) : 0;
-    const size_t ldsStage = ldsFast + static_cast<size_t>(kAsmThreads / 64) * B * 8;
-    const bool stage = ldsStage <= kMaxLds;
+    const size_t ldsRow = static_cast<size_t>(kAsmThreads / 64) * B * 8;
+    const bool segWalk = spec != 0 && kAsmThreads > 64;
+    int depth = ldsFast + ldsRow <= kMaxLds ? 1 : 0;
+    if (segWalk && ldsFast + 2 * ldsRow <= kMaxLds) depth = 2;
+    if (segWalk && h->dbg.asm_force_stage_depth != 0) {
+      const int forced = h->dbg.asm_force_stage_depth - 1;
+      if (forced < 0 || forced > 2 || ldsFast + forced * ldsRow > kMaxLds)
+        throw std::runtime_error(fmt("asm_force_stage_depth: %d staging rows per wave do not fit the LDS at B = %d", forced, static_cast<int>(B)));
+      depth = forced;
+    }
+    const size_t ldsStage = ldsFast + static_cast<size_t>(depth) * ldsRow;
+    const bool stage = depth > 0;
+    const AsmSegs segs{h->dAsmSegs.p, h->dAsmWaveOff.p, depth};
+    if (segWalk && !h->dAsmWaveOff.p) throw std::logic_error("assembly: the segment list of the work list is missing");
 #define CVD_LAUNCH_ASM_S(DENSEV, STAGEV, SPECV)                                                                            \
     CVD_DISPATCH_KD(c.KD, {                                                                                              \
-      recordAsm(kAsmThreads, SPECV, KD, DENSEV ? 2 : 1, h->nAsmParts, h->nAsmSlots);                                       \
+      if (SPECV != 0 && kAsmThreads > 64) recordAsm(kAsmThreads, SPECV, KD, 1, h->nAsmParts, h->nAsmSlots, depth, h->nAsmSegs); \
+      else recordAsm(kAsmThreads, SPECV, KD, DENSEV ? 2 : 1, h->nAsmParts, h->nAsmSlots);                                  \
       allowLds((k_assemble_fast<KD, DENSEV, STAGEV, false, SPECV>), STAGEV ? ldsStage : ldsFast);                          \
       hipLaunchKernelGGL((k_assemble_fast<KD, DENSEV, STAGEV, false, SPECV>), dim3(h->nAsmParts),                          \
                          dim3(kAsmThreads), STAGEV ? ldsStage : ldsFast, s,                                                \
                          c.L, c.T, x, h->dFc.p, h->dMask.p, h->dMedian.p, h->dRegOwner.p, h->dInRange.p, work, h->dG.p, h->dH.p,  \
-                         h->dCostFrame.p, h->dFocal.p, h->dFocal.p + c.L.F);                                             \
+                         h->dCostFrame.p, h->dFocal.p, h->dFocal.p + c.L.F, asmSegsAsArgument(segs));                    \
     })
 #define CVD_LAUNCH_ASM(DENSEV, STAGEV) CVD_LAUNCH_ASM_S(DENSEV, STAGEV, 0)
 #ifndef CVD_ASM_STAGE
@@ -270,4 +283,8 @@
   (void)hipDeviceSynchronize();
   return hipMemcpyFromSymbol(out, HIP_SYMBOL(cvd::g_asmProf), sizeof(unsigned long long) * 2048 * 16) == hipSuccess ? 0 : 1;
 }
+extern "C" int32_t cvd_debug_asm_waits(unsigned long long* out) {
+  (void)hipDeviceSynchronize();
+  return hipMemcpyFromSymbol(out, HIP_SYMBOL(cvd::g_asmWait), sizeof(unsigned long long) * 2048 * 8 * 8) == hipSuccess ? 0 : 1;
+}
 #endif
diff --git a/robust_cvd_amd/csrc/cvd_host.h b/robust_cvd_amd/csrc/cvd_host.h
--- a/robust_cvd_amd/csrc/cvd_host.h
+++ b/robust_cvd_amd/csrc/cvd_host.h
@@ -31,6 +31,7 @@
 
 #include "../../include/cvd_hip_debug.h"
 #include "cvd_kernels.h"
+#include "cvd_asm_segments.h"
 
 
 namespace cvd {
@@ -223,6 +224,9 @@
   DevBuf<double> dAsmScratch;
   DevBuf<unsigned int> dAsmCount;
   int nAsmParts = 0, nAsmSlots = 0;
+  DevBuf<AsmSegment> dAsmSegs;
+  DevBuf<int32_t> dAsmWaveOff;
+  int nAsmSegs = 0;
   int numCU = 256;
   hipStream_t stream2 = nullptr;
   rocblas_handle rbMain = nullptr;
@@ -354,7 +358,7 @@
   bool tailStageRows = false;
   int lastKD = 0;
   int lastProduct[6] = {0, 0, 0, -1, 0, 0};
-  int lastAssembly[6] = {0, 0, 0, -1, 0, 0};
+  int lastAssembly[8] = {0, 0, 0, -1, 0, 0, -1, 0};
   bool tailDisabled = false;
   bool forceGeneric = false;
 
diff --git a/robust_cvd_amd/csrc/cvd_setup.hip b/robust_cvd_amd/csrc/cvd_setup.hip
--- a/robust_cvd_amd/csrc/cvd_setup.hip
+++ b/robust_cvd_amd/csrc/cvd_setup.hip
@@ -1023,7 +1023,8 @@
     for (int f = 0; f < h->F; ++f) activeFrames += inRange[f] ? 1 : 0;
     constexpr double partsPerCU = 1.0;
     const long long denom = std::max<long long>(1, std::max<long long>(activeFrames, static_cast<long long>(partsPerCU * h->numCU)));
-    const int capU = static_cast<int>(std::max<long long>(kAsmThreads / 64, (static_cast<long long>(units.size()) + denom - 1) / denom));
+    const int capRule = static_cast<int>(std::max<long long>(kAsmThreads / 64, (static_cast<long long>(units.size()) + denom - 1) / denom));
+    const int capU = h->dbg.asm_force_part_units > 0 ? h->dbg.asm_force_part_units : capRule;
     std::vector<AsmPart> parts;
     int slots = 0;
     for (int f = 0; f < h->F; ++f) {
@@ -1048,6 +1049,20 @@
     h->nAsmSlots = slots;
     h->dAsmParts.upload(parts.data(), parts.size(), s);
     h->dAsmUnits.upload(units.data(), units.size(), s);
+    h->nAsmSegs = 0;
+    if (!h->dense) {
+      std::vector<AsmUnitRange> ranges(parts.size());
+      for (size_t q = 0; q < parts.size(); ++q) ranges[q] = AsmUnitRange{parts[q].u0, parts[q].u1};
+      std::vector<AsmUnitDesc> descs(units.size());
+      for (size_t u = 0; u < units.size(); ++u) descs[u] = AsmUnitDesc{units[u].x, units[u].y};
+      std::vector<AsmSegment> segs;
+      std::vector<int32_t> waveOff;
+      cutAsmSegments(ranges, descs, h->pairA.data(), h->pairB.data(), h->pairOff.data(), kAsmThreads / 64, kAsmUnit, segs, waveOff);
+      h->nAsmSegs = static_cast<int>(segs.size());
+      if (segs.empty()) segs.push_back(AsmSegment{});
+      h->dAsmSegs.upload(segs.data(), segs.size(), s);
+      h->dAsmWaveOff.upload(waveOff.data(), waveOff.size(), s);
+    }
     if (h->dAsmCount.n < static_cast<size_t>(h->F)) {
       h->dAsmCount.ensure(h->F);
       HIP_CHECK(hipMemsetAsync(h->dAsmCount.p, 0, sizeof(unsigned int) * h->F, s));
```

After: 360.3 (median of 6 runs). 1.01x the previous value.
